# enkeejunior1/Diffusion-Pullback

Measured on AMD Instinct MI355X. Metric: pullback top-k SVD iters/sec (SD-v1.5 mid-block, 4x64x64), higher is better.
Workload: dtype bf16; 1 GPU; BASELINE configs[2]: SD-v1.5 4x64x64 latent, no edit prompt (seeded null ctx[1,77,768]), mid-block h[1280,8,8], t=696.27; pca_rank=5, ctx=null, samples_total=5, samples_this_rank=5, samples_advanced_together=1, spectrum=shaped (configs.Spectrum()), parallelism=single process, no collective, rccl_world_size=0, repeats=7

## Files before the change

### diffusion_pullback_amd/csrc/attn_fused.hip

```cpp
#include "kernels.h"

namespace dpb {

#ifndef DPB_ATT_ABL
#define DPB_ATT_ABL 0
#endif
#ifndef DPB_OUT_STORE_ATT
#define DPB_OUT_STORE_ATT 0
#endif
#define DPB_ATT_PAD 8

constexpr int att_waves(int d) { return d > 80 ? 4 : 8; }

template <int D, int W = att_waves(D)> struct FA {
  static constexpr int WAVES = W, NT = WAVES * 64;
  static constexpr int NS = (D + 15) / 16;
  static constexpr int DP = NS * 16;
  static constexpr int ND = (D + 31) / 32;
  static constexpr int DO = ND * 32;
  static constexpr int BI = D <= 80 ? 128 : 64;
  static constexpr int LDR = (DP > DO ? DP : DO) + DPB_ATT_PAD;
  static constexpr int LDT = BI + 4;
  static constexpr int ROW_ELEMS = BI * LDR;
  static constexpr int T_ELEMS = DO * LDT;
};

template <int D, int NTH = FA<D>::NT> struct RowRegs { uint4 v[(FA<D>::BI * (FA<D>::DP / 8) + NTH - 1) / NTH]; };
template <int D, int NTH = FA<D>::NT, unsigned ONE = 0>
__device__ inline void fetch_row(const bf16* __restrict__ src, long gs, RowRegs<D, NTH>& rg, int tid) {
  using F = FA<D>;
  constexpr int CPR = F::DP / 8, N = (F::BI * CPR + NTH - 1) / NTH;
#pragma unroll
  for (int i = 0; i < N; ++i) {
    const int c = tid + i * NTH;
    const int r = c / CPR, cc = (c % CPR) * 8;
    rg.v[i] = make_uint4(ONE != 0 && cc == D ? ONE : 0u, 0, 0, 0);
    if (c < F::BI * CPR && cc < D) rg.v[i] = *reinterpret_cast<const uint4*>(src + (long)r * gs + cc);
  }
}
template <int D, int NTH = FA<D>::NT>
__device__ inline void commit_row(const RowRegs<D, NTH>& rg, bf16* lds, int tid) {
  using F = FA<D>;
  constexpr int CPR = F::DP / 8, N = (F::BI * CPR + NTH - 1) / NTH;
#pragma unroll
  for (int i = 0; i < N; ++i) {
    const int c = tid + i * NTH;
    if (c < F::BI * CPR) *reinterpret_cast<uint4*>(lds + (c / CPR) * F::LDR + (c % CPR) * 8) = rg.v[i];
  }
}
template <int D, int NTH = FA<D>::NT> struct TRegs { uint4 v[(FA<D>::DO * (FA<D>::BI / 8) + NTH - 1) / NTH]; };
template <int D, int NTH = FA<D>::NT>
__device__ inline void fetch_t(const bf16* __restrict__ src, long gs, TRegs<D, NTH>& rg, int tid) {
  using F = FA<D>;
  constexpr int CPR = F::BI / 8, N = (F::DO * CPR + NTH - 1) / NTH;
#pragma unroll
  for (int i = 0; i < N; ++i) {
    const int c = tid + i * NTH;
    const int r = c / CPR, cc = (c % CPR) * 8;
    rg.v[i] = make_uint4(0, 0, 0, 0);
    if (c < F::DO * CPR && r < D) rg.v[i] = *reinterpret_cast<const uint4*>(src + (long)r * gs + cc);
  }
}
template <int D, int NTH = FA<D>::NT>
__device__ inline void commit_t(const TRegs<D, NTH>& rg, bf16* lds, int tid) {
  using F = FA<D>;
  constexpr int CPR = F::BI / 8, N = (F::DO * CPR + NTH - 1) / NTH;
#pragma unroll
  for (int i = 0; i < N; ++i) {
    const int c = tid + i * NTH;
    if (c < F::DO * CPR) {
      bf16* dst = lds + (c / CPR) * F::LDT + (c % CPR) * 8;
      *reinterpret_cast<uint2*>(dst) = make_uint2(rg.v[i].x, rg.v[i].y);
      *reinterpret_cast<uint2*>(dst + 4) = make_uint2(rg.v[i].z, rg.v[i].w);
    }
  }
}
template <int D>
__device__ inline void load_outer_frags(const bf16* __restrict__ rowptr, bf16x8* f, int lhi) {
  using F = FA<D>;
#pragma unroll
  for (int st = 0; st < F::NS; ++st) {
    const int col = st * 16 + lhi * 8;
    uint4 v = make_uint4(0, 0, 0, 0);
    if (col < D) v = *reinterpret_cast<const uint4*>(rowptr + col);
    f[st] = *reinterpret_cast<bf16x8*>(&v);
  }
}
__device__ inline bf16x8 lds_a_frag(const bf16* tile, int row, int ld, int col) {
  return *reinterpret_cast<const bf16x8*>(tile + row * ld + col);
}
__device__ inline bf16x8 lds_t_frag(const bf16* tile, int drow, int ld, int base, int lhi) {
  uint2 lo = *reinterpret_cast<const uint2*>(tile + drow * ld + base + 4 * lhi);
  uint2 hi = *reinterpret_cast<const uint2*>(tile + drow * ld + base + 8 + 4 * lhi);
  uint4 v = make_uint4(lo.x, lo.y, hi.x, hi.y);
  return *reinterpret_cast<bf16x8*>(&v);
}
typedef __attribute__((ext_vector_type(4))) short short4_;
__device__ inline bf16x8 lds_tr_frag(const bf16* tile, int ld, int base, int d0, int lane) {
  const int i16 = lane & 15, g = lane >> 4;
  const bf16* p = tile + (base + 4 * (g >> 1) + (i16 >> 2)) * ld + d0 + (g & 1) * 16 + (i16 & 3) * 4;
  short4_ lo = __builtin_amdgcn_ds_read_tr16_b64_v4i16((__attribute__((address_space(3))) short4_*)p);
  short4_ hi = __builtin_amdgcn_ds_read_tr16_b64_v4i16((__attribute__((address_space(3))) short4_*)(p + 8 * ld));
  uint2 l2 = *reinterpret_cast<uint2*>(&lo), h2 = *reinterpret_cast<uint2*>(&hi);
  uint4 v = make_uint4(l2.x, l2.y, h2.x, h2.y);
  return *reinterpret_cast<bf16x8*>(&v);
}
template <int FL>
__device__ inline void pack_b(const float* x, bf16x8* out) {
  out[0] = H16<FL>::pack8(x);
  out[1] = H16<FL>::pack8(x + 8);
}
struct BlockXY { int x, y; };
__device__ inline BlockXY xcd_group_blocks(int on) {
  const int nx = gridDim.x, ny = gridDim.y;
  if (!on || (ny & 7)) return {(int)blockIdx.x, (int)blockIdx.y};
  const int lin = blockIdx.y * nx + blockIdx.x, xcd = lin & 7, slot = lin >> 3;
  return {slot % nx, (slot / nx) * 8 + xcd};
}

static int g_attn_shared = getenv("DPB_ATTN_SHARED") ? atoi(getenv("DPB_ATTN_SHARED")) : 2;
void attn_debug_shared(int bits) { g_attn_shared = bits; }

#define MFMA(a, b, c) H16<FL>::mfma(a, b, c)

struct FusedArgs {
  const bf16 *Q, *K, *V, *O;
  const bf16 *KT, *VT, *QT;
  const float* stats;
  float* Drow;
  float* Dout;
  const bf16 *dQ, *dK, *dV, *dVT;
  bf16* dO;
  const bf16 *gO, *gOT;
  bf16 *gQ, *gK, *gV;
  int accQ, accK, accV;
  int xcd;
  int L, C, Co, H, kps;
  float scale;
};

template <int D, int FL, int W = att_waves(D)>
__global__ __launch_bounds__((FA<D, W>::NT)) void attn_fwd_kernel(FusedArgs a, bf16* O, float* stats_out) {
  using F = FA<D, W>;
  __shared__ __attribute__((aligned(16))) bf16 sm[2 * F::ROW_ELEMS];
  bf16* sK = sm; bf16* sV = sK + F::ROW_ELEMS;
  const int tid = threadIdx.x, lane = tid & 63, wave = tid >> 6, l31 = lane & 31, lhi = lane >> 5;
  const BlockXY blk = xcd_group_blocks(a.xcd);
  const int b = blk.y / a.H, h = blk.y % a.H;
  const int q_ = blk.x * (F::WAVES * 32) + wave * 32 + l31;
  const bool live = q_ < a.L;
  const int q = live ? q_ : a.L - 1;
  const long LC = (long)a.L * a.C;
  const bf16* Kp = a.K + b * LC + h * D;
  const bf16* Vp = a.V + b * LC + h * D;
  bf16x8 qf[F::NS];
  load_outer_frags<D>(a.Q + b * LC + (long)q * a.C + h * D, qf, lhi);
  const float c2 = a.scale * 1.44269504088896f;
  constexpr float FWD_THR = 4.f;
  constexpr bool LSUM = F::DP > D;
  constexpr unsigned ONE16 = FL ? 0x3C00u : 0x3F80u, VONE = LSUM ? ONE16 : 0u;
  f32x16 acc[F::ND];
#pragma unroll
  for (int d = 0; d < F::ND; ++d)
#pragma unroll
    for (int r = 0; r < 16; ++r) acc[d][r] = 0.f;
  float m = -INFINITY, l = 0.f;
  RowRegs<D, F::NT> rK, rV;
  fetch_row<D, F::NT>(Kp, a.C, rK, tid); fetch_row<D, F::NT, VONE>(Vp, a.C, rV, tid);
  for (int k0 = 0; k0 < a.L; k0 += F::BI) {
    __syncthreads();
    commit_row<D, F::NT>(rK, sK, tid); commit_row<D, F::NT>(rV, sV, tid);
    __syncthreads();
    if (k0 + F::BI < a.L) {
      const int k1 = k0 + F::BI;
      fetch_row<D, F::NT>(Kp + (long)k1 * a.C, a.C, rK, tid); fetch_row<D, F::NT, VONE>(Vp + (long)k1 * a.C, a.C, rV, tid);
    }
#pragma unroll
    for (int kb = 0; kb < F::BI / 32; ++kb) {
      f32x16 s;
#pragma unroll
      for (int r = 0; r < 16; ++r) s[r] = 0.f;
#pragma unroll
      for (int stp = 0; stp < F::NS; ++stp) s = MFMA(lds_a_frag(sK, kb * 32 + l31, F::LDR, stp * 16 + lhi * 8), qf[stp], s);
      float mx = s[0];
#pragma unroll
      for (int r = 1; r < 16; ++r) mx = fmaxf(mx, s[r]);
      mx = fmaxf(mx, __shfl_xor(mx, 32, 64)) * c2;
      if (!__all(mx - m <= FWD_THR)) {
        const float mn = fmaxf(m, mx);
        const float alpha = __builtin_amdgcn_exp2f(m - mn);
#pragma unroll
        for (int d = 0; d < F::ND; ++d)
#pragma unroll
          for (int r = 0; r < 16; ++r) acc[d][r] *= alpha;
        if (!LSUM) l *= alpha;
        m = mn;
      }
      float p[16];
#pragma unroll
      for (int r = 0; r < 16; ++r) p[r] = __builtin_amdgcn_exp2f(__builtin_fmaf(s[r], c2, -m));
      if (!LSUM) {
        float ps = 0.f;
#pragma unroll
        for (int r = 0; r < 16; ++r) ps += p[r];
        ps += __shfl_xor(ps, 32, 64);
        l += ps;
      }
      bf16x8 pb[2];
      pack_b<FL>(p, pb);
#pragma unroll
      for (int ks = 0; ks < 2; ++ks)
#pragma unroll
        for (int d = 0; d < F::ND; ++d)
          acc[d] = MFMA(lds_tr_frag(sV, F::LDR, kb * 32 + ks * 16, d * 32, lane), pb[ks], acc[d]);
    }
  }
  if (LSUM) {
    static_assert(!LSUM || (D % 8 == 0 && (D % 32) / 8 * 4 < 16), "ones column of V outside the accumulator layout");
    const float lv = acc[D / 32][(D % 32) / 8 * 4];
    const float lo = __shfl_xor(lv, 32, 64);
    l = lhi == 0 ? lv : lo;
  }
  const float il = 1.f / l;
  if (lhi == 0 && live) {
    float* st = stats_out + (((long)b * a.H + h) * a.L + q) * 2;
    st[0] = m * 0.69314718055994531f;
    st[1] = il;
  }
  bf16* Op = O + b * (long)a.L * a.Co + (long)q * a.Co + h * D;
#pragma unroll
  for (int d = 0; d < F::ND; ++d)
#pragma unroll
    for (int g = 0; g < 4; ++g) {
      const int col = d * 32 + 8 * g + 4 * lhi;
      if (col < D && live) {
        store_out8<DPB_OUT_STORE_ATT>(Op + col, H16<FL>::pack2(acc[d][g * 4] * il, acc[d][g * 4 + 1] * il),
                                                         H16<FL>::pack2(acc[d][g * 4 + 2] * il, acc[d][g * 4 + 3] * il));
      }
    }
}

template <int D, int FL, int W = att_waves(D)>
__global__ __launch_bounds__((FA<D, W>::NT), (W == 4 && D <= 40 ? 2 : 1)) void attn_jvp_kernel(FusedArgs a) {
  using F = FA<D, W>;
  __shared__ __attribute__((aligned(16))) bf16 sm[4 * F::ROW_ELEMS];
  bf16* sK = sm; bf16* sdK = sK + F::ROW_ELEMS; bf16* sV = sdK + F::ROW_ELEMS; bf16* sdV = sV + F::ROW_ELEMS;
  const int tid = threadIdx.x, lane = tid & 63, wave = tid >> 6, l31 = lane & 31, lhi = lane >> 5;
  const BlockXY blk = xcd_group_blocks(a.xcd);
  const int j = blk.y / a.H, h = blk.y % a.H, b = j / a.kps;
  const int q_ = blk.x * (F::WAVES * 32) + wave * 32 + l31;
  const bool live = q_ < a.L;
  const int q = live ? q_ : a.L - 1;
  const long LC = (long)a.L * a.C;
  const bf16* Qp = a.Q + b * LC + h * D;
  const bf16* Kp = a.K + b * LC + h * D;
  const bf16* dQp = a.dQ + j * LC + h * D;
  const bf16* dKp = a.dK + j * LC + h * D;
  const bf16* Vp = a.V + b * LC + h * D;
  const bf16* dVp = a.dV + j * LC + h * D;
  bf16x8 qf[F::NS], dqf[F::NS];
  load_outer_frags<D>(Qp + (long)q * a.C, qf, lhi);
  load_outer_frags<D>(dQp + (long)q * a.C, dqf, lhi);
  const float* st = a.stats + (((long)b * a.H + h) * a.L + q) * 2;
  const float c2 = a.scale * 1.44269504088896f;
  const float m2 = st[0] * 1.44269504088896f - __builtin_log2f(st[1]);
  constexpr bool SUMROW = F::DO > D && ((D % 32) & 4) == 0;
  constexpr unsigned ONE16 = FL ? 0x3C00u : 0x3F80u, VONE = (SUMROW && F::DP > D) ? ONE16 : 0u;
  if constexpr (SUMROW && F::DP == D) {
    for (int r = tid; r < F::BI; r += F::NT) {
      reinterpret_cast<unsigned short*>(sV)[r * F::LDR + D] = (unsigned short)ONE16;
      reinterpret_cast<unsigned short*>(sdV)[r * F::LDR + D] = 0;
    }
  }
  f32x16 acc[F::ND];
#pragma unroll
  for (int d = 0; d < F::ND; ++d)
#pragma unroll
    for (int r = 0; r < 16; ++r) acc[d][r] = 0.f;
  float delta = 0.f;
  RowRegs<D, F::NT> rK, rdK, rV, rdV;
  fetch_row<D, F::NT>(Kp, a.C, rK, tid); fetch_row<D, F::NT>(dKp, a.C, rdK, tid);
  fetch_row<D, F::NT, VONE>(Vp, a.C, rV, tid); fetch_row<D, F::NT>(dVp, a.C, rdV, tid);
  for (int k0 = 0; k0 < a.L; k0 += F::BI) {
    __syncthreads();
    commit_row<D, F::NT>(rK, sK, tid); commit_row<D, F::NT>(rdK, sdK, tid); commit_row<D, F::NT>(rV, sV, tid); commit_row<D, F::NT>(rdV, sdV, tid);
    __syncthreads();
    if (k0 + F::BI < a.L) {
      const int k1 = k0 + F::BI;
      fetch_row<D, F::NT>(Kp + (long)k1 * a.C, a.C, rK, tid); fetch_row<D, F::NT>(dKp + (long)k1 * a.C, a.C, rdK, tid);
      fetch_row<D, F::NT, VONE>(Vp + (long)k1 * a.C, a.C, rV, tid); fetch_row<D, F::NT>(dVp + (long)k1 * a.C, a.C, rdV, tid);
    }
    constexpr bool PIPE = D <= 40;
    bf16x8 kf[F::NS], dkf[F::NS];
    auto load1 = [&](int kb) {
#pragma unroll
      for (int stp = 0; stp < F::NS; ++stp) {
        kf[stp] = lds_a_frag(sK, kb * 32 + l31, F::LDR, stp * 16 + lhi * 8);
        dkf[stp] = lds_a_frag(sdK, kb * 32 + l31, F::LDR, stp * 16 + lhi * 8);
      }
    };
    if constexpr (PIPE) load1(0);
#pragma unroll
    for (int kb = 0; kb < F::BI / 32; ++kb) {
      bf16x8 vf[2][F::ND], dvf[2][F::ND];
      if constexpr (PIPE) {
#pragma unroll
        for (int ks = 0; ks < 2; ++ks)
#pragma unroll
          for (int d = 0; d < F::ND; ++d) {
            vf[ks][d] = lds_tr_frag(sV, F::LDR, kb * 32 + ks * 16, d * 32, lane);
            dvf[ks][d] = lds_tr_frag(sdV, F::LDR, kb * 32 + ks * 16, d * 32, lane);
          }
        __builtin_amdgcn_sched_barrier(0);
      } else {
        load1(kb);
      }
      f32x16 s, ds;
#pragma unroll
      for (int r = 0; r < 16; ++r) s[r] = ds[r] = 0.f;
#pragma unroll
      for (int stp = 0; stp < F::NS; ++stp) {
        s = MFMA(kf[stp], qf[stp], s);
        ds = MFMA(kf[stp], dqf[stp], ds);
        if (!((DPB_ATT_ABL & 2) && D == 40 && stp == F::NS - 1)) ds = MFMA(dkf[stp], qf[stp], ds);
      }
      if constexpr (PIPE) {
        __builtin_amdgcn_sched_barrier(0);
        if (kb + 1 < F::BI / 32) load1(kb + 1);
        __builtin_amdgcn_sched_barrier(0);
      }
      float p[16], x[16];
#pragma unroll
      for (int r = 0; r < 16; ++r) {
        p[r] = (DPB_ATT_ABL & 4) ? c2 * s[r] - m2 : __builtin_amdgcn_exp2f(c2 * s[r] - m2);
        x[r] = p[r] * (a.scale * ds[r]);
        if constexpr (!SUMROW) delta += x[r];
      }
      bf16x8 pb[2], xb[2];
      pack_b<FL>(p, pb);
      pack_b<FL>(x, xb);
#pragma unroll
      for (int ks = 0; ks < 2; ++ks)
#pragma unroll
        for (int d = 0; d < F::ND; ++d) {
          if constexpr (!PIPE) {
            vf[ks][d] = lds_tr_frag(sV, F::LDR, kb * 32 + ks * 16, d * 32, lane);
            dvf[ks][d] = lds_tr_frag(sdV, F::LDR, kb * 32 + ks * 16, d * 32, lane);
          }
          if ((DPB_ATT_ABL & 1) && D == 40 && ks == 1 && d == 1) continue;
          acc[d] = MFMA(vf[ks][d], xb[ks], acc[d]);
          acc[d] = MFMA(dvf[ks][d], pb[ks], acc[d]);
        }
    }
  }
  if constexpr (SUMROW) delta = __shfl(acc[D / 32][((D % 32) & 3) + 4 * ((D % 32) >> 3)], l31, 64);
  else delta += __shfl_xor(delta, 32, 64);
  const long LCo = (long)a.L * a.Co;
  const bf16* Op = a.O + b * LCo + (long)q * a.Co + h * D;
  bf16* dOp = a.dO + j * LCo + (long)q * a.Co + h * D;
#pragma unroll
  for (int d = 0; d < F::ND; ++d)
#pragma unroll
    for (int g = 0; g < 4; ++g) {
      const int col = d * 32 + 8 * g + 4 * lhi;
      if (col < D && live) {
        uint2 ov = *reinterpret_cast<const uint2*>(Op + col);
        unsigned ow[2] = {ov.x, ov.y};
        unsigned w[2];
#pragma unroll
        for (int i = 0; i < 2; ++i) {
          float o0 = H16<FL>::lo(ow[i]), o1 = H16<FL>::hi(ow[i]);
          float v0 = acc[d][g * 4 + 2 * i] - delta * o0, v1 = acc[d][g * 4 + 2 * i + 1] - delta * o1;
          w[i] = H16<FL>::pack2(v0, v1);
        }
        store_out8<DPB_OUT_STORE_ATT>(dOp + col, w[0], w[1]);
      }
    }
}

template <int D, int FL>
__global__ __launch_bounds__(FA<D>::NT) void attn_adj_q_kernel(FusedArgs a) {
  using F = FA<D>;
  __shared__ __attribute__((aligned(16))) bf16 sm[2 * F::ROW_ELEMS];
  bf16* sK = sm; bf16* sV = sK + F::ROW_ELEMS;
  const int tid = threadIdx.x, lane = tid & 63, wave = tid >> 6, l31 = lane & 31, lhi = lane >> 5;
  const BlockXY blk = xcd_group_blocks(a.xcd);
  const int j = blk.y / a.H, h = blk.y % a.H, b = j / a.kps;
  const int q_ = blk.x * (F::WAVES * 32) + wave * 32 + l31;
  const bool live = q_ < a.L;
  const int q = live ? q_ : a.L - 1;
  const long LC = (long)a.L * a.C;
  const bf16* Kp = a.K + b * LC + h * D;
  const bf16* Vp = a.V + b * LC + h * D;
  bf16x8 qf[F::NS], gof[F::NS], of[F::NS];
  load_outer_frags<D>(a.Q + b * LC + (long)q * a.C + h * D, qf, lhi);
  const long LCo = (long)a.L * a.Co;
  load_outer_frags<D>(a.gO + j * LCo + (long)q * a.Co + h * D, gof, lhi);
  load_outer_frags<D>(a.O + b * LCo + (long)q * a.Co + h * D, of, lhi);
  float Dq = 0.f;
#pragma unroll
  for (int stp = 0; stp < F::NS; ++stp) {
    const unsigned short* g16 = reinterpret_cast<const unsigned short*>(&gof[stp]);
    const unsigned short* o16 = reinterpret_cast<const unsigned short*>(&of[stp]);
#pragma unroll
    for (int e = 0; e < 8; ++e) Dq += H16<FL>::up(g16[e]) * H16<FL>::up(o16[e]);
  }
  Dq += __shfl_xor(Dq, 32, 64);
  const float* st = a.stats + (((long)b * a.H + h) * a.L + q) * 2;
  const float c2 = a.scale * 1.44269504088896f;
  const float m2 = st[0] * 1.44269504088896f - __builtin_log2f(st[1]);
  f32x16 acc[F::ND];
#pragma unroll
  for (int d = 0; d < F::ND; ++d)
#pragma unroll
    for (int r = 0; r < 16; ++r) acc[d][r] = 0.f;
  RowRegs<D> rK, rV;
  fetch_row<D>(Kp, a.C, rK, tid); fetch_row<D>(Vp, a.C, rV, tid);
  for (int k0 = 0; k0 < a.L; k0 += F::BI) {
    __syncthreads();
    commit_row<D>(rK, sK, tid); commit_row<D>(rV, sV, tid);
    __syncthreads();
    if (k0 + F::BI < a.L) {
      const int k1 = k0 + F::BI;
      fetch_row<D>(Kp + (long)k1 * a.C, a.C, rK, tid); fetch_row<D>(Vp + (long)k1 * a.C, a.C, rV, tid);
    }
#pragma unroll
    for (int kb = 0; kb < F::BI / 32; ++kb) {
      f32x16 s, gp;
#pragma unroll
      for (int r = 0; r < 16; ++r) s[r] = gp[r] = 0.f;
#pragma unroll
      for (int stp = 0; stp < F::NS; ++stp) {
        s = MFMA(lds_a_frag(sK, kb * 32 + l31, F::LDR, stp * 16 + lhi * 8), qf[stp], s);
        gp = MFMA(lds_a_frag(sV, kb * 32 + l31, F::LDR, stp * 16 + lhi * 8), gof[stp], gp);
      }
      float gs[16];
#pragma unroll
      for (int r = 0; r < 16; ++r) gs[r] = __builtin_amdgcn_exp2f(c2 * s[r] - m2) * (gp[r] - Dq);
      bf16x8 gsb[2];
      pack_b<FL>(gs, gsb);
#pragma unroll
      for (int ks = 0; ks < 2; ++ks)
#pragma unroll
        for (int d = 0; d < F::ND; ++d)
          acc[d] = MFMA(lds_tr_frag(sK, F::LDR, kb * 32 + ks * 16, d * 32, lane), gsb[ks], acc[d]);
    }
  }
  bf16* gQp = a.gQ + j * LC + (long)q * a.C + h * D;
#pragma unroll
  for (int d = 0; d < F::ND; ++d)
#pragma unroll
    for (int g = 0; g < 4; ++g) {
      const int col = d * 32 + 8 * g + 4 * lhi;
      if (col < D && live) {
        float v[4];
#pragma unroll
        for (int i = 0; i < 4; ++i) v[i] = a.scale * acc[d][g * 4 + i];
        if (a.accQ) {
          uint2 ov = *reinterpret_cast<const uint2*>(gQp + col);
          v[0] += H16<FL>::lo(ov.x); v[1] += H16<FL>::hi(ov.x);
          v[2] += H16<FL>::lo(ov.y); v[3] += H16<FL>::hi(ov.y);
        }
        store_out8<DPB_OUT_STORE_ATT>(gQp + col, H16<FL>::pack2(v[0], v[1]), H16<FL>::pack2(v[2], v[3]));
      }
    }
}

template <int D, int TJ, int FL>
__global__ __launch_bounds__(256) void attn_adj_q_multi_kernel(FusedArgs a) {
  using F = FA<D>;
  constexpr int NTH = 256;
  __shared__ __attribute__((aligned(16))) bf16 sm[2 * F::ROW_ELEMS];
  bf16* sK = sm; bf16* sV = sK + F::ROW_ELEMS;
  const int tid = threadIdx.x, lane = tid & 63, wave = tid >> 6, l31 = lane & 31, lhi = lane >> 5;
  const int ngrp = (a.kps + TJ - 1) / TJ;
  const int grp = blockIdx.y % ngrp, bh = blockIdx.y / ngrp, b = bh / a.H, h = bh % a.H;
  const int j0 = b * a.kps + grp * TJ, nj = min(TJ, a.kps - grp * TJ);
  const int q = blockIdx.x * 128 + wave * 32 + l31;
  const long LC = (long)a.L * a.C, LCo = (long)a.L * a.Co;
  const bf16* Kp = a.K + b * LC + h * D;
  const bf16* Vp = a.V + b * LC + h * D;
  bf16x8 qf[F::NS], gof[TJ][F::NS];
  load_outer_frags<D>(a.Q + b * LC + (long)q * a.C + h * D, qf, lhi);
  float Dq[TJ];
  {
    bf16x8 of[F::NS];
    load_outer_frags<D>(a.O + b * LCo + (long)q * a.Co + h * D, of, lhi);
#pragma unroll
    for (int t = 0; t < TJ; ++t) {
      Dq[t] = 0.f;
      if (t < nj) {
        load_outer_frags<D>(a.gO + (long)(j0 + t) * LCo + (long)q * a.Co + h * D, gof[t], lhi);
#pragma unroll
        for (int stp = 0; stp < F::NS; ++stp) {
          const unsigned short* g16 = reinterpret_cast<const unsigned short*>(&gof[t][stp]);
          const unsigned short* o16 = reinterpret_cast<const unsigned short*>(&of[stp]);
#pragma unroll
          for (int e = 0; e < 8; ++e) Dq[t] += H16<FL>::up(g16[e]) * H16<FL>::up(o16[e]);
        }
        Dq[t] += __shfl_xor(Dq[t], 32, 64);
        if (a.Dout && lhi == 0) a.Dout[((long)(j0 + t) * a.H + h) * a.L + q] = Dq[t];
      } else {
#pragma unroll
        for (int stp = 0; stp < F::NS; ++stp) gof[t][stp] = bf16x8{};
      }
    }
  }
  const float* st = a.stats + (((long)b * a.H + h) * a.L + q) * 2;
  const float c2 = a.scale * 1.44269504088896f;
  const float m2 = st[0] * 1.44269504088896f - __builtin_log2f(st[1]);
  f32x16 acc[TJ][F::ND];
#pragma unroll
  for (int t = 0; t < TJ; ++t)
#pragma unroll
    for (int d = 0; d < F::ND; ++d)
#pragma unroll
      for (int r = 0; r < 16; ++r) acc[t][d][r] = 0.f;
  RowRegs<D, NTH> rK, rV;
  fetch_row<D, NTH>(Kp, a.C, rK, tid); fetch_row<D, NTH>(Vp, a.C, rV, tid);
  for (int k0 = 0; k0 < a.L; k0 += F::BI) {
    __syncthreads();
    commit_row<D, NTH>(rK, sK, tid); commit_row<D, NTH>(rV, sV, tid);
    __syncthreads();
    if (k0 + F::BI < a.L) {
      const int k1 = k0 + F::BI;
      fetch_row<D, NTH>(Kp + (long)k1 * a.C, a.C, rK, tid); fetch_row<D, NTH>(Vp + (long)k1 * a.C, a.C, rV, tid);
    }
#pragma unroll
    for (int kb = 0; kb < F::BI / 32; ++kb) {
      bf16x8 vf[F::NS], ktf[2][F::ND];
      f32x16 s;
#pragma unroll
      for (int r = 0; r < 16; ++r) s[r] = 0.f;
#pragma unroll
      for (int stp = 0; stp < F::NS; ++stp) {
        s = MFMA(lds_a_frag(sK, kb * 32 + l31, F::LDR, stp * 16 + lhi * 8), qf[stp], s);
        vf[stp] = lds_a_frag(sV, kb * 32 + l31, F::LDR, stp * 16 + lhi * 8);
      }
#pragma unroll
      for (int ks = 0; ks < 2; ++ks)
#pragma unroll
        for (int d = 0; d < F::ND; ++d) ktf[ks][d] = lds_tr_frag(sK, F::LDR, kb * 32 + ks * 16, d * 32, lane);
      float p[16];
#pragma unroll
      for (int r = 0; r < 16; ++r) p[r] = __builtin_amdgcn_exp2f(c2 * s[r] - m2);
#pragma unroll
      for (int t = 0; t < TJ; ++t) {
        if (t < nj) {
          f32x16 gp;
#pragma unroll
          for (int r = 0; r < 16; ++r) gp[r] = 0.f;
#pragma unroll
          for (int stp = 0; stp < F::NS; ++stp) gp = MFMA(vf[stp], gof[t][stp], gp);
          float gs[16];
#pragma unroll
          for (int r = 0; r < 16; ++r) gs[r] = p[r] * (gp[r] - Dq[t]);
          bf16x8 gsb[2];
          pack_b<FL>(gs, gsb);
#pragma unroll
          for (int ks = 0; ks < 2; ++ks)
#pragma unroll
            for (int d = 0; d < F::ND; ++d) {
              if ((DPB_ATT_ABL & 1) && D == 40 && ks == 1 && d == 1) continue;
              acc[t][d] = MFMA(ktf[ks][d], gsb[ks], acc[t][d]);
            }
        }
      }
    }
  }
#pragma unroll
  for (int t = 0; t < TJ; ++t) {
    if (t >= nj) continue;
    bf16* gQp = a.gQ + (long)(j0 + t) * LC + (long)q * a.C + h * D;
#pragma unroll
    for (int d = 0; d < F::ND; ++d)
#pragma unroll
      for (int g = 0; g < 4; ++g) {
        const int col = d * 32 + 8 * g + 4 * lhi;
        if (col < D) {
          float v[4];
#pragma unroll
          for (int i = 0; i < 4; ++i) v[i] = a.scale * acc[t][d][g * 4 + i];
          if (a.accQ) {
            uint2 ov = *reinterpret_cast<const uint2*>(gQp + col);
            v[0] += H16<FL>::lo(ov.x); v[1] += H16<FL>::hi(ov.x);
            v[2] += H16<FL>::lo(ov.y); v[3] += H16<FL>::hi(ov.y);
          }
          store_out8<DPB_OUT_STORE_ATT>(gQp + col, H16<FL>::pack2(v[0], v[1]), H16<FL>::pack2(v[2], v[3]));
        }
      }
  }
}

template <int D, int FL, int W = att_waves(D)>
__global__ __launch_bounds__((FA<D, W>::NT), (D <= 40 ? 2 : 1)) void attn_adj_kv_kernel(FusedArgs a) {
  using F = FA<D, W>;
  __shared__ __attribute__((aligned(16))) bf16 sm[2 * F::ROW_ELEMS];
  __shared__ float sstat[2][F::BI];
  bf16* sQ = sm; bf16* sgO = sQ + F::ROW_ELEMS;
  const int tid = threadIdx.x, lane = tid & 63, wave = tid >> 6, l31 = lane & 31, lhi = lane >> 5;
  const BlockXY blk = xcd_group_blocks(a.xcd);
  const int j = blk.y / a.H, h = blk.y % a.H, b = j / a.kps;
  const int key_ = blk.x * (F::WAVES * 32) + wave * 32 + l31;
  const bool live = key_ < a.L;
  const int key = live ? key_ : a.L - 1;
  const long LC = (long)a.L * a.C;
  const bf16* Qp = a.Q + b * LC + h * D;
  const long LCo = (long)a.L * a.Co;
  const bf16* Op = a.O + b * LCo + h * D;
  const bf16* gOp = a.gO + j * LCo + h * D;
  const float* stp_ = a.stats + ((long)b * a.H + h) * a.L * 2;
  bf16x8 kf[F::NS], vf[F::NS];
  load_outer_frags<D>(a.K + b * LC + (long)key * a.C + h * D, kf, lhi);
  load_outer_frags<D>(a.V + b * LC + (long)key * a.C + h * D, vf, lhi);
  const float c2 = a.scale * 1.44269504088896f;
  f32x16 accK[F::ND], accV[F::ND];
#pragma unroll
  for (int d = 0; d < F::ND; ++d)
#pragma unroll
    for (int r = 0; r < 16; ++r) accK[d][r] = accV[d][r] = 0.f;
  RowRegs<D, F::NT> rQ, rgO;
  float st0 = 0.f, st2 = 0.f;
  auto fetch_stats = [&](int q0) {
    if (tid < F::BI) {
      const int qq = q0 + tid;
      st0 = stp_[2 * qq] * 1.44269504088896f - __builtin_log2f(stp_[2 * qq + 1]);
      float dq = 0.f;
      for (int c = 0; c < D; c += 8) {
        float g8[8], o8[8];
        H16<FL>::load8(gOp + (long)qq * a.Co + c, g8);
        H16<FL>::load8(Op + (long)qq * a.Co + c, o8);
#pragma unroll
        for (int e = 0; e < 8; ++e) dq += g8[e] * o8[e];
      }
      st2 = dq;
    }
  };
  fetch_row<D, F::NT>(Qp, a.C, rQ, tid); fetch_row<D, F::NT>(gOp, a.Co, rgO, tid);
  fetch_stats(0);
  for (int q0 = 0; q0 < a.L; q0 += F::BI) {
    __syncthreads();
    commit_row<D, F::NT>(rQ, sQ, tid); commit_row<D, F::NT>(rgO, sgO, tid);
    if (tid < F::BI) { sstat[0][tid] = st0; sstat[1][tid] = st2; }
    __syncthreads();
    if (q0 + F::BI < a.L) {
      const int q1 = q0 + F::BI;
      fetch_row<D, F::NT>(Qp + (long)q1 * a.C, a.C, rQ, tid); fetch_row<D, F::NT>(gOp + (long)q1 * a.Co, a.Co, rgO, tid);
      fetch_stats(q1);
    }
#pragma unroll
    for (int qb = 0; qb < F::BI / 32; ++qb) {
      f32x16 s, gp;
#pragma unroll
      for (int r = 0; r < 16; ++r) s[r] = gp[r] = 0.f;
#pragma unroll
      for (int stp = 0; stp < F::NS; ++stp) {
        s = MFMA(lds_a_frag(sQ, qb * 32 + l31, F::LDR, stp * 16 + lhi * 8), kf[stp], s);
        gp = MFMA(lds_a_frag(sgO, qb * 32 + l31, F::LDR, stp * 16 + lhi * 8), vf[stp], gp);
      }
      float p[16], gs[16];
#pragma unroll
      for (int r = 0; r < 16; ++r) {
        const int qi = qb * 32 + (r & 3) + 8 * (r >> 2) + 4 * lhi;
        p[r] = __builtin_amdgcn_exp2f(c2 * s[r] - sstat[0][qi]);
        gs[r] = p[r] * (gp[r] - sstat[1][qi]);
      }
      bf16x8 pb[2], gsb[2];
      pack_b<FL>(p, pb);
      pack_b<FL>(gs, gsb);
#pragma unroll
      for (int ks = 0; ks < 2; ++ks)
#pragma unroll
        for (int d = 0; d < F::ND; ++d) {
          accV[d] = MFMA(lds_tr_frag(sgO, F::LDR, qb * 32 + ks * 16, d * 32, lane), pb[ks], accV[d]);
          accK[d] = MFMA(lds_tr_frag(sQ, F::LDR, qb * 32 + ks * 16, d * 32, lane), gsb[ks], accK[d]);
        }
    }
  }
  bf16* gKp = a.gK + j * LC + (long)key * a.C + h * D;
  bf16* gVp = a.gV + j * LC + (long)key * a.C + h * D;
  const bool kv_same = a.gK == a.gV;
#pragma unroll
  for (int d = 0; d < F::ND; ++d)
#pragma unroll
    for (int g = 0; g < 4; ++g) {
      const int col = d * 32 + 8 * g + 4 * lhi;
      if (col < D && live) {
        float vk[4], vv[4];
#pragma unroll
        for (int i = 0; i < 4; ++i) { vk[i] = a.scale * accK[d][g * 4 + i]; vv[i] = accV[d][g * 4 + i]; }
        if (kv_same)
          for (int i = 0; i < 4; ++i) vk[i] += vv[i];
        if (a.accK) {
          uint2 ov = *reinterpret_cast<const uint2*>(gKp + col);
          vk[0] += H16<FL>::lo(ov.x); vk[1] += H16<FL>::hi(ov.x);
          vk[2] += H16<FL>::lo(ov.y); vk[3] += H16<FL>::hi(ov.y);
        }
        if (a.accV && !kv_same) {
          uint2 ov = *reinterpret_cast<const uint2*>(gVp + col);
          vv[0] += H16<FL>::lo(ov.x); vv[1] += H16<FL>::hi(ov.x);
          vv[2] += H16<FL>::lo(ov.y); vv[3] += H16<FL>::hi(ov.y);
        }
        store_out8<DPB_OUT_STORE_ATT>(gKp + col, H16<FL>::pack2(vk[0], vk[1]), H16<FL>::pack2(vk[2], vk[3]));
        if (!kv_same) store_out8<DPB_OUT_STORE_ATT>(gVp + col, H16<FL>::pack2(vv[0], vv[1]), H16<FL>::pack2(vv[2], vv[3]));
      }
    }
}

template <int D, int FL>
__global__ __launch_bounds__(256) void attn_rowdot_kernel(FusedArgs a, int nt) {
  const long idx = (long)blockIdx.x * 256 + threadIdx.x;
  if (idx >= (long)nt * a.L * a.H) return;
  const int h = (int)(idx % a.H);
  const long jq = idx / a.H;
  const int q = (int)(jq % a.L), j = (int)(jq / a.L), b = j / a.kps;
  const bf16* gp_ = a.gO + ((long)j * a.L + q) * a.Co + h * D;
  const bf16* op_ = a.O + ((long)b * a.L + q) * a.Co + h * D;
  float dq = 0.f;
#pragma unroll
  for (int c = 0; c < D; c += 8) {
    float g8[8], o8[8];
    H16<FL>::load8(gp_ + c, g8);
    H16<FL>::load8(op_ + c, o8);
#pragma unroll
    for (int e = 0; e < 8; ++e) dq += g8[e] * o8[e];
  }
  a.Drow[((long)j * a.H + h) * a.L + q] = dq;
}

template <int D, int TJ> struct SHK {
  static constexpr int QG = 2, NP = QG, NW = NP + QG * TJ, NT = NW * 64;
  static constexpr int BI = 64;
  static constexpr int NS = (D + 15) / 16, DP = NS * 16, ND = (D + 31) / 32, DO = ND * 32;
  static constexpr int LDR = (DP > DO ? DP : DO) + DPB_ATT_PAD, ROW_ELEMS = BI * LDR;
  static constexpr int NTILE = 1 + TJ, CPR = DP / 8;
  static constexpr int CPT = BI * CPR;
  static constexpr int NLD = NTILE * CPT / NT;
  static_assert(NTILE * CPT % NT == 0, "whole loads per thread");
};

template <int D, int TJ, int FL>
__global__ __launch_bounds__((SHK<D, TJ>::NT)) void attn_adj_kv_shared_kernel(FusedArgs a) {
  using S = SHK<D, TJ>;
  __shared__ __attribute__((aligned(16))) bf16 sm[2 * S::NTILE * S::ROW_ELEMS];
  __shared__ __attribute__((aligned(16))) uint4 sP[2][2][S::QG][2][64];
  __shared__ float sD[2][TJ][S::BI];
  const int tid = threadIdx.x, lane = tid & 63, wave = tid >> 6, l31 = lane & 31, lhi = lane >> 5;
  const int ngrp = (a.kps + TJ - 1) / TJ;
  const int grp = blockIdx.y % ngrp, bh = blockIdx.y / ngrp, b = bh / a.H, h = bh % a.H;
  const int j0 = b * a.kps + grp * TJ, nj = min(TJ, a.kps - grp * TJ);
  const long LC = (long)a.L * a.C, LCo = (long)a.L * a.Co;
  const bf16* Qp = a.Q + b * LC + h * D;
  const float* stp_ = a.stats + ((long)b * a.H + h) * a.L * 2;
  const bf16* lsrc[S::NLD];
  long lstr[S::NLD];
  int ldst[S::NLD];
#pragma unroll
  for (int i = 0; i < S::NLD; ++i) {
    const int c = tid + i * S::NT, tile = c / S::CPT, lrow = (c % S::CPT) / S::CPR, lcc = (c % S::CPR) * 8;
    const bf16* base = nullptr;
    lstr[i] = tile == 0 ? a.C : a.Co;
    if (tile == 0) base = Qp;
    else if (tile - 1 < nj) base = a.gO + (long)(j0 + tile - 1) * LCo + h * D;
    lsrc[i] = (base && lcc < D) ? base + (long)lrow * lstr[i] + lcc : nullptr;
    ldst[i] = tile * S::ROW_ELEMS + lrow * S::LDR + lcc;
  }
  uint4 rg[S::NLD];
  float dreg = 0.f;
  const int dt_ = tid / S::BI, dq_ = tid % S::BI;
  auto fetch = [&](int q0) {
#pragma unroll
    for (int i = 0; i < S::NLD; ++i) rg[i] = lsrc[i] ? *reinterpret_cast<const uint4*>(lsrc[i] + (long)q0 * lstr[i]) : make_uint4(0, 0, 0, 0);
    if (dt_ < nj) dreg = a.Drow[((long)(j0 + dt_) * a.H + h) * a.L + q0 + dq_];
  };
  auto commit = [&](int par) {
#pragma unroll
    for (int i = 0; i < S::NLD; ++i) *reinterpret_cast<uint4*>(sm + par * S::NTILE * S::ROW_ELEMS + ldst[i]) = rg[i];
    if (dt_ < TJ) sD[par][dt_][dq_] = dreg;
  };
  const bool producer = wave < S::NP;
  const int g = producer ? wave : (wave - S::NP) % S::QG;
  const int t = producer ? 0 : (wave - S::NP) / S::QG;
  const int key = blockIdx.x * (S::QG * 32) + g * 32 + l31;
  const float c2 = a.scale * 1.44269504088896f;
  const int nst = a.L / S::BI;
  bf16x8 of[S::NS];
  load_outer_frags<D>((producer ? a.K : a.V) + b * LC + (long)key * a.C + h * D, of, lhi);
  fetch(0);
  commit(0);
  if (nst > 1) fetch(S::BI);
  if (producer) {
    bf16x8 qfn[2][S::NS];
    float4 stn[2][8];
    auto load_q = [&](int q0) {
#pragma unroll
      for (int qb = 0; qb < 2; ++qb) {
#pragma unroll
        for (int st_ = 0; st_ < S::NS; ++st_) {
          const int col = st_ * 16 + lhi * 8;
          uint4 v = make_uint4(0, 0, 0, 0);
          if (col < D) v = *reinterpret_cast<const uint4*>(Qp + (long)(q0 + qb * 32 + l31) * a.C + col);
          qfn[qb][st_] = *reinterpret_cast<bf16x8*>(&v);
        }
#pragma unroll
        for (int gg = 0; gg < 4; ++gg) {
          const float* sp = stp_ + 2 * (long)(q0 + qb * 32 + 8 * gg + 4 * lhi);
          stn[qb][2 * gg] = *reinterpret_cast<const float4*>(sp);
          stn[qb][2 * gg + 1] = *reinterpret_cast<const float4*>(sp + 4);
        }
      }
    };
    auto produce = [&](int par) {
#pragma unroll
      for (int qb = 0; qb < 2; ++qb) {
        f32x16 sc;
#pragma unroll
        for (int r = 0; r < 16; ++r) sc[r] = 0.f;
#pragma unroll
        for (int st_ = 0; st_ < S::NS; ++st_) sc = MFMA(qfn[qb][st_], of[st_], sc);
        float p[16];
#pragma unroll
        for (int gg = 0; gg < 4; ++gg) {
          const float4 s0 = stn[qb][2 * gg], s1 = stn[qb][2 * gg + 1];
          p[4 * gg] = __builtin_amdgcn_exp2f(c2 * sc[4 * gg] - s0.x * 1.44269504088896f) * s0.y;
          p[4 * gg + 1] = __builtin_amdgcn_exp2f(c2 * sc[4 * gg + 1] - s0.z * 1.44269504088896f) * s0.w;
          p[4 * gg + 2] = __builtin_amdgcn_exp2f(c2 * sc[4 * gg + 2] - s1.x * 1.44269504088896f) * s1.y;
          p[4 * gg + 3] = __builtin_amdgcn_exp2f(c2 * sc[4 * gg + 3] - s1.z * 1.44269504088896f) * s1.w;
        }
        bf16x8 pb[2];
        pack_b<FL>(p, pb);
        sP[par][qb][g][0][lane] = *reinterpret_cast<uint4*>(&pb[0]);
        sP[par][qb][g][1][lane] = *reinterpret_cast<uint4*>(&pb[1]);
      }
    };
    load_q(0);
    produce(0);
    if (nst > 1) load_q(S::BI);
    __syncthreads();
    for (int s = 0; s < nst; ++s) {
      if (s + 1 < nst) {
        commit((s + 1) & 1);
        if (s + 2 < nst) fetch((s + 2) * S::BI);
        produce((s + 1) & 1);
        if (s + 2 < nst) load_q((s + 2) * S::BI);
      }
      __syncthreads();
    }
    return;
  }
  f32x16 accK[S::ND], accV[S::ND];
#pragma unroll
  for (int d = 0; d < S::ND; ++d)
#pragma unroll
    for (int r = 0; r < 16; ++r) accK[d][r] = accV[d][r] = 0.f;
  __syncthreads();
  for (int s = 0; s < nst; ++s) {
    if (s + 1 < nst) {
      commit((s + 1) & 1);
      if (s + 2 < nst) fetch((s + 2) * S::BI);
    }
    if (t < nj) {
      const bf16* sQ = sm + (s & 1) * S::NTILE * S::ROW_ELEMS;
      const bf16* sgO = sQ + (1 + t) * S::ROW_ELEMS;
#pragma unroll
      for (int qb = 0; qb < 2; ++qb) {
        f32x16 gp;
#pragma unroll
        for (int r = 0; r < 16; ++r) gp[r] = 0.f;
#pragma unroll
        for (int st_ = 0; st_ < S::NS; ++st_) gp = MFMA(lds_a_frag(sgO, qb * 32 + l31, S::LDR, st_ * 16 + lhi * 8), of[st_], gp);
        uint4 pw[2] = {sP[s & 1][qb][g][0][lane], sP[s & 1][qb][g][1][lane]};
        const unsigned w[8] = {pw[0].x, pw[0].y, pw[0].z, pw[0].w, pw[1].x, pw[1].y, pw[1].z, pw[1].w};
        float gs[16];
#pragma unroll
        for (int i = 0; i < 8; ++i) {
          const int r0 = 2 * i, r1 = 2 * i + 1;
          const int q0i = qb * 32 + (r0 & 3) + 8 * (r0 >> 2) + 4 * lhi;
          gs[r0] = H16<FL>::lo(w[i]) * (gp[r0] - sD[s & 1][t][q0i]);
          gs[r1] = H16<FL>::hi(w[i]) * (gp[r1] - sD[s & 1][t][q0i + 1]);
        }
        bf16x8 gsb[2];
        pack_b<FL>(gs, gsb);
#pragma unroll
        for (int ks = 0; ks < 2; ++ks)
#pragma unroll
          for (int d = 0; d < S::ND; ++d) {
            if ((DPB_ATT_ABL & 1) && D == 40 && ks == 1 && d == 1) continue;
            accV[d] = MFMA(lds_tr_frag(sgO, S::LDR, qb * 32 + ks * 16, d * 32, lane), *reinterpret_cast<bf16x8*>(&pw[ks]), accV[d]);
            accK[d] = MFMA(lds_tr_frag(sQ, S::LDR, qb * 32 + ks * 16, d * 32, lane), gsb[ks], accK[d]);
          }
      }
    }
    __syncthreads();
  }
  if (t >= nj) return;
  bf16* gKp = a.gK + (long)(j0 + t) * LC + (long)key * a.C + h * D;
  bf16* gVp = a.gV + (long)(j0 + t) * LC + (long)key * a.C + h * D;
  const bool kv_same = a.gK == a.gV;
#pragma unroll
  for (int d = 0; d < S::ND; ++d)
#pragma unroll
    for (int gg = 0; gg < 4; ++gg) {
      const int col = d * 32 + 8 * gg + 4 * lhi;
      if (col < D) {
        float vk[4], vv[4];
#pragma unroll
        for (int i = 0; i < 4; ++i) { vk[i] = a.scale * accK[d][gg * 4 + i]; vv[i] = accV[d][gg * 4 + i]; }
        if (kv_same)
          for (int i = 0; i < 4; ++i) vk[i] += vv[i];
        if (a.accK) {
          uint2 ov = *reinterpret_cast<const uint2*>(gKp + col);
          vk[0] += H16<FL>::lo(ov.x); vk[1] += H16<FL>::hi(ov.x);
          vk[2] += H16<FL>::lo(ov.y); vk[3] += H16<FL>::hi(ov.y);
        }
        if (a.accV && !kv_same) {
          uint2 ov = *reinterpret_cast<const uint2*>(gVp + col);
          vv[0] += H16<FL>::lo(ov.x); vv[1] += H16<FL>::hi(ov.x);
          vv[2] += H16<FL>::lo(ov.y); vv[3] += H16<FL>::hi(ov.y);
        }
        store_out8<DPB_OUT_STORE_ATT>(gKp + col, H16<FL>::pack2(vk[0], vk[1]), H16<FL>::pack2(vk[2], vk[3]));
        if (!kv_same) store_out8<DPB_OUT_STORE_ATT>(gVp + col, H16<FL>::pack2(vv[0], vv[1]), H16<FL>::pack2(vv[2], vv[3]));
      }
    }
}

struct CrossArgs {
  const bf16 *Q, *K, *V;
  const bf16* BT;
  const bf16* X; bf16* Y;
  int L, Lk, Lkp, C, Ck, Cx, Cy, H, kps, a_is_v, accumulate, xcd;
  int primal;
  float scale, c_in, c_out;
};
constexpr int XKEYS = 96, XLDT = XKEYS + 4;

template <int D, int FL>
__global__ __launch_bounds__(256) void attn_cross_kernel(CrossArgs a) {
  using F = FA<D>;
  __shared__ __attribute__((aligned(16))) bf16 sm[2 * XKEYS * F::LDR + F::DO * XLDT];
  bf16* sK = sm; bf16* sV = sK + XKEYS * F::LDR; bf16* sBT = sV + XKEYS * F::LDR;
  const int tid = threadIdx.x, nthr = blockDim.x, lane = tid & 63, wave = tid >> 6, l31 = lane & 31, lhi = lane >> 5;
  const BlockXY blk = xcd_group_blocks(a.xcd);
  const int j = blk.y / a.H, h = blk.y % a.H, b = j / a.kps;
  const int q = blk.x * (nthr >> 1) + wave * 32 + l31;
  {
    constexpr int CPR = F::DP / 8;
    const bf16* Kp = a.K + (long)b * a.Lk * a.Ck + h * D;
    const bf16* Vp = a.V + (long)b * a.Lk * a.Ck + h * D;
    for (int c = tid; c < XKEYS * CPR; c += nthr) {
      const int r = c / CPR, cc = (c % CPR) * 8;
      uint4 kv = make_uint4(0, 0, 0, 0), vv = kv;
      if (r < a.Lk && cc < D) {
        kv = *reinterpret_cast<const uint4*>(Kp + (long)r * a.Ck + cc);
        vv = *reinterpret_cast<const uint4*>(Vp + (long)r * a.Ck + cc);
      }
      *reinterpret_cast<uint4*>(sK + r * F::LDR + cc) = kv;
      *reinterpret_cast<uint4*>(sV + r * F::LDR + cc) = vv;
    }
    constexpr int CPT = XKEYS / 8;
    if (a.BT) {
      const bf16* Bp = a.BT + ((long)b * a.H + h) * D * a.Lkp;
      for (int c = tid; c < F::DO * CPT; c += nthr) {
        const int r = c / CPT, cc = (c % CPT) * 8;
        uint4 v = make_uint4(0, 0, 0, 0);
        if (r < D && cc < a.Lkp) v = *reinterpret_cast<const uint4*>(Bp + (long)r * a.Lkp + cc);
        bf16* dst = sBT + r * XLDT + cc;
        *reinterpret_cast<uint2*>(dst) = make_uint2(v.x, v.y);
        *reinterpret_cast<uint2*>(dst + 4) = make_uint2(v.z, v.w);
      }
    } else {
      const bf16* Bp = (a.a_is_v ? a.K : a.V) + (long)b * a.Lk * a.Ck + h * D;
      for (int c = tid; c < XKEYS * (F::DO / 8); c += nthr) {
        const int r = c % XKEYS, cc = (c / XKEYS) * 8;
        uint4 v = make_uint4(0, 0, 0, 0);
        if (r < a.Lk && cc < D) v = *reinterpret_cast<const uint4*>(Bp + (long)r * a.Ck + cc);
        const unsigned short* e = reinterpret_cast<const unsigned short*>(&v);
#pragma unroll
        for (int i = 0; i < 8; ++i) sBT[(cc + i) * XLDT + r].v = e[i];
      }
    }
  }
  bf16x8 qf[F::NS], xf[F::NS];
  load_outer_frags<D>(a.Q + (long)b * a.L * a.C + (long)q * a.C + h * D, qf, lhi);
  if (!a.primal) load_outer_frags<D>(a.X + (long)j * a.L * a.Cx + (long)q * a.Cx + h * D, xf, lhi);
  __syncthreads();
  const bf16* sA = a.a_is_v ? sV : sK;
  f32x16 s[3], t[3];
#pragma unroll
  for (int kb = 0; kb < 3; ++kb) {
#pragma unroll
    for (int r = 0; r < 16; ++r) s[kb][r] = t[kb][r] = 0.f;
#pragma unroll
    for (int stp = 0; stp < F::NS; ++stp) {
      s[kb] = MFMA(lds_a_frag(sK, kb * 32 + l31, F::LDR, stp * 16 + lhi * 8), qf[stp], s[kb]);
      if (!a.primal) t[kb] = MFMA(lds_a_frag(sA, kb * 32 + l31, F::LDR, stp * 16 + lhi * 8), xf[stp], t[kb]);
    }
  }
  const float c2 = a.scale * 1.44269504088896f;
  float mx = -INFINITY;
#pragma unroll
  for (int kb = 0; kb < 3; ++kb)
#pragma unroll
    for (int r = 0; r < 16; ++r) {
      const int key = kb * 32 + (r & 3) + 8 * (r >> 2) + 4 * lhi;
      s[kb][r] = key < a.Lk ? s[kb][r] * c2 : -INFINITY;
      mx = fmaxf(mx, s[kb][r]);
    }
  mx = fmaxf(mx, __shfl_xor(mx, 32, 64));
  float l = 0.f;
#pragma unroll
  for (int kb = 0; kb < 3; ++kb)
#pragma unroll
    for (int r = 0; r < 16; ++r) { s[kb][r] = __builtin_amdgcn_exp2f(s[kb][r] - mx); l += s[kb][r]; }
  l += __shfl_xor(l, 32, 64);
  const float il = 1.f / l;
  float delta = 0.f;
#pragma unroll
  for (int kb = 0; kb < 3; ++kb)
#pragma unroll
    for (int r = 0; r < 16; ++r) {
      s[kb][r] *= il;
      t[kb][r] *= a.c_in * s[kb][r];
      delta += t[kb][r];
    }
  delta += __shfl_xor(delta, 32, 64);
  f32x16 acc[F::ND];
#pragma unroll
  for (int d = 0; d < F::ND; ++d)
#pragma unroll
    for (int r = 0; r < 16; ++r) acc[d][r] = 0.f;
#pragma unroll
  for (int kb = 0; kb < 3; ++kb) {
    float w[16];
#pragma unroll
    for (int r = 0; r < 16; ++r) w[r] = a.primal ? s[kb][r] : t[kb][r] - delta * s[kb][r];
    bf16x8 wb[2];
    pack_b<FL>(w, wb);
#pragma unroll
    for (int ks = 0; ks < 2; ++ks)
#pragma unroll
      for (int d = 0; d < F::ND; ++d)
        acc[d] = MFMA(lds_t_frag(sBT, d * 32 + l31, XLDT, kb * 32 + ks * 16, lhi), wb[ks], acc[d]);
  }
  bf16* Yp = a.Y + (long)j * a.L * a.Cy + (long)q * a.Cy + h * D;
#pragma unroll
  for (int d = 0; d < F::ND; ++d)
#pragma unroll
    for (int g = 0; g < 4; ++g) {
      const int col = d * 32 + 8 * g + 4 * lhi;
      if (col < D) {
        float v[4];
#pragma unroll
        for (int i = 0; i < 4; ++i) v[i] = a.c_out * acc[d][g * 4 + i];
        if (a.accumulate) {
          uint2 ov = *reinterpret_cast<const uint2*>(Yp + col);
          v[0] += H16<FL>::lo(ov.x); v[1] += H16<FL>::hi(ov.x);
          v[2] += H16<FL>::lo(ov.y); v[3] += H16<FL>::hi(ov.y);
        }
        *reinterpret_cast<uint2*>(Yp + col) =
            make_uint2(H16<FL>::pack2(v[0], v[1]), H16<FL>::pack2(v[2], v[3]));
      }
    }
}

static bool head_dim_ok(int d) { return d == 40 || d == 64 || d == 80 || d == 160; }
#define DPB_ATT_DISPATCH(d, fl, ...)                                                        \
  do {                                                                                       \
    if ((fl) == 0) { constexpr int FL = 0; DPB_ATT_D(d, __VA_ARGS__) } else { constexpr int FL = 1; DPB_ATT_D(d, __VA_ARGS__) } \
  } while (0)
#define DPB_ATT_D(d, ...)                                          \
  if ((d) == 40) { constexpr int D = 40; __VA_ARGS__; }            \
  else if ((d) == 64) { constexpr int D = 64; __VA_ARGS__; }       \
  else if ((d) == 80) { constexpr int D = 80; __VA_ARGS__; }       \
  else { constexpr int D = 160; __VA_ARGS__; }

int cross_attention_supported(int dtype, int d, int Lq, int Lk, int kv_const) {
  return dtype != DT_F32 && kv_const && head_dim_ok(d) && Lk <= XKEYS && Lq % 32 == 0 && (Lq >= 128 ? Lq % 128 == 0 : true);
}

int launch_attn_cross(const CrossAttnArgs& f, int nt, hipStream_t st) {
  CrossArgs a;
  a.Q = (const bf16*)f.Q; a.K = (const bf16*)f.K; a.V = (const bf16*)f.V; a.BT = (const bf16*)f.BT;
  a.X = (const bf16*)f.X; a.Y = (bf16*)f.Y;
  a.L = f.L; a.Lk = f.Lk; a.Lkp = f.Lkp; a.C = f.C; a.Ck = f.Ck; a.Cx = f.Cx; a.Cy = f.Cy; a.H = f.H; a.kps = f.kps;
  a.a_is_v = f.adjoint; a.accumulate = f.accumulate; a.scale = f.scale; a.xcd = 0;
  a.c_in = f.adjoint ? 1.f : f.scale; a.c_out = f.adjoint ? f.scale : 1.f;
  a.primal = f.primal;
  if (f.primal) { a.a_is_v = 0; a.c_in = 1.f; a.c_out = 1.f; a.accumulate = 0; }
  const int waves = f.L >= 128 ? 4 : f.L / 32;
  dim3 grid(f.L / (waves * 32), nt * f.H);
  if (!head_dim_ok(f.d)) { set_error("cross attention: head dim %d unsupported", f.d); return -1; }
  DPB_ATT_DISPATCH(f.d, f.fl, hipLaunchKernelGGL((attn_cross_kernel<D, FL>), grid, dim3(waves * 64), 0, st, a));
  DPB_CHECK(hipGetLastError());
  return 0;
}

template <int FL>
__global__ __launch_bounds__(256) void row_stats_kernel(const bf16* S, float* stats, long nrows, int Lk, int ld) {
  const int lane = threadIdx.x & 63;
  const long row = (long)blockIdx.x * 4 + (threadIdx.x >> 6);
  if (row >= nrows) return;
  const bf16* sp = S + row * ld;
  float m = -INFINITY;
  for (int c = lane * 8; c < Lk; c += 512) {
    float v[8];
    H16<FL>::load8(sp + c, v);
#pragma unroll
    for (int e = 0; e < 8; ++e) if (c + e < Lk) m = fmaxf(m, v[e]);
  }
  m = wave_max(m);
  float s = 0.f;
  for (int c = lane * 8; c < Lk; c += 512) {
    float v[8];
    H16<FL>::load8(sp + c, v);
#pragma unroll
    for (int e = 0; e < 8; ++e) if (c + e < Lk) s += __expf(v[e] - m);
  }
  s = wave_sum(s);
  if (lane == 0) { stats[2 * row] = m; stats[2 * row + 1] = 1.f / s; }
}

int fused_attention_supported(int dtype, int d, int L, int kv_const) {
  return dtype != DT_F32 && !kv_const && head_dim_ok(d) && ((L >= 256 && L % (att_waves(d) * 32) == 0) || (d == 160 && L == 64));
}

int launch_row_stats(int fl, const void* S, float* stats, long nrows, int Lk, int ld, hipStream_t st) {
  if (fl) hipLaunchKernelGGL((row_stats_kernel<1>), dim3((unsigned)((nrows + 3) / 4)), dim3(256), 0, st, (const bf16*)S, stats, nrows, Lk, ld);
  else hipLaunchKernelGGL((row_stats_kernel<0>), dim3((unsigned)((nrows + 3) / 4)), dim3(256), 0, st, (const bf16*)S, stats, nrows, Lk, ld);
  DPB_CHECK(hipGetLastError());
  return 0;
}

static int attn_xcd_on() { static int on = getenv("DPB_ATTN_XCD") ? atoi(getenv("DPB_ATTN_XCD")) : 0; return on; }

static FusedArgs to_args(const FusedAttnArgs& f) {
  FusedArgs a;
  a.xcd = attn_xcd_on();
  a.Q = (const bf16*)f.Q; a.K = (const bf16*)f.K; a.V = (const bf16*)f.V; a.O = (const bf16*)f.O;
  a.KT = (const bf16*)f.KT; a.VT = (const bf16*)f.VT; a.QT = (const bf16*)f.QT; a.stats = f.stats; a.Drow = f.Drow; a.Dout = nullptr;
  a.dQ = (const bf16*)f.dQ; a.dK = (const bf16*)f.dK; a.dV = (const bf16*)f.dV; a.dVT = (const bf16*)f.dVT; a.dO = (bf16*)f.dO;
  a.gO = (const bf16*)f.gO; a.gOT = (const bf16*)f.gOT; a.gQ = (bf16*)f.gQ; a.gK = (bf16*)f.gK; a.gV = (bf16*)f.gV;
  a.accQ = f.accQ; a.accK = f.accK; a.accV = f.accV;
  a.L = f.L; a.C = f.C; a.Co = f.Co; a.H = f.H; a.kps = f.kps; a.scale = f.scale;
  return a;
}

int launch_attn_fwd_fused(const FusedAttnArgs& f, int batch, void* O, float* stats, hipStream_t st) {
  FusedArgs a = to_args(f);
  dim3 grid((f.L + att_waves(f.d) * 32 - 1) / (att_waves(f.d) * 32), batch * f.H);
  if (!head_dim_ok(f.d)) { set_error("fused attention: head dim %d unsupported", f.d); return -1; }
  static const int fwd4 = getenv("DPB_ATTN_FWD4") ? atoi(getenv("DPB_ATTN_FWD4")) : 1;
  if (fwd4 && att_waves(f.d) == 8 && f.L % 128 == 0 && f.L >= 256 && (long)grid.x * grid.y < 256) {
    dim3 g4(f.L / 128, batch * f.H);
    if (f.d == 40) { if (f.fl) hipLaunchKernelGGL((attn_fwd_kernel<40, 1, 4>), g4, dim3(256), 0, st, a, (bf16*)O, stats); else hipLaunchKernelGGL((attn_fwd_kernel<40, 0, 4>), g4, dim3(256), 0, st, a, (bf16*)O, stats); }
    else if (f.d == 64) { if (f.fl) hipLaunchKernelGGL((attn_fwd_kernel<64, 1, 4>), g4, dim3(256), 0, st, a, (bf16*)O, stats); else hipLaunchKernelGGL((attn_fwd_kernel<64, 0, 4>), g4, dim3(256), 0, st, a, (bf16*)O, stats); }
    else { if (f.fl) hipLaunchKernelGGL((attn_fwd_kernel<80, 1, 4>), g4, dim3(256), 0, st, a, (bf16*)O, stats); else hipLaunchKernelGGL((attn_fwd_kernel<80, 0, 4>), g4, dim3(256), 0, st, a, (bf16*)O, stats); }
    DPB_CHECK(hipGetLastError());
    return 0;
  }
  DPB_ATT_DISPATCH(f.d, f.fl, hipLaunchKernelGGL((attn_fwd_kernel<D, FL>), grid, dim3(att_waves(D) * 64), 0, st, a, (bf16*)O, stats));
  DPB_CHECK(hipGetLastError());
  return 0;
}

static int att_block_waves(int d, int L, int pairs) {
  static const int force = getenv("DPB_ATTN_WAVES") ? atoi(getenv("DPB_ATTN_WAVES")) : 0;
  if (d != 40 || L % 256) return att_waves(d);
  if (force == 4 || force == 8) return force;
  return ((long)(L / 256) * pairs) % 256 == 0 ? 8 : 4;
}

int attn_jvp_block_waves(int d, int L, int pairs) { return att_block_waves(d, L, pairs); }

int launch_attn_jvp_fused(const FusedAttnArgs& f, int nt, hipStream_t st) {
  FusedArgs a = to_args(f);
  if (!head_dim_ok(f.d)) { set_error("fused attention: head dim %d unsupported", f.d); return -1; }
  if (att_block_waves(f.d, f.L, nt * f.H) == 4 && f.d == 40) {
    dim3 g4(f.L / 128, nt * f.H);
    if (f.fl) hipLaunchKernelGGL((attn_jvp_kernel<40, 1, 4>), g4, dim3(256), 0, st, a);
    else hipLaunchKernelGGL((attn_jvp_kernel<40, 0, 4>), g4, dim3(256), 0, st, a);
    DPB_CHECK(hipGetLastError());
    return 0;
  }
  dim3 grid((f.L + att_waves(f.d) * 32 - 1) / (att_waves(f.d) * 32), nt * f.H);
  DPB_ATT_DISPATCH(f.d, f.fl, hipLaunchKernelGGL((attn_jvp_kernel<D, FL>), grid, dim3(att_waves(D) * 64), 0, st, a));
  DPB_CHECK(hipGetLastError());
  return 0;
}

static int attn_adj_route(int d, int L, int kps, int nt, bool have_drow) {
  static const int multi = getenv("DPB_ATTN_MULTI") ? atoi(getenv("DPB_ATTN_MULTI")) : 1;
  const int shared = g_attn_shared;
  const bool dsh = d == 40 || (d == 64 && (shared & 4));
  int r = 0;
  if (dsh && (multi & 1) && L % 128 == 0 && nt % kps == 0) r |= 1;
  if (dsh && (shared & 2) && L % 64 == 0 && kps >= 4 && nt % kps == 0 && have_drow) r |= 2;
  return r;
}
int attn_adj_route_bits(int d, int L, int kps, int nt) { return attn_adj_route(d, L, kps, nt, true); }
int attn_adj_launches(int d, int L, int kps, int nt) { const int r = attn_adj_route(d, L, kps, nt, true); return 2 + (r == 2); }

int launch_attn_adj_fused(const FusedAttnArgs& f, int nt, hipStream_t st) {
  FusedArgs a = to_args(f);
  dim3 grid((f.L + att_waves(f.d) * 32 - 1) / (att_waves(f.d) * 32), nt * f.H);
  if (!head_dim_ok(f.d)) { set_error("fused attention: head dim %d unsupported", f.d); return -1; }
  const int route = attn_adj_route(f.d, f.L, f.kps, nt, f.Drow != nullptr);
  if (route & 1) {
    constexpr int TJ = 5;
    const int ngrp = (f.kps + TJ - 1) / TJ;
    const dim3 gq(f.L / 128, (nt / f.kps) * f.H * ngrp);
    if (route & 2) a.Dout = a.Drow;
#define DPB_ADJQ(DV, FLV) hipLaunchKernelGGL((attn_adj_q_multi_kernel<DV, TJ, FLV>), gq, dim3(256), 0, st, a)
    if (f.d == 40) { if (f.fl) DPB_ADJQ(40, 1); else DPB_ADJQ(40, 0); }
    else { if (f.fl) DPB_ADJQ(64, 1); else DPB_ADJQ(64, 0); }
#undef DPB_ADJQ
  } else {
    DPB_ATT_DISPATCH(f.d, f.fl, hipLaunchKernelGGL((attn_adj_q_kernel<D, FL>), grid, dim3(att_waves(D) * 64), 0, st, a));
  }
  if (route & 2) {
    constexpr int TJ = 5;
    const int ngrp = (f.kps + TJ - 1) / TJ;
    const dim3 gs(f.L / 64, (nt / f.kps) * f.H * ngrp);
    const unsigned nrd = (unsigned)(((long)nt * f.L * f.H + 255) / 256);
#define DPB_ADJKV(DV, FLV)                                                                                                          \
    do {                                                                                                                              \
      if (!(route & 1)) hipLaunchKernelGGL((attn_rowdot_kernel<DV, FLV>), dim3(nrd), dim3(256), 0, st, a, nt);                       \
      hipLaunchKernelGGL((attn_adj_kv_shared_kernel<DV, TJ, FLV>), gs, dim3(SHK<DV, TJ>::NT), 0, st, a);                             \
    } while (0)
    if (f.d == 40) { if (f.fl) DPB_ADJKV(40, 1); else DPB_ADJKV(40, 0); }
    else { if (f.fl) DPB_ADJKV(64, 1); else DPB_ADJKV(64, 0); }
#undef DPB_ADJKV
  } else if (att_block_waves(f.d, f.L, nt * f.H) == 4 && f.d == 40) {
    dim3 g4(f.L / 128, nt * f.H);
    if (f.fl) hipLaunchKernelGGL((attn_adj_kv_kernel<40, 1, 4>), g4, dim3(256), 0, st, a);
    else hipLaunchKernelGGL((attn_adj_kv_kernel<40, 0, 4>), g4, dim3(256), 0, st, a);
  } else {
    DPB_ATT_DISPATCH(f.d, f.fl, hipLaunchKernelGGL((attn_adj_kv_kernel<D, FL>), grid, dim3(att_waves(D) * 64), 0, st, a));
  }
  DPB_CHECK(hipGetLastError());
  return 0;
}

}
```

### diffusion_pullback_amd/csrc/engine.cpp

```cpp
#include <math.h>
#include <stdarg.h>
#include <stdio.h>
#include <stdlib.h>
#include <string.h>

#include <string>
#include <vector>

#include "../../include/dpb.h"
#include "kernels.h"

namespace dpb {

static thread_local char g_err[1024] = "";
void set_error(const char* fmt, ...) {
  va_list ap;
  va_start(ap, fmt);
  vsnprintf(g_err, sizeof(g_err), fmt, ap);
  va_end(ap);
}
const char* last_error() { return g_err; }

static inline size_t align_up(size_t v, size_t a = 256) { return (v + a - 1) / a * a; }
static inline int round8(int v) { return (v + 7) / 8 * 8; }

struct Buf {
  int rows = 0, C = 0, kind = 0, Cv = 0;
  bool is_const = true;
  size_t p_off = 0, t_off = 0, g_off = 0, g_off0 = 0;
};

struct AttnPlan {
  int heads = 0, d = 0, Lq = 0, Lk = 0, Lqp = 0, Lkp = 0;
  bool causal = false;
  bool kv_const = false, fused = false, cross = false;
  int oq = 0, ok = 0, ov = 0;
  size_t P = 0, PT = 0, KT = 0, VT = 0, QT = 0, stats = 0;
};

struct Op {
  dpb_op_desc d;
  bool is_const = true;
  int attn = -1;
  size_t pstats = 0, tstats = 0;
  int geglu_next = -1;
  int geglu_prev = -1;
  int ln_next = -1;
  int ln_prev = -1;
};

}

using namespace dpb;

struct dpb_engine {
  int dtype = DT_F32, es = 4;
  int maxB = 1, maxT = 1;
  std::vector<Buf> bufs;
  std::vector<Op> ops;
  std::vector<AttnPlan> plans;
  std::vector<int> producer;
  int x_buf = -1, x_channels = 0, temb_buf = -1, temb_dim = 0, temb_flip = 0, temb_hm1 = 0, ctx_buf = -1;
  hipStream_t stream = 0;
  char* ws = nullptr;
  size_t ws_bytes = 0;
  size_t pstats_off = 0, pstats_bytes = 0, tstats_off = 0, tstats_bytes = 0, gnpart = 0, gnpart_bytes = 0, gnticket = 0;
  size_t S1 = 0, S2 = 0, T1 = 0, Dv = 0, convtmp = 0, io_in = 0, io_out = 0, orth = 0, slab = 0, slab_bytes = 64u << 20, zeros = 0;
  size_t orth_stride = 0;
  size_t pbW = 0;
  size_t temb_host_stage = 0;
  int cur_batch = 0;
  std::vector<int> uses;
  int cur_tap = -1;
  int src = -1;
  const char* bact = nullptr;
  const char* oact = nullptr;
  std::vector<std::vector<char>> act_cache;
  int primal_last = -1;
  int fwd_seed = -1;
  const float* fwd_h = nullptr;
  struct { bool on = false; GemmArgs a; } pend;
  bool fwd_only = false;
  std::vector<char> ginit;
  std::vector<char> skip;
  long n_launch = 0;
  double flops = 0, gbytes = 0;
  struct GraphKey {
    int tap, k, B; const void *V, *U, *s, *conv;
    bool operator==(const GraphKey& o) const { return tap == o.tap && k == o.k && B == o.B && V == o.V && U == o.U && s == o.s && conv == o.conv; }
  };
  hipGraphExec_t gexec = nullptr;
  GraphKey gkey{};
  long g_launches = 0; double g_flops = 0, g_bytes = 0;
  bool profiling = false;
  struct Prof { hipEvent_t a, b; double flops; int big; int M, N, K, Z, gather; };
  std::vector<Prof> prof;
  float prof_overhead_ms = 0.f;

  char* P(int b) const { return ws + bufs[b].p_off; }
  char* T(int b) const { return ws + bufs[b].t_off; }
  char* G(int b) const { return ws + bufs[b].g_off; }
};

namespace {

int fail(const char* fmt, ...) {
  va_list ap;
  va_start(ap, fmt);
  vsnprintf(g_err, sizeof(g_err), fmt, ap);
  va_end(ap);
  return -1;
}

void gemm_prep(dpb_engine* e, GemmArgs& a) {
  a.slab = (float*)(e->ws + e->slab);
  a.zeros = e->ws + e->zeros;
  a.slab_bytes = e->slab_bytes;
}

int g_lazy_reduce = getenv("DPB_LAZY_REDUCE") ? atoi(getenv("DPB_LAZY_REDUCE")) : 1;
int g_ln_fuse = getenv("DPB_LN_FUSE") ? atoi(getenv("DPB_LN_FUSE")) : 0;
int g_ln_kmax = getenv("DPB_LN_FUSE_KMAX") ? atoi(getenv("DPB_LN_FUSE_KMAX")) : 1024;

int flush_pending(dpb_engine* e) {
  if (!e->pend.on) return 0;
  e->pend.on = false;
  e->n_launch++;
  return launch_gemm_reduce(e->dtype, e->pend.a, e->stream);
}

int prof_open(dpb_engine* e, double flops, int kind, int M, int N, int K, int Z, int gather) {
  if (!e->profiling) return -1;
  dpb_engine::Prof p;
  p.flops = flops; p.big = kind; p.M = M; p.N = N; p.K = K; p.Z = Z; p.gather = gather;
  if (hipEventCreate(&p.a) != hipSuccess) return -1;
  if (hipEventCreate(&p.b) != hipSuccess) { (void)hipEventDestroy(p.a); return -1; }
  (void)hipEventRecord(p.a, e->stream);
  e->prof.push_back(p);
  return (int)e->prof.size() - 1;
}
void prof_close(dpb_engine* e, int idx) {
  if (idx >= 0) (void)hipEventRecord(e->prof[idx].b, e->stream);
}

int g_geglu_fwd = getenv("DPB_GEGLU_FWD") ? atoi(getenv("DPB_GEGLU_FWD")) : 1;
int g_cross_primal = getenv("DPB_CROSS_PRIMAL") ? atoi(getenv("DPB_CROSS_PRIMAL")) : 1;
int gemm(dpb_engine* e, GemmArgs a, bool can_defer = false) {
  if (e->pend.on)
    if (int r = flush_pending(e)) return r;
  gemm_prep(e, a);
  GemmArgs* pend = (can_defer && g_lazy_reduce) ? &e->pend.a : nullptr;
  const double kk = (double)a.K + (a.A2 ? a.K2 : 0);
  e->flops += 2.0 * a.M * (double)a.N * kk * a.Z1 * a.Z2;
  e->gbytes += ((double)a.M * a.K + (double)a.N * a.K + (double)a.M * a.N) * a.Z1 * a.Z2 * e->es;
  int nl = 1;
  if (!e->profiling) { const int r = launch_gemm(e->dtype, a, e->stream, &nl, pend); e->n_launch += nl; e->pend.on = pend && pend->splitk > 1; return r; }
  int kind;
  { GemmArgs az = a; az.zeros = e->ws + e->zeros; const int dm = gemm_uses_dma(e->dtype, a); kind = gemm_uses_halo(e->dtype, az) ? 5 : dm == 540 ? 12 : dm == 530 ? 11 : dm == 518 ? 6 : dm >= 512 ? 4 : (dm == 128 || dm == 130 || dm == 132 || dm == 256) ? 2 : dm ? 3 : gemm_uses_big_tile(e->dtype, a); }
  const int pi = prof_open(e, 2.0 * a.M * (double)a.N * kk * a.Z1 * a.Z2, kind, a.M, a.N, a.K, a.Z1 * a.Z2, a.gather);
  int r = launch_gemm(e->dtype, a, e->stream, &nl, pend);
  e->n_launch += nl;
  e->pend.on = pend && pend->splitk > 1;
  prof_close(e, pi);
  return r;
}

int conv_fwd(dpb_engine* e, const Op& op, int mode, int n) {
  const dpb_op_desc& d = op.d;
  const int H = d.ip[0], W = d.ip[1], Cin = d.ip[2], Ho = d.ip[3], Wo = d.ip[4], Cout = d.ip[5], KS = d.ip[6];
  const Buf& bi = e->bufs[d.in0];
  const Buf& bo = e->bufs[d.out];
  if (mode == 1 && !e->bact[d.in0]) {
    e->n_launch++;
    return launch_axpy(e->dtype, e->T(d.res), e->T(d.out), (long)n * bo.rows * bo.C, 0, e->stream);
  }
  GemmArgs g;
  const bool shared_out = bo.kind == DPB_BUF_SHARED;
  const int ns = shared_out ? 1 : n;
  g.A = mode == 0 ? e->P(d.in0) : e->T(d.in0);
  g.B = d.w[0];
  g.C = mode == 0 ? e->P(d.out) : e->T(d.out);
  g.N = Cout;
  g.K = KS * KS * Cin;
  g.ldb = g.K;
  g.ldc = bo.C;
  g.lda = bi.C;
  g.gather = d.ip[9];
  if (g.gather == GATHER_NONE) {
    g.M = ns * bi.rows;
  } else {
    g.M = ns * Ho * Wo;
    g.H = H; g.W = W; g.Cin = Cin; g.Ho = Ho; g.Wo = Wo; g.KS = KS; g.stride = d.ip[7]; g.pad = d.ip[8];
  }
  if (mode == 0) {
    g.bias = (const float*)d.w[2];
    if (d.rowbias >= 0) {
      g.rowbias = e->P(d.rowbias) + (size_t)d.ip[10] * e->es;
      g.rows_per_sample = bo.rows;
      g.rowbias_div = 1 << 30;
    }
  }
  if (d.res >= 0 && (mode == 0 || e->bact[d.res])) {
    g.R = mode == 0 ? e->P(d.res) : e->T(d.res);
    g.ldr = e->bufs[d.res].C;
  }
  if (mode == 1 && op.ln_next >= 0 && g_ln_fuse) {
    const dpb_op_desc& ld = e->ops[op.ln_next].d;
    GemmArgs f = g;
    f.epi = EPI_LN_TAN; f.C2 = e->T(ld.out); f.ln_x = e->P(ld.in0); f.ln_gamma = (const float*)ld.w[0]; f.ln_eps = ld.fp[0];
    f.rows_per_sample = bo.rows; f.epi_kps = n / e->cur_batch;
    gemm_prep(e, f);
    if (gemm_epi_supported(e->dtype, f)) {
      e->skip[op.ln_next] = 1;
      return gemm(e, f);
    }
  }
  if (mode == 1 && op.geglu_next >= 0) {
    const dpb_op_desc& gd = e->ops[op.geglu_next].d;
    GemmArgs f = g;
    f.epi = EPI_GEGLU_TAN; f.hprim = e->P(d.out); f.epi_kps = n / e->cur_batch; f.rows_per_sample = bo.rows;
    f.C = e->T(gd.out); f.ldc = e->bufs[gd.out].C;
    gemm_prep(e, f);
    if (gemm_epi_supported(e->dtype, f)) {
      e->skip[op.geglu_next] = 1;
      return gemm(e, f);
    }
  }
  if (mode == 0 && e->fwd_only && op.geglu_next >= 0 && g_geglu_fwd && !shared_out && d.out != e->cur_tap && d.out != e->fwd_seed) {
    const dpb_op_desc& gd = e->ops[op.geglu_next].d;
    GemmArgs f = g;
    f.epi = EPI_GEGLU_FWD; f.C = e->P(gd.out); f.ldc = e->bufs[gd.out].C; f.rowbias = nullptr; f.R = nullptr;
    gemm_prep(e, f);
    GemmArgs probe = g; gemm_prep(e, probe);
    if (!g.rowbias && !g.R && gemm_epi_supported(e->dtype, f) && gemm_plan(e->dtype, probe).splitk == 1) {
      e->skip[op.geglu_next] = 1;
      return gemm(e, f);
    }
  }
  return gemm(e, g, mode == 1 && !shared_out);
}

int conv_adj(dpb_engine* e, const Op& op, int n) {
  const dpb_op_desc& d = op.d;
  const int H = d.ip[0], W = d.ip[1], Cin = d.ip[2], Ho = d.ip[3], Wo = d.ip[4], KS = d.ip[6];
  const Buf& bi = e->bufs[d.in0];
  const Buf& bo = e->bufs[d.out];
  const int Cout = bo.C;
  if (e->bact[d.in0]) {
    if (!d.w[1]) return fail("conv op has no transposed weight (w[1]) but its adjoint is needed");
    GemmArgs g;
    g.A = e->G(d.out);
    g.lda = bo.C;
    g.B = d.w[1];
    g.N = Cin;
    g.K = KS * KS * Cout;
    g.ldb = g.K;
    g.ldc = bi.C;
    const int gather = d.ip[9];
    if (gather == GATHER_NONE && op.ln_prev >= 0 && g_ln_fuse && e->uses[d.in0] == 1 && d.in0 != e->src && (g.K <= g_ln_kmax || (g_ln_fuse & 2))) {
      const dpb_op_desc& ld = e->ops[op.ln_prev].d;
      GemmArgs f = g;
      f.M = n * bi.rows;
      f.epi = EPI_LN_ADJ; f.C = e->G(ld.in0); f.ldc = e->bufs[ld.in0].C; f.accumulate = e->ginit[ld.in0];
      f.ln_x = e->P(ld.in0); f.ln_gamma = (const float*)ld.w[0]; f.ln_eps = ld.fp[0];
      f.rows_per_sample = bi.rows; f.epi_kps = n / e->cur_batch;
      gemm_prep(e, f);
      if (gemm_epi_supported(e->dtype, f)) {
        if (int r = gemm(e, f)) return r;
        e->ginit[ld.in0] = 1;
        goto residual;
      }
    }
    if (gather == GATHER_NONE && op.geglu_prev >= 0 && d.in0 != e->src) {
      const dpb_op_desc& gd = e->ops[op.geglu_prev].d;
      GemmArgs f = g;
      f.M = n * bi.rows;
      f.epi = EPI_GEGLU_ADJ; f.hprim = e->P(gd.in0); f.epi_kps = n / e->cur_batch; f.rows_per_sample = bi.rows;
      f.C = e->G(gd.in0); f.ldc = e->bufs[gd.in0].C; f.accumulate = e->ginit[gd.in0];
      gemm_prep(e, f);
      if (gemm_epi_supported(e->dtype, f)) {
        if (int r = gemm(e, f)) return r;
        e->ginit[gd.in0] = 1;
        goto residual;
      }
    }
    const bool lone = e->uses[d.in0] == 1 && d.in0 != e->src;
    if (gather == GATHER_NONE) {
      g.M = n * bi.rows;
      g.C = e->G(d.in0);
      g.accumulate = e->ginit[d.in0];
      if (int r = gemm(e, g, lone)) return r;
    } else if (gather == GATHER_CONV) {
      g.gather = GATHER_CONVT;
      g.M = n * H * W;
      g.H = Ho; g.W = Wo; g.Cin = Cout; g.Ho = H; g.Wo = W; g.KS = KS; g.stride = d.ip[7]; g.pad = d.ip[8];
      g.C = e->G(d.in0);
      g.accumulate = e->ginit[d.in0];
      if (int r = gemm(e, g, lone)) return r;
    } else {
      g.gather = GATHER_CONVT;
      g.M = n * Ho * Wo;
      g.H = Ho; g.W = Wo; g.Cin = Cout; g.Ho = Ho; g.Wo = Wo; g.KS = KS; g.stride = 1; g.pad = 1;
      g.C = e->ws + e->convtmp;
      if (int r = gemm(e, g)) return r;
      e->n_launch++;
      if (int r = launch_pool2x2_sum(e->dtype, e->ws + e->convtmp, e->G(d.in0), n, H, W, bi.C, e->ginit[d.in0], e->stream)) return r;
    }
    e->ginit[d.in0] = 1;
  }
residual:
  if (d.res >= 0 && e->bact[d.res]) {
    Buf& br = e->bufs[d.res];
    if (!e->ginit[d.res] && br.rows == bo.rows && br.C == bo.C && br.kind == bo.kind) {
      std::swap(br.g_off, e->bufs[d.out].g_off);
    } else {
      e->n_launch++;
      if (int r = launch_axpy(e->dtype, e->G(d.out), e->G(d.res), (long)n * bo.rows * bo.C, e->ginit[d.res], e->stream)) return r;
    }
    e->ginit[d.res] = 1;
  }
  return 0;
}

void take_pending(dpb_engine* e, SlabSrc& src, const void* d, bool store) {
  if (!e->pend.on || e->pend.a.C != d) return;
  const GemmArgs& g = e->pend.a;
  src.slab = g.slab; src.splitk = g.splitk; src.MN = (long)g.M * g.N; src.N = g.N;
  src.R = g.R; src.ldr = g.ldr;
  src.store = store ? g.C : nullptr;
  e->pend.on = false;
}

bool consumes_pending(dpb_engine* e, const Op& op, int mode) {
  if (mode == MODE_PRIMAL || (op.d.kind != DPB_OP_GROUPNORM && op.d.kind != DPB_OP_LAYERNORM)) return false;
  const void* d = mode == MODE_TANGENT ? (const void*)e->T(op.d.in0) : (const void*)e->G(op.d.out);
  if (d != e->pend.a.C) return false;
  const Buf& bi = e->bufs[op.d.in0];
  if (e->pend.a.N != bi.C) return false;
  if (op.d.kind == DPB_OP_GROUPNORM) {
    GNArgs a; a.HW = bi.rows; a.C = bi.C; a.G = op.d.ip[0]; a.NT = 1;
    return groupnorm_launches(e->dtype, mode, a) == 1;
  }
  return true;
}

int gn_run(dpb_engine* e, const Op& op, int mode, int n) {
  const dpb_op_desc& d = op.d;
  const Buf& bi = e->bufs[d.in0];
  GNArgs a;
  a.x = e->P(d.in0);
  a.gamma = (const float*)d.w[0];
  a.beta = (const float*)d.w[1];
  a.pstats = (double*)(e->ws + op.pstats);
  a.tstats = (double*)(e->ws + op.tstats);
  a.part = (float*)(e->ws + e->gnpart); a.part_bytes = e->gnpart_bytes; a.ticket = (int*)(e->ws + e->gnticket);
  a.det = gn_deterministic();
  a.HW = bi.rows; a.C = bi.C; a.G = d.ip[0]; a.silu = d.ip[1]; a.eps = d.fp[0];
  a.Bp = e->cur_batch;
  if (mode == MODE_PRIMAL) {
    a.Bp = n;
    a.y = e->P(d.out);
  } else {
    a.NT = n;
    a.kps = n / e->cur_batch;
    if (mode == MODE_TANGENT) {
      a.d = e->T(d.in0);
      a.y = e->T(d.out);
    } else {
      a.d = e->G(d.out);
      a.y = e->G(d.in0);
      a.accumulate = e->ginit[d.in0];
      e->ginit[d.in0] = 1;
    }
    take_pending(e, a.src, a.d, mode == MODE_TANGENT && (e->uses[d.in0] > 1 || d.in0 == e->cur_tap));
  }
  e->n_launch += groupnorm_launches(e->dtype, mode, a);
  return launch_groupnorm(e->dtype, mode, a, e->stream);
}

int ln_run(dpb_engine* e, const Op& op, int mode, int n) {
  const dpb_op_desc& d = op.d;
  const Buf& bi = e->bufs[d.in0];
  LNArgs a;
  a.x = e->P(d.in0);
  a.gamma = (const float*)d.w[0];
  a.beta = (const float*)d.w[1];
  a.rows_per_sample = bi.rows; a.C = bi.C; a.eps = d.fp[0];
  a.Bp = e->cur_batch;
  if (mode == MODE_PRIMAL) {
    a.Bp = n;
    a.y = e->P(d.out);
  } else {
    a.NT = n;
    a.kps = n / e->cur_batch;
    if (mode == MODE_TANGENT) {
      a.d = e->T(d.in0);
      a.y = e->T(d.out);
    } else {
      a.d = e->G(d.out);
      a.y = e->G(d.in0);
      a.accumulate = e->ginit[d.in0];
      e->ginit[d.in0] = 1;
    }
    take_pending(e, a.src, a.d, mode == MODE_TANGENT && (e->uses[d.in0] > 1 || d.in0 == e->cur_tap));
  }
  e->n_launch++;
  return launch_layernorm(e->dtype, mode, a, e->stream);
}

int geglu_run(dpb_engine* e, const Op& op, int mode, int n) {
  const dpb_op_desc& d = op.d;
  const Buf& bi = e->bufs[d.in0];
  GegluArgs a;
  a.h = e->P(d.in0);
  a.rows_per_sample = bi.rows; a.F = bi.C / 2; a.il = d.ip[1];
  a.Bp = e->cur_batch;
  if (mode == MODE_PRIMAL) {
    a.Bp = n;
    a.y = e->P(d.out);
    a.stash = !e->fwd_only;
  } else {
    a.NT = n;
    a.kps = n / e->cur_batch;
    if (mode == MODE_TANGENT) {
      a.d = e->T(d.in0);
      a.y = e->T(d.out);
    } else {
      a.d = e->G(d.out);
      a.y = e->G(d.in0);
      a.accumulate = e->ginit[d.in0];
      e->ginit[d.in0] = 1;
    }
  }
  e->n_launch++;
  return launch_geglu(e->dtype, mode, a, e->stream);
}

int concat_run(dpb_engine* e, const Op& op, int mode, int n) {
  const dpb_op_desc& d = op.d;
  const Buf& b0 = e->bufs[d.in0];
  const Buf& b1 = e->bufs[d.in1];
  const Buf& bo = e->bufs[d.out];
  const long rows = (long)n * bo.rows;
  e->n_launch += 2;
  if (mode == MODE_ADJOINT) {
    if (e->bact[d.in0]) {
      if (int r = launch_copy_cols(e->dtype, e->G(d.out), bo.C, 0, e->G(d.in0), b0.C, 0, rows, b0.C, e->ginit[d.in0], e->stream)) return r;
      e->ginit[d.in0] = 1;
    }
    if (e->bact[d.in1]) {
      if (int r = launch_copy_cols(e->dtype, e->G(d.out), bo.C, b0.C, e->G(d.in1), b1.C, 0, rows, b1.C, e->ginit[d.in1], e->stream)) return r;
      e->ginit[d.in1] = 1;
    }
    return 0;
  }
  if (mode == MODE_TANGENT && (!e->bact[d.in0] || !e->bact[d.in1])) {
    char* o = e->T(d.out);
    if (int r = e->bact[d.in0] ? launch_copy_cols(e->dtype, e->T(d.in0), b0.C, 0, o, bo.C, 0, rows, b0.C, 0, e->stream)
                               : launch_zero_cols(e->dtype, o, bo.C, 0, rows, b0.C, e->stream)) return r;
    return e->bact[d.in1] ? launch_copy_cols(e->dtype, e->T(d.in1), b1.C, 0, o, bo.C, b0.C, rows, b1.C, 0, e->stream)
                          : launch_zero_cols(e->dtype, o, bo.C, b0.C, rows, b1.C, e->stream);
  }
  char* o = mode == MODE_PRIMAL ? e->P(d.out) : e->T(d.out);
  const char* i0 = mode == MODE_PRIMAL ? e->P(d.in0) : e->T(d.in0);
  const char* i1 = mode == MODE_PRIMAL ? e->P(d.in1) : e->T(d.in1);
  if (int r = launch_copy_cols(e->dtype, i0, b0.C, 0, o, bo.C, 0, rows, b0.C, 0, e->stream)) return r;
  return launch_copy_cols(e->dtype, i1, b1.C, 0, o, bo.C, b0.C, rows, b1.C, 0, e->stream);
}

struct AttnPtrs {
  const char *Q, *K, *V; char* O;
  int ldq, ldk, ldv, ldo;
};
static AttnPtrs attn_ptrs(dpb_engine* e, const dpb_op_desc& d, const AttnPlan& p, int which ) {
  AttnPtrs a;
  auto base = [&](int b) { return which == 0 ? e->P(b) : which == 1 ? e->T(b) : e->G(b); };
  a.ldq = e->bufs[d.in0].C; a.ldk = e->bufs[d.in1].C; a.ldv = e->bufs[d.in2].C; a.ldo = e->bufs[d.out].C;
  a.Q = base(d.in0) + (size_t)p.oq * e->es;
  a.K = (which == 0 || !p.kv_const) ? base(d.in1) + (size_t)p.ok * e->es : nullptr;
  a.V = (which == 0 || !p.kv_const) ? base(d.in2) + (size_t)p.ov * e->es : nullptr;
  a.O = base(d.out);
  return a;
}

static void fill_fused(dpb_engine* e, const AttnPlan& p, const AttnPtrs& x, FusedAttnArgs& f, int kps, float scale);

int attn_primal(dpb_engine* e, const Op& op, int B) {
  const dpb_op_desc& d = op.d;
  const AttnPlan& p = e->plans[op.attn];
  const int H = p.heads;
  const float scale = 1.f / sqrtf((float)p.d);
  char* ws = e->ws;
  const AttnPtrs x = attn_ptrs(e, d, p, 0);
  if (p.fused) {
    e->n_launch += 1;
    FusedAttnArgs f;
    fill_fused(e, p, x, f, 1, scale);
    const double fl = 2.0 * p.Lq * (double)p.Lk * p.d * 2 * B * H;
    e->flops += fl;
    const int pi = prof_open(e, fl, 7, p.Lq, p.Lk, p.d, B * H, 0);
    const int r = launch_attn_fwd_fused(f, B, x.O, (float*)(ws + p.stats), e->stream);
    prof_close(e, pi);
    return r;
  }
  if (p.cross && g_cross_primal) {
    CrossAttnArgs f;
    f.Q = x.Q; f.K = x.K; f.V = x.V; f.BT = nullptr; f.X = nullptr; f.Y = x.O;
    f.L = p.Lq; f.Lk = p.Lk; f.Lkp = p.Lkp; f.C = x.ldq; f.Ck = x.ldk; f.Cx = x.ldq; f.Cy = x.ldo;
    f.H = H; f.d = p.d; f.kps = 1; f.primal = 1; f.scale = scale; f.fl = e->dtype == DT_F16;
    e->n_launch++;
    const double fl = 2.0 * p.Lq * (double)p.Lk * p.d * 2 * B * H;
    e->flops += fl;
    const int pi = prof_open(e, fl, 10, p.Lq, p.Lk, p.d, B * H, 2);
    const int r = launch_attn_cross(f, B, e->stream);
    prof_close(e, pi);
    if (r || e->fwd_only) return r;
    e->n_launch += 2;
    if (int r2 = launch_transpose(e->dtype, x.V, ws + p.VT, B, H, (long)p.Lk * x.ldv, p.d, p.Lk, p.d, x.ldv, p.Lkp, (long)p.d * p.Lkp, e->stream)) return r2;
    return launch_transpose(e->dtype, x.K, ws + p.KT, B, H, (long)p.Lk * x.ldk, p.d, p.Lk, p.d, x.ldk, p.Lkp, (long)p.d * p.Lkp, e->stream);
  }
  GemmArgs g;
  g.A = x.Q; g.lda = x.ldq; g.sA1 = (long)p.Lq * x.ldq; g.sA2 = p.d;
  g.B = x.K; g.ldb = x.ldk; g.sB1 = (long)p.Lk * x.ldk; g.sB2 = p.d;
  g.C = ws + p.P; g.ldc = p.Lkp; g.sC1 = (long)H * p.Lq * p.Lkp; g.sC2 = (long)p.Lq * p.Lkp;
  g.M = p.Lq; g.N = p.Lk; g.K = p.d; g.Z1 = B; g.Z2 = H; g.alpha = scale;
  if (int r = gemm(e, g)) return r;
  e->n_launch += 3;
  if (p.fused) {
    e->n_launch++;
    if (int r = launch_row_stats(e->dtype == DT_F16, ws + p.P, (float*)(ws + p.stats), (long)B * H * p.Lq, p.Lk, p.Lkp, e->stream)) return r;
  }
  if (int r = launch_softmax_fwd(e->dtype, ws + p.P, (long)B * H, p.Lq, p.Lk, p.Lkp, p.causal, e->stream)) return r;
  if (int r = launch_transpose(e->dtype, x.V, ws + p.VT, B, H, (long)p.Lk * x.ldv, p.d, p.Lk, p.d, x.ldv, p.Lkp, (long)p.d * p.Lkp, e->stream)) return r;
  if (e->fwd_only) e->n_launch--;
  else if (int r = launch_transpose(e->dtype, x.K, ws + p.KT, B, H, (long)p.Lk * x.ldk, p.d, p.Lk, p.d, x.ldk, p.Lkp, (long)p.d * p.Lkp, e->stream)) return r;
  GemmArgs o;
  o.A = ws + p.P; o.lda = p.Lkp; o.sA1 = (long)H * p.Lq * p.Lkp; o.sA2 = (long)p.Lq * p.Lkp;
  o.B = ws + p.VT; o.ldb = p.Lkp; o.sB1 = (long)H * p.d * p.Lkp; o.sB2 = (long)p.d * p.Lkp;
  o.C = x.O; o.ldc = x.ldo; o.sC1 = (long)p.Lq * x.ldo; o.sC2 = p.d;
  o.M = p.Lq; o.N = p.d; o.K = p.Lkp; o.Z1 = B; o.Z2 = H;
  if (int r = gemm(e, o)) return r;
  if (!p.kv_const && !e->fwd_only) {
    e->n_launch += 2;
    if (!p.fused)
      if (int r = launch_transpose(e->dtype, ws + p.P, ws + p.PT, B * H, 1, (long)p.Lq * p.Lkp, 0, p.Lq, p.Lk, p.Lkp, p.Lqp, (long)p.Lk * p.Lqp, e->stream)) return r;
    if (int r = launch_transpose(e->dtype, x.Q, ws + p.QT, B, H, (long)p.Lq * x.ldq, p.d, p.Lq, p.d, x.ldq, p.Lqp, (long)p.d * p.Lqp, e->stream)) return r;
  }
  return 0;
}

static void fill_fused(dpb_engine* e, const AttnPlan& p, const AttnPtrs& x, FusedAttnArgs& f, int kps, float scale) {
  char* ws = e->ws;
  f.Q = x.Q; f.K = x.K; f.V = x.V; f.O = x.O; f.VT = ws + p.VT; f.KT = ws + p.KT; f.QT = ws + p.QT;
  f.stats = (const float*)(ws + p.stats);
  f.L = p.Lq; f.C = x.ldq; f.Co = x.ldo; f.H = p.heads; f.d = p.d; f.kps = kps; f.scale = scale; f.fl = e->dtype == DT_F16;
}

int attn_tangent(dpb_engine* e, const Op& op, int nt) {
  const dpb_op_desc& d = op.d;
  const AttnPlan& p = e->plans[op.attn];
  const int H = p.heads, kps = nt / e->cur_batch;
  const float scale = 1.f / sqrtf((float)p.d);
  char* ws = e->ws;
  char* S1 = ws + e->S1;
  const AttnPtrs x = attn_ptrs(e, d, p, 0), t = attn_ptrs(e, d, p, 1);
  if (p.fused) {
    e->n_launch += 1;
    FusedAttnArgs f;
    fill_fused(e, p, x, f, kps, scale);
    f.dQ = t.Q; f.dK = t.K; f.dV = t.V; f.dO = t.O;
    const double fl = 2.0 * p.Lq * (double)p.Lk * p.d * 5 * nt * H;
    e->flops += fl;
    const int pi = prof_open(e, fl, 8, p.Lq, p.Lk, p.d, nt * H, attn_jvp_block_waves(p.d, p.Lq, nt * H));
    const int r = launch_attn_jvp_fused(f, nt, e->stream);
    prof_close(e, pi);
    return r;
  }
  if (p.cross) {
    CrossAttnArgs f;
    f.Q = x.Q; f.K = x.K; f.V = x.V; f.BT = ws + p.VT; f.X = t.Q; f.Y = t.O;
    f.L = p.Lq; f.Lk = p.Lk; f.Lkp = p.Lkp; f.C = x.ldq; f.Ck = x.ldk; f.Cx = t.ldq; f.Cy = t.ldo;
    f.H = H; f.d = p.d; f.kps = kps; f.adjoint = 0; f.scale = scale; f.fl = e->dtype == DT_F16;
    e->n_launch++;
    const double fl = 2.0 * p.Lq * (double)p.Lk * p.d * 2 * nt * H;
    e->flops += fl;
    const int pi = prof_open(e, fl, 10, p.Lq, p.Lk, p.d, nt * H, 0);
    const int r = launch_attn_cross(f, nt, e->stream);
    prof_close(e, pi);
    return r;
  }
  GemmArgs g;
  g.A = t.Q; g.lda = t.ldq; g.sA1 = (long)p.Lq * t.ldq; g.sA2 = p.d;
  g.B = x.K; g.ldb = x.ldk; g.sB1 = (long)p.Lk * x.ldk; g.sB2 = p.d; g.divB = kps;
  g.C = S1; g.ldc = p.Lkp; g.sC1 = (long)H * p.Lq * p.Lkp; g.sC2 = (long)p.Lq * p.Lkp;
  g.M = p.Lq; g.N = p.Lk; g.K = p.d; g.Z1 = nt; g.Z2 = H; g.alpha = scale;
  if (!p.kv_const) {
    g.A2 = x.Q; g.lda2 = x.ldq; g.sA21 = (long)p.Lq * x.ldq; g.sA22 = p.d; g.divA2 = kps;
    g.B2 = t.K; g.ldb2 = t.ldk; g.sB21 = (long)p.Lk * t.ldk; g.sB22 = p.d; g.divB2 = 1;
    g.K2 = p.d;
  }
  if (int r = gemm(e, g)) return r;
  e->n_launch++;
  if (int r = launch_softmax_jvp(e->dtype, ws + p.P, S1, nullptr, (long)nt * H, H, kps, p.Lq, p.Lk, p.Lkp, e->stream)) return r;
  GemmArgs o;
  o.A = S1; o.lda = p.Lkp; o.sA1 = (long)H * p.Lq * p.Lkp; o.sA2 = (long)p.Lq * p.Lkp;
  o.B = ws + p.VT; o.ldb = p.Lkp; o.sB1 = (long)H * p.d * p.Lkp; o.sB2 = (long)p.d * p.Lkp; o.divB = kps;
  o.C = t.O; o.ldc = t.ldo; o.sC1 = (long)p.Lq * t.ldo; o.sC2 = p.d;
  o.M = p.Lq; o.N = p.d; o.K = p.Lkp; o.Z1 = nt; o.Z2 = H;
  if (!p.kv_const) {
    char* T1 = ws + e->T1;
    e->n_launch++;
    if (int r = launch_transpose(e->dtype, t.V, T1, nt, H, (long)p.Lk * t.ldv, p.d, p.Lk, p.d, t.ldv, p.Lkp, (long)p.d * p.Lkp, e->stream)) return r;
    o.A2 = ws + p.P; o.lda2 = p.Lkp; o.sA21 = (long)H * p.Lq * p.Lkp; o.sA22 = (long)p.Lq * p.Lkp; o.divA2 = kps;
    o.B2 = T1; o.ldb2 = p.Lkp; o.sB21 = (long)H * p.d * p.Lkp; o.sB22 = (long)p.d * p.Lkp; o.divB2 = 1;
    o.K2 = p.Lkp;
  }
  return gemm(e, o);
}

int attn_adjoint(dpb_engine* e, const Op& op, int nt) {
  const dpb_op_desc& d = op.d;
  const AttnPlan& p = e->plans[op.attn];
  const int H = p.heads, kps = nt / e->cur_batch;
  const float scale = 1.f / sqrtf((float)p.d);
  char* ws = e->ws;
  char* S1 = ws + e->S1;
  float* Dv = (float*)(ws + e->Dv);
  const AttnPtrs x = attn_ptrs(e, d, p, 0), c = attn_ptrs(e, d, p, 2);
  const char* gO = c.O;
  const bool kq = d.in1 == d.in0 && p.ok == p.oq, vq = d.in2 == d.in0 && p.ov == p.oq, vk = d.in2 == d.in1 && p.ov == p.ok;
  const int accQ = e->ginit[d.in0], accK = p.kv_const ? 0 : e->ginit[d.in1] || kq || (!p.fused && vk),
            accV = p.kv_const ? 0 : e->ginit[d.in2] || vq;
  if (p.fused) {
    e->n_launch += attn_adj_launches(p.d, p.Lq, kps, nt);
    FusedAttnArgs f;
    fill_fused(e, p, x, f, kps, scale);
    f.gO = gO; f.gQ = (void*)c.Q; f.gK = (void*)c.K; f.gV = (void*)c.V; f.Drow = Dv;
    f.accQ = accQ; f.accK = accK; f.accV = accV;
    const double fl = 2.0 * p.Lq * (double)p.Lk * p.d * 7 * nt * H;
    e->flops += fl;
    const int pi = prof_open(e, fl, 9, p.Lq, p.Lk, p.d, nt * H, attn_adj_route_bits(p.d, p.Lq, kps, nt));
    const int r = launch_attn_adj_fused(f, nt, e->stream);
    prof_close(e, pi);
    if (r) return r;
    e->ginit[d.in0] = e->ginit[d.in1] = e->ginit[d.in2] = 1;
    return 0;
  }
  if (p.cross) {
    CrossAttnArgs f;
    f.Q = x.Q; f.K = x.K; f.V = x.V; f.BT = ws + p.KT; f.X = gO; f.Y = (void*)c.Q;
    f.L = p.Lq; f.Lk = p.Lk; f.Lkp = p.Lkp; f.C = x.ldq; f.Ck = x.ldk; f.Cx = c.ldo; f.Cy = c.ldq;
    f.H = H; f.d = p.d; f.kps = kps; f.adjoint = 1; f.accumulate = accQ; f.scale = scale; f.fl = e->dtype == DT_F16;
    e->n_launch++;
    const double fl = 2.0 * p.Lq * (double)p.Lk * p.d * 2 * nt * H;
    e->flops += fl;
    const int pi = prof_open(e, fl, 10, p.Lq, p.Lk, p.d, nt * H, 1);
    const int r = launch_attn_cross(f, nt, e->stream);
    prof_close(e, pi);
    if (r) return r;
    e->ginit[d.in0] = 1;
    return 0;
  }
  GemmArgs g;
  g.A = gO; g.lda = c.ldo; g.sA1 = (long)p.Lq * c.ldo; g.sA2 = p.d;
  g.B = x.V; g.ldb = x.ldv; g.sB1 = (long)p.Lk * x.ldv; g.sB2 = p.d; g.divB = kps;
  g.C = S1; g.ldc = p.Lkp; g.sC1 = (long)H * p.Lq * p.Lkp; g.sC2 = (long)p.Lq * p.Lkp;
  g.M = p.Lq; g.N = p.Lk; g.K = p.d; g.Z1 = nt; g.Z2 = H;
  if (int r = gemm(e, g)) return r;
  e->n_launch++;
  if (int r = launch_softmax_jvp(e->dtype, ws + p.P, S1, p.kv_const ? nullptr : Dv, (long)nt * H, H, kps, p.Lq, p.Lk, p.Lkp, e->stream)) return r;
  GemmArgs q;
  q.A = S1; q.lda = p.Lkp; q.sA1 = (long)H * p.Lq * p.Lkp; q.sA2 = (long)p.Lq * p.Lkp;
  q.B = ws + p.KT; q.ldb = p.Lkp; q.sB1 = (long)H * p.d * p.Lkp; q.sB2 = (long)p.d * p.Lkp; q.divB = kps;
  q.C = (void*)c.Q; q.ldc = c.ldq; q.sC1 = (long)p.Lq * c.ldq; q.sC2 = p.d;
  q.M = p.Lq; q.N = p.d; q.K = p.Lkp; q.Z1 = nt; q.Z2 = H; q.alpha = scale;
  q.accumulate = accQ;
  if (int r = gemm(e, q)) return r;
  e->ginit[d.in0] = 1;
  if (p.kv_const) return 0;
  char* T1 = ws + e->T1;
  char* S2 = ws + e->S2;
  e->n_launch += 2;
  if (int r = launch_transpose(e->dtype, gO, T1, nt, H, (long)p.Lq * c.ldo, p.d, p.Lq, p.d, c.ldo, p.Lqp, (long)p.d * p.Lqp, e->stream)) return r;
  GemmArgs v;
  v.A = ws + p.PT; v.lda = p.Lqp; v.sA1 = (long)H * p.Lk * p.Lqp; v.sA2 = (long)p.Lk * p.Lqp; v.divA = kps;
  v.B = T1; v.ldb = p.Lqp; v.sB1 = (long)H * p.d * p.Lqp; v.sB2 = (long)p.d * p.Lqp;
  v.C = (void*)c.V; v.ldc = c.ldv; v.sC1 = (long)p.Lk * c.ldv; v.sC2 = p.d;
  v.M = p.Lk; v.N = p.d; v.K = p.Lqp; v.Z1 = nt; v.Z2 = H;
  v.accumulate = accV;
  if (int r = gemm(e, v)) return r;
  GemmArgs t;
  t.A = x.V; t.lda = x.ldv; t.sA1 = (long)p.Lk * x.ldv; t.sA2 = p.d; t.divA = kps;
  t.B = gO; t.ldb = c.ldo; t.sB1 = (long)p.Lq * c.ldo; t.sB2 = p.d;
  t.C = S2; t.ldc = p.Lqp; t.sC1 = (long)H * p.Lk * p.Lqp; t.sC2 = (long)p.Lk * p.Lqp;
  t.M = p.Lk; t.N = p.Lq; t.K = p.d; t.Z1 = nt; t.Z2 = H;
  if (int r = gemm(e, t)) return r;
  if (int r = launch_softmax_adjT(e->dtype, ws + p.PT, S2, Dv, (long)nt * H, H, kps, p.Lk, p.Lq, p.Lqp, e->stream)) return r;
  GemmArgs k;
  k.A = S2; k.lda = p.Lqp; k.sA1 = (long)H * p.Lk * p.Lqp; k.sA2 = (long)p.Lk * p.Lqp;
  k.B = ws + p.QT; k.ldb = p.Lqp; k.sB1 = (long)H * p.d * p.Lqp; k.sB2 = (long)p.d * p.Lqp; k.divB = kps;
  k.C = (void*)c.K; k.ldc = c.ldk; k.sC1 = (long)p.Lk * c.ldk; k.sC2 = p.d;
  k.M = p.Lk; k.N = p.d; k.K = p.Lqp; k.Z1 = nt; k.Z2 = H; k.alpha = scale;
  k.accumulate = accK;
  if (int r = gemm(e, k)) return r;
  e->ginit[d.in1] = e->ginit[d.in2] = 1;
  return 0;
}

int run_op(dpb_engine* e, const Op& op, int mode, int n) {
  if (e->pend.on && !consumes_pending(e, op, mode))
    if (int r = flush_pending(e)) return r;
  switch (op.d.kind) {
    case DPB_OP_CONV: return mode == MODE_ADJOINT ? conv_adj(e, op, n) : conv_fwd(e, op, mode, n);
    case DPB_OP_GROUPNORM: return gn_run(e, op, mode, n);
    case DPB_OP_LAYERNORM: return ln_run(e, op, mode, n);
    case DPB_OP_GEGLU: return geglu_run(e, op, mode, n);
    case DPB_OP_CONCAT: return concat_run(e, op, mode, n);
    case DPB_OP_ATTENTION:
      return mode == MODE_PRIMAL ? attn_primal(e, op, n) : mode == MODE_TANGENT ? attn_tangent(e, op, n) : attn_adjoint(e, op, n);
    case DPB_OP_SILU: {
      if (mode != MODE_PRIMAL) return fail("SILU / quick-GELU ops are primal only (time-embedding path, text encoder)");
      const Buf& b = e->bufs[op.d.in0];
      e->n_launch++;
      if (op.d.ip[0] == 2)
        return launch_gelu(e->dtype, e->P(op.d.in0), e->P(op.d.out), (long)(b.kind == DPB_BUF_SHARED ? 1 : n) * b.rows * b.C, e->stream);
      if (op.d.ip[0] == 1)
        return launch_quick_gelu(e->dtype, e->P(op.d.in0), e->P(op.d.out), (long)(b.kind == DPB_BUF_SHARED ? 1 : n) * b.rows * b.C, e->stream);
      return launch_silu(e->dtype, e->P(op.d.in0), e->P(op.d.out), (long)(b.kind == DPB_BUF_SHARED ? 1 : n) * b.rows * b.C, e->stream);
    }
  }
  return fail("unknown op kind %d", op.d.kind);
}

int check_tap(dpb_engine* e, int tap, int nt) {
  if (!e->ws) return fail("workspace not set (dpb_engine_set_workspace)");
  if (tap < 0 || tap >= (int)e->bufs.size() || e->producer[tap] < 0) return fail("invalid tap buffer %d", tap);
  if (e->bufs[tap].is_const) return fail("tap buffer %d does not depend on x", tap);
  if (e->cur_batch <= 0) return fail("dpb_primal must run before jvp/vjp");
  if (nt <= 0 || nt > e->maxT || nt % e->cur_batch) return fail("nt=%d must be a positive multiple of batch=%d and <= max_tangents=%d", nt, e->cur_batch, e->maxT);
  return 0;
}

int set_seed(dpb_engine* e, int src) {
  const int nb = (int)e->bufs.size(), no = (int)e->ops.size();
  std::vector<char>& a = e->act_cache[src];
  if (a.empty()) {
    std::vector<char> f(nb + no, 0);
    if (src == e->x_buf) {
      for (int b = 0; b < nb; ++b) f[b] = !e->bufs[b].is_const;
      for (int i = 0; i < no; ++i) f[nb + i] = !e->ops[i].is_const;
    } else {
      f[src] = 1;
      for (int i = e->producer[src] + 1; i < no; ++i) {
        const Op& op = e->ops[i];
        const dpb_op_desc& d = op.d;
        bool on = f[d.in0];
        if (d.kind == DPB_OP_ATTENTION || d.kind == DPB_OP_CONCAT) on = on || f[d.in1];
        if (d.kind == DPB_OP_ATTENTION) on = on || f[d.in2];
        if (d.kind == DPB_OP_CONV && d.res >= 0) on = on || f[d.res];
        if (d.kind == DPB_OP_SILU && on) return fail("op %d (SILU / GELU, primal only) depends on source buffer %d", i, src);
        if (on && d.kind == DPB_OP_ATTENTION) {
          const AttnPlan& p = e->plans[op.attn];
          if (!f[d.in0] || f[d.in1] != f[d.in2] || (bool)f[d.in1] == p.kv_const)
            return fail("attention op %d: q, k, v depend on source buffer %d differently than on x (unsupported)", i, src);
        }
        f[nb + i] = on;
        if (on) f[d.out] = 1;
      }
    }
    a.swap(f);
  }
  e->src = src;
  e->bact = a.data();
  e->oact = a.data() + nb;
  return 0;
}

int seed_channels(const dpb_engine* e, int src) { return src == e->x_buf ? e->x_channels : e->bufs[src].Cv; }

int check_pair(dpb_engine* e, int src, int dst, int nt) {
  if (int r = check_tap(e, dst, nt)) return r;
  if (src != e->x_buf) {
    if (src < 0 || src >= (int)e->bufs.size() || e->producer[src] < 0 || e->bufs[src].kind != DPB_BUF_ACT) return fail("invalid source buffer %d", src);
    if (e->bufs[src].is_const) return fail("source buffer %d does not depend on x", src);
    if (e->producer[dst] > e->primal_last)
      return fail("no primal state up to dst buffer %d (produced by op %d, the primal pass covers ops 0..%d): run dpb_primal with upto_buf = dst or later",
                  dst, e->producer[dst], e->primal_last);
  }
  if (int r = set_seed(e, src)) return r;
  if (dst == src || !e->bact[dst]) return fail("dst buffer %d is not downstream of source buffer %d", dst, src);
  return 0;
}

}

extern "C" {

const char* dpb_last_error(void) { return g_err; }
int dpb_abi_version(void) { return DPB_ABI_VERSION; }

int dpb_engine_create(const dpb_net_desc* net, dpb_engine** out) {
  if (!net || !out) return fail("null argument");
  if (net->dtype != DPB_F32 && net->dtype != DPB_BF16 && net->dtype != DPB_F16) return fail("bad dtype %d", net->dtype);
  if (net->max_batch < 1 || net->max_tangents < 1) return fail("max_batch/max_tangents must be >= 1");
  dpb_engine* e = new dpb_engine();
  e->dtype = net->dtype;
  e->es = net->dtype == DPB_F32 ? 4 : 2;
  e->maxB = net->max_batch;
  e->maxT = net->max_tangents;
  e->x_buf = net->x_buf; e->x_channels = net->x_channels; e->temb_buf = net->temb_buf; e->temb_dim = net->temb_dim;
  e->temb_flip = net->temb_flip_sin_to_cos; e->temb_hm1 = net->temb_half_minus_one; e->ctx_buf = net->ctx_buf;
  const int nb = net->n_buffers;
  e->bufs.resize(nb);
  e->producer.assign(nb, -1);
  auto bad = [&](const char* m, int i) { fail("op %d: %s", i, m); delete e; return -1; };
  for (int i = 0; i < nb; ++i) {
    e->bufs[i].rows = net->buffers[i].rows;
    e->bufs[i].C = net->buffers[i].channels;
    e->bufs[i].kind = net->buffers[i].kind;
    e->bufs[i].Cv = net->buffers[i].valid_channels > 0 ? net->buffers[i].valid_channels : net->buffers[i].channels;
    if (e->bufs[i].rows < 1 || e->bufs[i].C < 8 || e->bufs[i].C % 8) { fail("buffer %d: rows=%d channels=%d (channels must be a multiple of 8)", i, e->bufs[i].rows, e->bufs[i].C); delete e; return -1; }
  }
  if (net->x_buf < 0 || net->x_buf >= nb) { fail("bad x_buf"); delete e; return -1; }
  e->bufs[net->x_buf].is_const = false;
  auto okb = [&](int b) { return b >= 0 && b < nb; };
  for (int i = 0; i < net->n_ops; ++i) {
    Op op;
    op.d = net->ops[i];
    const dpb_op_desc& d = op.d;
    if (!okb(d.in0) || !okb(d.out)) return bad("bad buffer id", i);
    bool c = e->bufs[d.in0].is_const;
    if (d.kind == DPB_OP_ATTENTION || d.kind == DPB_OP_CONCAT) {
      if (!okb(d.in1)) return bad("bad in1", i);
      c = c && e->bufs[d.in1].is_const;
    }
    if (d.kind == DPB_OP_ATTENTION) {
      if (!okb(d.in2)) return bad("bad in2", i);
      c = c && e->bufs[d.in2].is_const;
      AttnPlan p;
      p.heads = d.ip[0];
      p.oq = d.ip[1]; p.ok = d.ip[2]; p.ov = d.ip[3];
      p.causal = d.ip[4] != 0;
      const int Cattn = e->bufs[d.out].C;
      if (p.heads < 1 || Cattn % p.heads) return bad("channels not divisible by heads", i);
      p.d = Cattn / p.heads;
      if (p.oq % 8 || p.ok % 8 || p.ov % 8 || p.oq + Cattn > e->bufs[d.in0].C || p.ok + Cattn > e->bufs[d.in1].C || p.ov + Cattn > e->bufs[d.in2].C)
        return bad("bad q/k/v column window", i);
      auto part = [&](int b0, int o0, int b1, int o1) { return b0 == b1 && o0 != o1 && o0 < o1 + Cattn && o1 < o0 + Cattn; };
      if (part(d.in0, p.oq, d.in1, p.ok) || part(d.in0, p.oq, d.in2, p.ov) || part(d.in1, p.ok, d.in2, p.ov))
        return bad("q/k/v windows of one buffer must coincide or be disjoint", i);
      if (p.d % 8) return bad("head dim must be a multiple of 8", i);
      p.Lq = e->bufs[d.in0].rows; p.Lk = e->bufs[d.in1].rows;
      p.Lqp = round8(p.Lq); p.Lkp = round8(p.Lk);
      if (e->bufs[d.in1].is_const != e->bufs[d.in2].is_const) return bad("k and v must both depend on x or both not", i);
      if (e->bufs[d.in0].is_const) return bad("attention query independent of x is unsupported", i);
      p.kv_const = e->bufs[d.in1].is_const;
      op.attn = (int)e->plans.size();
      e->plans.push_back(p);
    }
    if (d.kind == DPB_OP_CONV) {
      if (d.res >= 0) { if (!okb(d.res)) return bad("bad res", i); c = c && e->bufs[d.res].is_const; }
      if (d.rowbias >= 0 && (!okb(d.rowbias) || e->bufs[d.rowbias].kind != DPB_BUF_SHARED)) return bad("rowbias must be a SHARED buffer", i);
      if (d.rowbias >= 0 && (d.ip[10] < 0 || d.ip[10] % 8 || d.ip[10] + round8(d.ip[5]) > e->bufs[d.rowbias].C)) return bad("bad rowbias column window", i);
      if (!d.w[0]) return bad("missing weight", i);
      if (d.ip[2] != e->bufs[d.in0].C || e->bufs[d.out].C != round8(d.ip[5])) return bad("conv channel mismatch", i);
    }
    op.is_const = c;
    e->bufs[d.out].is_const = c;
    if (e->producer[d.out] >= 0) return bad("buffer written twice (tape must be SSA)", i);
    e->producer[d.out] = i;
    e->ops.push_back(op);
  }
  {
    std::vector<int> uses(nb, 0), user(nb, -1);
    for (size_t i = 0; i < e->ops.size(); ++i) {
      const dpb_op_desc& d = e->ops[i].d;
      for (int b : {d.in0, d.in1, d.in2, d.res}) if (b >= 0 && b < nb) { uses[b]++; user[b] = (int)i; }
    }
    e->uses = uses;
    for (size_t j = 0; j < e->ops.size(); ++j) {
      const dpb_op_desc& d = e->ops[j].d;
      if (d.kind != DPB_OP_LAYERNORM || e->ops[j].is_const || e->dtype == DT_F32 || e->bufs[d.in0].C != 320 || e->bufs[d.in0].kind != DPB_BUF_ACT) continue;
      const int pi = e->producer[d.in0];
      if (pi >= 0 && e->ops[pi].d.kind == DPB_OP_CONV && e->ops[pi].d.ip[9] == DPB_GATHER_NONE && !e->ops[pi].is_const) e->ops[pi].ln_next = (int)j;
      if (uses[d.out] == 1) {
        const int ci = user[d.out];
        const dpb_op_desc& cd = e->ops[ci].d;
        if (cd.kind == DPB_OP_CONV && cd.ip[9] == DPB_GATHER_NONE && cd.in0 == d.out && cd.w[1]) e->ops[ci].ln_prev = (int)j;
      }
    }
    for (size_t j = 0; j < e->ops.size(); ++j) {
      const dpb_op_desc& d = e->ops[j].d;
      if (d.kind == DPB_OP_GEGLU && uses[d.in0] != 1) return bad("the input buffer of a GEGLU op must have no other consumer (the primal pass overwrites it in place)", (int)j);
      if (d.kind != DPB_OP_GEGLU || d.ip[1] != 64 || e->ops[j].is_const || getenv("DPB_NO_GEGLU_FUSE")) continue;
      const int pi = e->producer[d.in0];
      if (pi >= 0 && uses[d.in0] == 1) {
        const dpb_op_desc& pd = e->ops[pi].d;
        if (pd.kind == DPB_OP_CONV && pd.ip[9] == DPB_GATHER_NONE && pd.res < 0 && e->bufs[d.in0].kind == DPB_BUF_ACT) e->ops[pi].geglu_next = (int)j;
      }
      if (uses[d.out] == 1) {
        const int ci = user[d.out];
        const dpb_op_desc& cd = e->ops[ci].d;
        if (cd.kind == DPB_OP_CONV && cd.ip[9] == DPB_GATHER_NONE && cd.in0 == d.out) e->ops[ci].geglu_prev = (int)j;
      }
    }
    e->skip.assign(e->ops.size(), 0);
  }
  size_t off = 0;
  auto take = [&](size_t bytes) { size_t o = off; off = align_up(off + bytes); return o; };
  const size_t es = e->es;
  for (auto& b : e->bufs) {
    size_t n = b.kind == DPB_BUF_SHARED ? 1 : e->maxB;
    b.p_off = take(n * b.rows * (size_t)b.C * es);
  }
  for (auto& b : e->bufs)
    if (!b.is_const) b.t_off = take((size_t)e->maxT * b.rows * b.C * es);
  for (auto& b : e->bufs)
    if (!b.is_const) b.g_off = b.g_off0 = take((size_t)e->maxT * b.rows * b.C * es);
  size_t s1 = 0, s2 = 0, t1 = 0, dv = 0, ctmp = 0, maxrc = 0;
  for (auto& op : e->ops) {
    const dpb_op_desc& d = op.d;
    if (d.kind == DPB_OP_ATTENTION) {
      AttnPlan& p = e->plans[op.attn];
      const size_t H = p.heads;
      p.fused = !p.causal && fused_attention_supported(e->dtype, p.d, p.Lq, p.kv_const) && !getenv("DPB_NO_FUSED_ATTN") &&
                p.Lq >= (getenv("DPB_FUSED_ATTN_MIN_L") ? atoi(getenv("DPB_FUSED_ATTN_MIN_L")) : 64) &&
                e->bufs[d.in0].C == e->bufs[d.in1].C && e->bufs[d.in0].C == e->bufs[d.in2].C;
      p.cross = !p.causal && cross_attention_supported(e->dtype, p.d, p.Lq, p.Lk, p.kv_const) && !getenv("DPB_NO_CROSS_ATTN") &&
                e->bufs[d.in1].C == e->bufs[d.in2].C;
      if (!p.fused) p.P = take((size_t)e->maxB * H * p.Lq * p.Lkp * es);
      p.VT = take((size_t)e->maxB * H * p.d * p.Lkp * es);
      p.KT = take((size_t)e->maxB * H * p.d * p.Lkp * es);
      if (!p.fused) s1 = std::max(s1, (size_t)e->maxT * H * p.Lq * p.Lkp * es);
      size_t lmax = std::max(p.Lqp, p.Lkp);
      t1 = std::max(t1, (size_t)e->maxT * H * p.d * lmax * es);
      if (p.fused) p.stats = take((size_t)e->maxB * H * p.Lq * 2 * sizeof(float));
      if (!p.kv_const) {
        if (!p.fused) p.PT = take((size_t)e->maxB * H * p.Lk * p.Lqp * es);
        p.QT = take((size_t)e->maxB * H * p.d * p.Lqp * es);
        if (!p.fused) s2 = std::max(s2, (size_t)e->maxT * H * p.Lk * p.Lqp * es);
        dv = std::max(dv, (size_t)e->maxT * H * p.Lq * sizeof(float));
      }
    } else if (d.kind == DPB_OP_GROUPNORM) {
      op.pstats = e->pstats_bytes;
      e->pstats_bytes += (size_t)e->maxB * d.ip[0] * 2 * sizeof(double);
      if (!op.is_const) {
        op.tstats = e->tstats_bytes;
        e->tstats_bytes += (size_t)e->maxT * d.ip[0] * 2 * sizeof(double);
      }
    } else if (d.kind == DPB_OP_CONV && d.ip[9] == DPB_GATHER_UPCONV && !op.is_const) {
      ctmp = std::max(ctmp, (size_t)e->maxT * d.ip[3] * d.ip[4] * e->bufs[d.in0].C * es);
    }
  }
  for (auto& b : e->bufs) maxrc = std::max(maxrc, (size_t)b.rows * b.C);
  e->pstats_off = take(e->pstats_bytes);
  e->tstats_off = take(e->tstats_bytes);
  {
    size_t need = 0;
    for (auto& op : e->ops)
      if (op.d.kind == DPB_OP_GROUPNORM) {
        const size_t hw = e->bufs[op.d.in0].rows, nmax = (size_t)std::max(e->maxB, e->maxT);
        const size_t blocks = std::max<size_t>(nmax * ((hw + 7) / 8), 1);
        need = std::max(need, std::min<size_t>(blocks, std::max<size_t>(1024, nmax * ((hw + 63) / 64))) * 2 * op.d.ip[0] * sizeof(float));
      }
    e->gnpart_bytes = need;
    e->gnpart = take(need);
    e->gnticket = take(sizeof(int) * (size_t)std::max(e->maxB, e->maxT));
  }
  for (auto& op : e->ops)
    if (op.d.kind == DPB_OP_GROUPNORM) { op.pstats += e->pstats_off; op.tstats += e->tstats_off; }
  e->S1 = take(s1); e->S2 = take(s2); e->T1 = take(t1); e->Dv = take(dv); e->convtmp = take(ctmp);
  const size_t nio = (size_t)std::max(e->maxB, e->maxT) * maxrc * sizeof(float);
  e->io_in = take(nio);
  e->io_out = take(nio);
  e->orth_stride = align_up(orth_scratch_bytes(std::min(ORTH_MAX_RANK, std::max(56, e->maxT)), (long)e->bufs[e->x_buf].rows * e->x_channels));
  e->orth = take(e->orth_stride * (size_t)e->maxB);
  e->slab = take(e->slab_bytes);
  e->zeros = take(256);
  const size_t nx = (size_t)e->bufs[e->x_buf].rows * e->x_channels;
  e->pbW = take((size_t)e->maxT * nx * sizeof(float));
  e->ws_bytes = off;
  e->ginit.assign(nb, 0);
  e->act_cache.assign(nb, std::vector<char>());
  if (set_seed(e, e->x_buf)) { delete e; return -1; }
  *out = e;
  return 0;
}

void dpb_engine_destroy(dpb_engine* e) {
  if (e && e->gexec) (void)hipGraphExecDestroy(e->gexec);
  delete e;
}

int dpb_engine_set_stream(dpb_engine* e, void* s) {
  if (!e) return fail("null engine");
  e->stream = (hipStream_t)s;
  return 0;
}

size_t dpb_engine_workspace_bytes(const dpb_engine* e) { return e ? e->ws_bytes : 0; }

int dpb_engine_set_workspace(dpb_engine* e, void* ws, size_t bytes) {
  if (!e || !ws) return fail("null argument");
  if (bytes < e->ws_bytes) return fail("workspace too small: %zu < %zu", bytes, e->ws_bytes);
  if ((uintptr_t)ws % 256) return fail("workspace must be 256-byte aligned");
  e->ws = (char*)ws;
  e->cur_batch = 0;
  DPB_CHECK(hipMemsetAsync(ws, 0, e->ws_bytes, e->stream));
  return 0;
}

static int primal_pass(dpb_engine* e, const float* x, int batch, float t, const float* ctx, int upto_buf) {
  if (!e || !x) return fail("null argument");
  if (!e->ws) return fail("workspace not set (dpb_engine_set_workspace)");
  if (batch < 1 || batch > e->maxB) return fail("batch=%d outside [1,%d]", batch, e->maxB);
  if (upto_buf < 0 || upto_buf >= (int)e->bufs.size() || e->producer[upto_buf] < 0) return fail("invalid upto buffer %d", upto_buf);
  e->n_launch = 0; e->flops = 0; e->gbytes = 0;
  const Buf& bx = e->bufs[e->x_buf];
  e->n_launch++;
  if (int r = launch_nchw_to_nhwc(e->dtype, x, e->P(e->x_buf), batch, e->x_channels, bx.rows, bx.C, e->stream)) return r;
  if (e->ctx_buf >= 0) {
    if (!ctx) return fail("this network needs ctx (encoder_hidden_states)");
    const Buf& bc = e->bufs[e->ctx_buf];
    e->n_launch++;
    if (int r = launch_nchw_to_nhwc(e->dtype, ctx, e->P(e->ctx_buf), batch * bc.rows, bc.Cv, 1, bc.C, e->stream)) return r;
  }
  if (e->temb_buf >= 0) {
    const int dim = e->temb_dim, half = dim / 2;
    std::vector<float> emb(e->bufs[e->temb_buf].C, 0.f);
    for (int i = 0; i < half; ++i) {
      float f;
      if (e->temb_hm1) f = expf((float)i * (float)(-(log(10000.0) / (double)(half - 1))));
      else f = expf(((float)(-log(10000.0)) * (float)i) / (float)half);
      float ang = t * f;
      float s = sinf(ang), c = cosf(ang);
      if (e->temb_flip) { emb[i] = c; emb[half + i] = s; } else { emb[i] = s; emb[half + i] = c; }
    }
    float* stage = (float*)(e->ws + e->io_in);
    DPB_CHECK(hipMemcpyAsync(stage, emb.data(), emb.size() * sizeof(float), hipMemcpyHostToDevice, e->stream));
    DPB_CHECK(hipStreamSynchronize(e->stream));
    e->n_launch++;
    if (int r = launch_nchw_to_nhwc(e->dtype, stage, e->P(e->temb_buf), 1, (int)emb.size(), 1, (int)emb.size(), e->stream)) return r;
  }
  if (e->pstats_bytes && !gn_deterministic()) DPB_CHECK(hipMemsetAsync(e->ws + e->pstats_off, 0, e->pstats_bytes, e->stream));
  e->cur_batch = batch;
  e->cur_tap = upto_buf; e->pend.on = false;
  const int last = e->producer[upto_buf];
  const int seed_op = e->fwd_seed >= 0 ? e->producer[e->fwd_seed] : -1;
  e->primal_last = -1;
  std::fill(e->skip.begin(), e->skip.end(), 0);
  for (int i = 0; i <= last; ++i) {
    if (!e->skip[i])
      if (int r = run_op(e, e->ops[i], MODE_PRIMAL, batch)) return r;
    if (i == seed_op) {
      const Buf& bs = e->bufs[e->fwd_seed];
      e->n_launch++;
      if (int r = launch_nchw_to_nhwc(e->dtype, e->fwd_h, e->P(e->fwd_seed), batch, bs.Cv, bs.rows, bs.C, e->stream)) return r;
    }
  }
  if (!e->fwd_only) e->primal_last = last;
  return 0;
}

int dpb_primal(dpb_engine* e, const float* x, int batch, float t, const float* ctx, int upto_buf) {
  if (e) e->fwd_only = false;
  return primal_pass(e, x, batch, t, ctx, upto_buf);
}

int dpb_forward(dpb_engine* e, const float* x, int batch, float t, const float* ctx, int upto_buf, int channels, float* out) {
  if (!e || !out) return fail("null argument");
  e->fwd_only = true;
  int r = primal_pass(e, x, batch, t, ctx, upto_buf);
  e->fwd_only = false;
  if (!r) r = dpb_read_buffer(e, upto_buf, channels, out);
  e->cur_batch = 0;
  return r;
}

int dpb_forward_from(dpb_engine* e, const float* x, int batch, float t, const float* ctx, int src_buf, const float* h, int dst_buf, int channels,
                     float* out) {
  if (!e || !out || !h) return fail("null argument");
  const int nb = (int)e->bufs.size();
  if (src_buf < 0 || src_buf >= nb || e->producer[src_buf] < 0 || e->bufs[src_buf].kind != DPB_BUF_ACT || e->bufs[src_buf].is_const)
    return fail("invalid source buffer %d (an x-dependent activation produced by an op)", src_buf);
  if (dst_buf < 0 || dst_buf >= nb || e->producer[dst_buf] < 0) return fail("invalid dst buffer %d", dst_buf);
  const int prev = e->src;
  if (int r = set_seed(e, src_buf)) return r;
  const bool down = dst_buf != src_buf && e->bact[dst_buf];
  set_seed(e, prev);
  if (!down) return fail("dst buffer %d is not downstream of source buffer %d", dst_buf, src_buf);
  e->fwd_seed = src_buf; e->fwd_h = h;
  const int r = dpb_forward(e, x, batch, t, ctx, dst_buf, channels, out);
  e->fwd_seed = -1; e->fwd_h = nullptr;
  return r;
}

int dpb_read_buffer(dpb_engine* e, int buf, int channels, float* out) {
  if (!e || !out) return fail("null argument");
  if (buf < 0 || buf >= (int)e->bufs.size()) return fail("bad buffer %d", buf);
  const Buf& b = e->bufs[buf];
  if (channels < 1 || channels > b.C) return fail("bad channel count");
  int n = b.kind == DPB_BUF_SHARED ? 1 : e->cur_batch;
  if (n < 1) return fail("no primal state to read (dpb_forward invalidates it; run dpb_primal first)");
  return launch_nhwc_to_nchw(e->dtype, e->P(buf), out, n, channels, b.rows, b.C, e->stream);
}

static int jvp_pass(dpb_engine* e, int src, int tap, const float* V, int nt, float* U) {
  if (!e || !V) return fail("null argument");
  if (int r = check_pair(e, src, tap, nt)) return r;
  e->n_launch = 0; e->flops = 0; e->gbytes = 0;
  const Buf& bx = e->bufs[src];
  e->n_launch++;
  if (int r = launch_nchw_to_nhwc(e->dtype, V, e->T(src), nt, seed_channels(e, src), bx.rows, bx.C, e->stream)) return r;
  if (e->tstats_bytes && !gn_deterministic()) DPB_CHECK(hipMemsetAsync(e->ws + e->tstats_off, 0, e->tstats_bytes, e->stream));
  const int last = e->producer[tap];
  std::fill(e->skip.begin(), e->skip.end(), 0);
  e->cur_tap = tap; e->pend.on = false;
  for (int i = e->producer[src] + 1; i <= last; ++i) {
    if (!e->oact[i] || e->skip[i]) continue;
    if (int r = run_op(e, e->ops[i], MODE_TANGENT, nt)) return r;
  }
  if (int r = flush_pending(e)) return r;
  if (!U) return 0;
  const Buf& bt = e->bufs[tap];
  e->n_launch++;
  return launch_nhwc_to_nchw(e->dtype, e->T(tap), U, nt, bt.Cv, bt.rows, bt.C, e->stream);
}

int dpb_jvp(dpb_engine* e, int tap, const float* V, int nt, float* U) {
  if (!U) return fail("null argument");
  return jvp_pass(e, e ? e->x_buf : -1, tap, V, nt, U);
}

int dpb_jvp_between(dpb_engine* e, int src_buf, int dst_buf, const float* V, int nt, float* U) {
  if (!e || !U) return fail("null argument");
  return jvp_pass(e, src_buf, dst_buf, V, nt, U);
}

static int vjp_pass(dpb_engine* e, int src, int tap, const float* U, int nt, float* W) {
  if (!e || !W) return fail("null argument");
  if (int r = check_pair(e, src, tap, nt)) return r;
  e->n_launch = 0; e->flops = 0; e->gbytes = 0;
  const Buf& bt = e->bufs[tap];
  std::fill(e->ginit.begin(), e->ginit.end(), 0);
  for (auto& b : e->bufs) b.g_off = b.g_off0;
  if (U) {
    e->n_launch++;
    if (int r = launch_nchw_to_nhwc(e->dtype, U, e->G(tap), nt, bt.Cv, bt.rows, bt.C, e->stream)) return r;
  } else {
    e->bufs[tap].g_off = e->bufs[tap].t_off;
  }
  e->ginit[tap] = 1;
  if (e->tstats_bytes && !gn_deterministic()) DPB_CHECK(hipMemsetAsync(e->ws + e->tstats_off, 0, e->tstats_bytes, e->stream));
  e->cur_tap = tap; e->pend.on = false;
  for (int i = e->producer[tap]; i > e->producer[src]; --i) {
    const Op& op = e->ops[i];
    if (!e->oact[i] || !e->ginit[op.d.out]) continue;
    if (int r = run_op(e, op, MODE_ADJOINT, nt)) return r;
  }
  if (int r = flush_pending(e)) return r;
  if (!e->ginit[src]) {
    for (auto& b : e->bufs) b.g_off = b.g_off0;
    return src == e->x_buf ? fail("tap buffer %d is not connected to x", tap) : fail("dst buffer %d is not connected to source buffer %d", tap, src);
  }
  const Buf& bx = e->bufs[src];
  e->n_launch++;
  const int r = launch_nhwc_to_nchw(e->dtype, e->G(src), W, nt, seed_channels(e, src), bx.rows, bx.C, e->stream);
  for (auto& b : e->bufs) b.g_off = b.g_off0;
  return r;
}

int dpb_vjp(dpb_engine* e, int tap, const float* U, int nt, float* W) {
  if (!U) return fail("null argument");
  return vjp_pass(e, e ? e->x_buf : -1, tap, U, nt, W);
}

int dpb_vjp_between(dpb_engine* e, int src_buf, int dst_buf, const float* U, int nt, float* W) {
  if (!e || !U) return fail("null argument");
  return vjp_pass(e, src_buf, dst_buf, U, nt, W);
}

int dpb_orth(const float* W, const float* Vprev, float* V, float* s, float* conv, void* scratch, int k, int64_t N, void* stream) {
  if (!W || !Vprev || !V || !s || !conv || !scratch) return fail("null argument");
  OrthArgs a;
  a.W = W; a.Vprev = Vprev; a.V = V; a.s = s; a.conv = conv; a.scratch = (double*)scratch; a.k = k; a.N = N;
  a.scratch_bytes = orth_scratch_bytes(k, N);
  return launch_orth(a, (hipStream_t)stream);
}

int dpb_orth_checked(const float* W, const float* Vprev, float* V, float* s, float* conv, void* scratch, size_t scratch_bytes, int k, int64_t N,
                     void* stream) {
  if (!W || !Vprev || !V || !s || !conv || !scratch) return fail("null argument");
  if (k < 1 || k > ORTH_MAX_RANK || N < 1) return fail("dpb_orth: k=%d outside [1,%d] or N=%lld < 1", k, ORTH_MAX_RANK, (long long)N);
  const size_t need = orth_scratch_bytes(k, N);
  if (scratch_bytes < need) return fail("dpb_orth: scratch of %zu bytes, dpb_orth_scratch_bytes(%d, %lld) = %zu", scratch_bytes, k, (long long)N, need);
  OrthArgs a;
  a.W = W; a.Vprev = Vprev; a.V = V; a.s = s; a.conv = conv; a.scratch = (double*)scratch; a.k = k; a.N = N;
  a.scratch_bytes = scratch_bytes;
  return launch_orth(a, (hipStream_t)stream);
}

size_t dpb_orth_scratch_bytes(int k, int64_t N) { return (k < 1 || k > ORTH_MAX_RANK || N < 1) ? 0 : orth_scratch_bytes(k, N); }

size_t dpb_pca_scratch_bytes(int q, int64_t N, int64_t D) { return pca_scratch_bytes(q, N, D); }

int dpb_pca_lowrank(const float* H, int64_t N, int64_t D, const float* R, int q, int niter, float* u, float* s, void* scratch,
                    size_t scratch_bytes, void* stream) {
  if (!H || !R || !u || !s || (!scratch && scratch_bytes)) return fail("dpb_pca_lowrank: null argument");
  return launch_pca_lowrank(H, N, D, R, q, niter, u, s, scratch, scratch_bytes, (hipStream_t)stream);
}

static int g_iter_alias = getenv("DPB_ITER_ALIAS") ? atoi(getenv("DPB_ITER_ALIAS")) : 1;
static int g_orth_batch = getenv("DPB_ORTH_BATCH") ? atoi(getenv("DPB_ORTH_BATCH")) : 1;
static int g_graph_iterate = 0;

static int iterate_pass(dpb_engine* e, int src, int tap, float* V, float* U, float* s, float* conv, int k, int n_iters, float* Wm, char* orth_scratch,
                        size_t orth_stride) {
  const int B = e->cur_batch;
  const int nt = k * B;
  const long N = (long)e->bufs[src].rows * seed_channels(e, src);
  long launches = 0; double fl = 0, gb = 0;
  const bool alias_ok = e->bufs[tap].Cv == e->bufs[tap].C && g_iter_alias;
  auto body = [&](bool want_u) -> int {
    const bool keep = alias_ok && !want_u;
    if (int r = jvp_pass(e, src, tap, V, nt, keep ? nullptr : U)) return r;
    launches += e->n_launch; fl += e->flops; gb += e->gbytes;
    if (int r = vjp_pass(e, src, tap, keep ? nullptr : U, nt, Wm)) return r;
    launches += e->n_launch; fl += e->flops; gb += e->gbytes;
    {
      OrthArgs a;
      a.W = Wm; a.Vprev = V; a.V = V; a.s = s; a.conv = conv; a.scratch = (double*)orth_scratch; a.k = k; a.N = N;
      a.scratch_bytes = orth_scratch_bytes(k, N);
      a.batch = B; a.stride_w = (long)k * N; a.stride_v = (long)k * N; a.stride_s = k; a.stride_conv = 2; a.scratch_stride = orth_stride;
      if (g_orth_batch) {
        if (int r = launch_orth(a, e->stream)) return r;
      } else {
        a.batch = 1;
        for (int b = 0; b < B; ++b) {
          if (int r = launch_orth(a, e->stream)) return r;
          a.W += a.stride_w; a.Vprev += a.stride_v; a.V += a.stride_v; a.s += k; a.conv += 2; a.scratch += orth_stride / sizeof(double);
        }
      }
    }
    launches += g_orth_batch ? 4 : 4 * B;
    return 0;
  };
  int it = 0;
  if (g_graph_iterate && !e->profiling && e->stream != 0 && src == e->x_buf) {
    const dpb_engine::GraphKey key{tap, k, B, V, U, s, conv};
    if (!e->gexec || !(key == e->gkey)) {
      if (int r = body(true)) return r;
      ++it;
      if (e->gexec) { (void)hipGraphExecDestroy(e->gexec); e->gexec = nullptr; }
      hipGraph_t g = nullptr;
      const long l0 = launches; const double f0 = fl, b0 = gb;
      DPB_CHECK(hipStreamBeginCapture(e->stream, hipStreamCaptureModeThreadLocal));
      const int r = body(true);
      const hipError_t ce = hipStreamEndCapture(e->stream, &g);
      e->g_launches = launches - l0; e->g_flops = fl - f0; e->g_bytes = gb - b0;
      launches = l0; fl = f0; gb = b0;
      if (r) { if (g) (void)hipGraphDestroy(g); return r; }
      DPB_CHECK(ce);
      DPB_CHECK(hipGraphInstantiate(&e->gexec, g, nullptr, nullptr, 0));
      (void)hipGraphDestroy(g);
      e->gkey = key;
    }
    for (; it < n_iters; ++it) {
      DPB_CHECK(hipGraphLaunch(e->gexec, e->stream));
      launches += e->g_launches; fl += e->g_flops; gb += e->g_bytes;
    }
  }
  for (; it < n_iters; ++it)
    if (int r = body(it == n_iters - 1)) return r;
  e->n_launch = launches; e->flops = fl; e->gbytes = gb;
  return 0;
}

int dpb_pullback_iterate(dpb_engine* e, int tap, float* V, float* U, float* s, float* conv, int k, int n_iters) {
  if (!e || !V || !U || !s || !conv) return fail("null argument");
  if (k < 1 || k > ORTH_MAX_RANK) return fail("pca_rank k=%d outside [1,%d]", k, ORTH_MAX_RANK);
  const int B = e->cur_batch;
  if (int r = check_tap(e, tap, k * (B > 0 ? B : 1))) return r;
  return iterate_pass(e, e->x_buf, tap, V, U, s, conv, k, n_iters, (float*)(e->ws + e->pbW), e->ws + e->orth, e->orth_stride);
}

static size_t between_scratch_bytes(const dpb_engine* e, int src, int k, int batch) {
  const long N = (long)e->bufs[src].rows * seed_channels(e, src);
  return align_up((size_t)batch * k * N * sizeof(float)) + (size_t)batch * align_up(orth_scratch_bytes(k, N));
}

size_t dpb_pullback_scratch_bytes(const dpb_engine* e, int src_buf, int k) {
  if (!e || k < 1 || k > ORTH_MAX_RANK || src_buf < 0 || src_buf >= (int)e->bufs.size() || e->bufs[src_buf].kind != DPB_BUF_ACT) return 0;
  return between_scratch_bytes(e, src_buf, k, e->maxB);
}

int dpb_pullback_iterate_between(dpb_engine* e, int src_buf, int dst_buf, float* V, float* U, float* s, float* conv, int k, int n_iters, void* scratch,
                                 size_t scratch_bytes) {
  if (!e || !V || !U || !s || !conv || !scratch) return fail("null argument");
  if (k < 1 || k > ORTH_MAX_RANK) return fail("pca_rank k=%d outside [1,%d]", k, ORTH_MAX_RANK);
  const int B = e->cur_batch;
  if (int r = check_pair(e, src_buf, dst_buf, k * (B > 0 ? B : 1))) return r;
  if ((uintptr_t)scratch % 256) return fail("scratch must be 256-byte aligned");
  const size_t need = between_scratch_bytes(e, src_buf, k, B);
  if (scratch_bytes < need) return fail("scratch of %zu bytes, the iteration needs %zu (dpb_pullback_scratch_bytes)", scratch_bytes, need);
  const long N = (long)e->bufs[src_buf].rows * seed_channels(e, src_buf);
  const size_t wbytes = align_up((size_t)B * k * N * sizeof(float));
  return iterate_pass(e, src_buf, dst_buf, V, U, s, conv, k, n_iters, (float*)scratch, (char*)scratch + wbytes, align_up(orth_scratch_bytes(k, N)));
}

int dpb_ddim_step(const float* x, const float* eps, float* out, float* x0, int64_t n, float a_t, float a_next, void* stream) {
  if (!x || !eps || !out) return fail("null argument");
  return launch_ddim_step(x, eps, out, x0, n, a_t, a_next, (hipStream_t)stream);
}

int dpb_embed_tokens(const int32_t* ids, const void* tok_table, const void* pos_table, int dtype, float* out, int batch, int tokens,
                     int channels, int vocab, void* stream) {
  if (!ids || !tok_table || !pos_table || !out) return fail("null argument");
  if (dtype != DPB_F32 && dtype != DPB_BF16 && dtype != DPB_F16) return fail("bad dtype %d", dtype);
  return launch_embed_tokens(dtype, ids, tok_table, pos_table, out, batch, tokens, channels, vocab, (hipStream_t)stream);
}

int dpb_lincomb(const float* x, const float* y, const float* z, float* out, int64_t n, float a, float b, float c, void* stream) {
  if (!x || !y || !out) return fail("null argument");
  return launch_lincomb(x, y, z, out, n, a, b, c, (hipStream_t)stream);
}

int dpb_engine_profile(dpb_engine* e, int enable) {
  if (!e) return fail("null engine");
  for (auto& p : e->prof) { (void)hipEventDestroy(p.a); (void)hipEventDestroy(p.b); }
  e->prof.clear();
  e->profiling = enable != 0;
  if (e->profiling) {
    hipEvent_t a, b;
    DPB_CHECK(hipEventCreate(&a));
    DPB_CHECK(hipEventCreate(&b));
    float best = 1e9f;
    for (int i = 0; i < 24; ++i) {
      DPB_CHECK(hipEventRecord(a, e->stream));
      if (int r = launch_axpy(e->dtype, e->ws + e->zeros, e->ws + e->zeros, 64, 0, e->stream)) return r;
      DPB_CHECK(hipEventRecord(b, e->stream));
      DPB_CHECK(hipEventSynchronize(b));
      float ms = 0;
      DPB_CHECK(hipEventElapsedTime(&ms, a, b));
      if (i >= 4) best = ms < best ? ms : best;
    }
    (void)hipEventDestroy(a);
    (void)hipEventDestroy(b);
    best -= 1.5e-3f;
    if (best < 0.f) best = 0.f;
    e->prof_overhead_ms = best < 1e8f ? best : 0.f;
  }
  return 0;
}

int dpb_engine_profile_dump(dpb_engine* e, const char* path) {
  if (!e || !path) return fail("null argument");
  DPB_CHECK(hipStreamSynchronize(e->stream));
  FILE* f = fopen(path, "w");
  if (!f) return fail("cannot open %s", path);
  fprintf(f, "idx,big,gather,M,N,K,Z,us,tflops,raw_us,bracket_overhead_us\n");
  int i = 0;
  for (auto& p : e->prof) {
    float raw = 0;
    (void)hipEventElapsedTime(&raw, p.a, p.b);
    const float ms = raw > e->prof_overhead_ms ? raw - e->prof_overhead_ms : 0.f;
    fprintf(f, "%d,%d,%d,%d,%d,%d,%d,%.2f,%.2f,%.2f,%.2f\n", i++, p.big, p.gather, p.M, p.N, p.K, p.Z, ms * 1e3, ms > 0 ? p.flops / (ms * 1e-3) / 1e12 : 0.0,
            raw * 1e3, e->prof_overhead_ms * 1e3);
  }
  fclose(f);
  return 0;
}

int dpb_engine_profile_read(dpb_engine* e, int big_tile, int64_t* count, double* total_ms, double* flops) {
  if (!e || !count || !total_ms || !flops) return fail("null argument");
  DPB_CHECK(hipStreamSynchronize(e->stream));
  *count = 0; *total_ms = 0; *flops = 0;
  const bool raw = big_tile >= 1000;
  if (raw) big_tile -= 1000;
  if (big_tile < 0 || big_tile > 12) return fail("dpb_engine_profile_read: kind must be 0..12 or 1000..1012");
  for (auto& p : e->prof) {
    if (p.big != big_tile) continue;
    float ms = 0;
    DPB_CHECK(hipEventElapsedTime(&ms, p.a, p.b));
    if (!raw) ms = ms > e->prof_overhead_ms ? ms - e->prof_overhead_ms : 0.f;
    *count += 1; *total_ms += ms; *flops += p.flops;
  }
  return 0;
}

int dpb_engine_profile_overhead(const dpb_engine* e, double* bracket_overhead_ms) {
  if (!e || !bracket_overhead_ms) return fail("null argument");
  *bracket_overhead_ms = e->prof_overhead_ms;
  return 0;
}

int dpb_debug_set(const char* key, int value) {
  static int tile = 0, splitk = 0, kch = 0;
  if (!key) return fail("null key");
  if (!strcmp(key, "gemm_tile")) tile = value;
  else if (!strcmp(key, "gemm_splitk")) splitk = value;
  else if (!strcmp(key, "gemm_kch")) kch = value;
  else if (!strcmp(key, "gemm_dma_auto")) { gemm_debug_dma_auto(value); return 0; }
  else if (!strcmp(key, "gemm_order")) { gemm_debug_order(value); return 0; }
  else if (!strcmp(key, "p8")) { gemm_debug_p8(value); return 0; }
  else if (!strcmp(key, "halo_loop")) { conv_halo_debug_loop(value); return 0; }
  else if (!strcmp(key, "wres")) { gemm_debug_wres(value); return 0; }
  else if (!strcmp(key, "gn_deterministic")) { gn_debug_deterministic(value); return 0; }
  else if (!strcmp(key, "graph_iterate")) { g_graph_iterate = value; return 0; }
  else if (!strcmp(key, "attn_shared")) { attn_debug_shared(value); return 0; }
  else if (!strcmp(key, "lazy_reduce")) { g_lazy_reduce = value; return 0; }
  else if (!strcmp(key, "ln_fuse")) { g_ln_fuse = value; return 0; }
  else if (!strcmp(key, "cross_primal")) { g_cross_primal = value; return 0; }
  else if (!strcmp(key, "geglu_fwd")) { g_geglu_fwd = value; return 0; }
  else if (!strcmp(key, "iter_alias")) { g_iter_alias = value; return 0; }
  else return fail("unknown debug key %s", key);
  gemm_debug_set(tile, splitk, kch);
  return 0;
}

int dpb_debug_gemm_plan(int dtype, int M, int N, int K, int conv_hw, int conv_cin, int epilogue, int64_t slab_bytes, int* kind, int* tile,
                        int* splitk) {
  if (!kind || !tile || !splitk) return fail("null argument");
  if (dtype != DPB_F32 && dtype != DPB_BF16 && dtype != DPB_F16) return fail("bad dtype %d", dtype);
  static char dummy[16];
  GemmArgs a;
  a.M = M; a.N = N; a.K = K; a.lda = K; a.ldb = K; a.ldc = N;
  a.zeros = dummy;
  if (slab_bytes > 0) { a.slab = (float*)dummy; a.slab_bytes = (size_t)slab_bytes; }
  a.epi = epilogue;
  if (conv_hw > 0) {
    if (conv_cin <= 0 || K != 9 * conv_cin || M % (conv_hw * conv_hw)) return fail("conv plan: K must be 9*cin and M whole images");
    a.gather = GATHER_CONV; a.H = a.W = a.Ho = a.Wo = conv_hw; a.Cin = conv_cin; a.KS = 3; a.stride = 1; a.pad = 1; a.lda = conv_cin;
  }
  const GemmPlan pl = gemm_plan(dtype, a);
  if (pl.kind < 0) return -1;
  *kind = pl.kind; *tile = pl.tile; *splitk = pl.splitk;
  return 0;
}

int dpb_engine_stats(const dpb_engine* e, int64_t* launches, double* gemm_flops, double* gemm_bytes) {
  if (!e) return fail("null engine");
  if (launches) *launches = e->n_launch;
  if (gemm_flops) *gemm_flops = e->flops;
  if (gemm_bytes) *gemm_bytes = e->gbytes;
  return 0;
}

}
```

### diffusion_pullback_amd/csrc/kernels.h

```cpp
#pragma once
#include <algorithm>

#include "common.h"

namespace dpb {

enum { GATHER_NONE = 0, GATHER_CONV = 1, GATHER_CONVT = 2, GATHER_UPCONV = 3 };
enum { EPI_PLAIN = 0, EPI_GEGLU_TAN = 1, EPI_GEGLU_ADJ = 2, EPI_LN_TAN = 3, EPI_LN_ADJ = 4, EPI_GEGLU_FWD = 5 };
struct GemmArgs {
  const void* A = nullptr; const void* B = nullptr; void* C = nullptr; const void* R = nullptr;
  const float* bias = nullptr;
  const void* rowbias = nullptr;
  int rows_per_sample = 1, rowbias_div = 1;
  int M = 0, N = 0, K = 0;
  int lda = 0, ldb = 0, ldc = 0, ldr = 0;
  int Z1 = 1, Z2 = 1;
  long sA1 = 0, sA2 = 0, sB1 = 0, sB2 = 0, sC1 = 0, sC2 = 0, sR1 = 0, sR2 = 0;
  int divA = 1, divB = 1;
  float alpha = 1.f;
  int accumulate = 0;
  int gather = GATHER_NONE;
  int H = 0, W = 0, Cin = 0, Ho = 0, Wo = 0, KS = 1, stride = 1, pad = 0;
  const void* A2 = nullptr; const void* B2 = nullptr;
  int K2 = 0, lda2 = 0, ldb2 = 0, divA2 = 1, divB2 = 1;
  long sA21 = 0, sA22 = 0, sB21 = 0, sB22 = 0;
  float* slab = nullptr; size_t slab_bytes = 0;
  const void* zeros = nullptr;
  int splitk = 1, vec_ok = 0;
  int epi = EPI_PLAIN, epi_kps = 1;
  const void* hprim = nullptr;
  const void* ln_x = nullptr; const float* ln_gamma = nullptr; float ln_eps = 1e-5f; void* C2 = nullptr;
  int fl = 0;
  int order = 0;
};
struct GemmPlan { int kind, tile, splitk; };
int launch_gemm(int dtype, const GemmArgs& a, hipStream_t st, int* launches = nullptr, GemmArgs* pending = nullptr);
int launch_gemm_reduce(int dtype, const GemmArgs& pending, hipStream_t st);
GemmPlan gemm_plan(int dtype, const GemmArgs& a);
int gemm_uses_big_tile(int dtype, const GemmArgs& a);
void gemm_debug_set(int tile, int splitk, int kch);
int gemm_kch(const GemmArgs& a);
int launch_gemm_dma(const GemmArgs& a, int tile, hipStream_t st);
int launch_gemm_ring64(const GemmArgs& a, int tile, hipStream_t st);
bool gemm_p8_fits32(const GemmArgs& a);
int launch_gemm_p8(const GemmArgs& a, int tile, hipStream_t st);
int conv_halo_supported(const GemmArgs& a);
int launch_conv_halo(const GemmArgs& a, hipStream_t st);
void conv_halo_debug_loop(int on);
int gemm_uses_halo(int dtype, const GemmArgs& a);
int gemm_epi_supported(int dtype, const GemmArgs& a);
int gemm_uses_dma(int dtype, const GemmArgs& a);
void gemm_debug_dma_auto(int on);
void gn_debug_deterministic(int on);
int gn_deterministic();
bool gemm_wres_supported(int dtype, const GemmArgs& a);
int launch_gemm_wres(const GemmArgs& a, hipStream_t st);
void gemm_debug_wres(int on);
void gemm_debug_p8(int on);
void gemm_debug_order(int o);
int gemm_pick_splitk_dma(const GemmArgs& a, int tile);

enum { MODE_PRIMAL = 0, MODE_TANGENT = 1, MODE_ADJOINT = 2 };
struct SlabSrc {
  const float* slab = nullptr; int splitk = 0; long MN = 0; int N = 0;
  const void* R = nullptr; int ldr = 0;
  void* store = nullptr;
};
struct GNArgs {
  const void* x = nullptr;
  const void* d = nullptr;
  void* y = nullptr;
  const float* gamma = nullptr; const float* beta = nullptr;
  double* pstats = nullptr;
  double* tstats = nullptr;
  float* part = nullptr;
  size_t part_bytes = 0;
  int* ticket = nullptr;
  int det = 1;
  int red = 0;
  int Bp = 1, NT = 0, kps = 1;
  int HW = 0, C = 0, G = 32;
  float eps = 1e-5f;
  int silu = 0, accumulate = 0;
  SlabSrc src;
};
int launch_groupnorm(int dtype, int mode, const GNArgs& a, hipStream_t st);
int groupnorm_launches(int dtype, int mode, const GNArgs& a);

struct LNArgs {
  const void* x = nullptr; const void* d = nullptr; void* y = nullptr;
  const float* gamma = nullptr; const float* beta = nullptr;
  int rows_per_sample = 0, Bp = 1, NT = 0, kps = 1, C = 0;
  float eps = 1e-5f;
  int accumulate = 0;
  SlabSrc src;
};
int launch_layernorm(int dtype, int mode, const LNArgs& a, hipStream_t st);

int launch_softmax_fwd(int dtype, void* S, long Z, int Lq, int Lk, int ld, int causal, hipStream_t st);
int launch_softmax_jvp(int dtype, const void* P, void* dS, float* D, long Z, int Z2, int kps, int Lq, int Lk, int ld,
                       hipStream_t st);
int launch_softmax_adjT(int dtype, const void* PT, void* gPT, const float* D, long Z, int Z2, int kps, int Lk, int Lq,
                        int ld, hipStream_t st);
int launch_transpose(int dtype, const void* in, void* out, int Z1, int Z2, long s1, long s2, int R, int Ccols, int ldin,
                     int ldout, long outZstride, hipStream_t st);

struct FusedAttnArgs {
  const void *Q = nullptr, *K = nullptr, *V = nullptr, *O = nullptr, *KT = nullptr, *VT = nullptr, *QT = nullptr;
  const float* stats = nullptr;
  float* Drow = nullptr;
  const void *dQ = nullptr, *dK = nullptr, *dV = nullptr, *dVT = nullptr; void* dO = nullptr;
  const void *gO = nullptr, *gOT = nullptr; void *gQ = nullptr, *gK = nullptr, *gV = nullptr;
  int accQ = 0, accK = 0, accV = 0;
  int fl = 0;
  int L = 0, C = 0, Co = 0, H = 0, d = 0, kps = 1;
  float scale = 1.f;
};
int fused_attention_supported(int dtype, int d, int L, int kv_const);
void attn_debug_shared(int bits);
struct CrossAttnArgs {
  const void *Q = nullptr, *K = nullptr, *V = nullptr;
  const void* BT = nullptr;
  const void* X = nullptr; void* Y = nullptr;
  int L = 0, Lk = 0, Lkp = 0, C = 0, Ck = 0, Cx = 0, Cy = 0, H = 0, d = 0, kps = 1, adjoint = 0, accumulate = 0, fl = 0;
  int primal = 0;
  float scale = 1.f;
};
int cross_attention_supported(int dtype, int d, int Lq, int Lk, int kv_const);
int launch_attn_cross(const CrossAttnArgs& f, int nt, hipStream_t st);
int launch_row_stats(int fl, const void* S, float* stats, long nrows, int Lk, int ld, hipStream_t st);
int attn_adj_route_bits(int d, int L, int kps, int nt);
int attn_adj_launches(int d, int L, int kps, int nt);
int attn_jvp_block_waves(int d, int L, int pairs);
int launch_attn_fwd_fused(const FusedAttnArgs& f, int batch, void* O, float* stats, hipStream_t st);
int launch_attn_jvp_fused(const FusedAttnArgs& f, int nt, hipStream_t st);
int launch_attn_adj_fused(const FusedAttnArgs& f, int nt, hipStream_t st);

struct GegluArgs {
  const void* h = nullptr;
  const void* d = nullptr;
  void* y = nullptr;
  int rows_per_sample = 0, Bp = 1, NT = 0, kps = 1, F = 0;
  int accumulate = 0;
  int stash = 1;
  int il = 0;
};
int launch_geglu(int dtype, int mode, const GegluArgs& a, hipStream_t st);
int launch_silu(int dtype, const void* x, void* y, long n, hipStream_t st);
int launch_quick_gelu(int dtype, const void* x, void* y, long n, hipStream_t st);
int launch_gelu(int dtype, const void* x, void* y, long n, hipStream_t st);
int launch_embed_tokens(int dtype, const int* ids, const void* tok, const void* pos, float* out, int batch, int L, int C, int vocab, hipStream_t st);
int launch_axpy(int dtype, const void* x, void* y, long n, int accumulate, hipStream_t st);
int launch_copy_cols(int dtype, const void* src, int lds, int cs0, void* dst, int ldd, int cd0, long rows, int ncols,
                     int accumulate, hipStream_t st);
int launch_zero_cols(int dtype, void* dst, int ldd, int cd0, long rows, int ncols, hipStream_t st);
int launch_nchw_to_nhwc(int dtype, const float* src, void* dst, int n, int C, int HW, int Cpad, hipStream_t st);
int launch_nhwc_to_nchw(int dtype, const void* src, float* dst, int n, int C, int HW, int Cpad, hipStream_t st);
int launch_pool2x2_sum(int dtype, const void* in, void* out, int n, int H, int W, int C, int accumulate, hipStream_t st);

struct OrthArgs {
  const float* W = nullptr;
  const float* Vprev = nullptr;
  float* V = nullptr;
  float* s = nullptr;
  float* conv = nullptr;
  double* scratch = nullptr;
  size_t scratch_bytes = 0;
  int k = 0; long N = 0;
  int batch = 1; long stride_w = 0, stride_v = 0, stride_s = 0, stride_conv = 0; size_t scratch_stride = 0;
};
constexpr int ORTH_MAX_RANK = 128;
int launch_orth(const OrthArgs& a, hipStream_t st);
size_t orth_scratch_bytes(int k, long N);

const char* pca_invalid(int q, long N, long D);
size_t pca_scratch_bytes(int q, long N, long D);
int launch_pca_lowrank(const float* H, long N, long D, const float* R, int q, int niter, float* u, float* s, void* scratch, size_t scratch_bytes,
                       hipStream_t st);

int launch_ddim_step(const float* x, const float* e, float* out, float* x0, long n, float a_t, float a_next, hipStream_t st);
int launch_lincomb(const float* x, const float* y, const float* z, float* out, long n, float a, float b, float c, hipStream_t st);

}
```

### diffusion_pullback_amd/lib.py

```python
from __future__ import annotations

import ctypes as C
import glob
import hashlib
import os
import subprocess

_HERE = os.path.dirname(os.path.abspath(__file__))
LIB_PATH = os.environ.get("DPB_LIB") or os.path.join(_HERE, "libdpb.so")
CSRC = os.path.join(_HERE, "csrc")
HIPCC = "/opt/rocm/bin/hipcc"
STAMP_PATH = LIB_PATH + ".srchash"

DPB_F32, DPB_BF16, DPB_F16 = 0, 1, 2


def dtype_code(dtype) -> int:
    import torch
    try:
        return {torch.float32: DPB_F32, torch.bfloat16: DPB_BF16, torch.float16: DPB_F16}[dtype]
    except KeyError:
        raise DpbError(f"engine dtype must be float32, bfloat16 or float16, got {dtype}") from None
OP_CONV, OP_GROUPNORM, OP_LAYERNORM, OP_ATTENTION, OP_GEGLU, OP_SILU, OP_CONCAT = 1, 2, 3, 4, 5, 6, 7
GATHER_NONE, GATHER_CONV, GATHER_UPCONV = 0, 1, 3
BUF_ACT, BUF_SHARED = 0, 1


class BufferDesc(C.Structure):
    _fields_ = [("rows", C.c_int32), ("channels", C.c_int32), ("kind", C.c_int32), ("valid_channels", C.c_int32)]


class OpDesc(C.Structure):
    _fields_ = [("kind", C.c_int32), ("in0", C.c_int32), ("in1", C.c_int32), ("in2", C.c_int32), ("out", C.c_int32),
                ("res", C.c_int32), ("rowbias", C.c_int32), ("ip", C.c_int32 * 12), ("fp", C.c_float * 4),
                ("w", C.c_void_p * 4)]


class NetDesc(C.Structure):
    _fields_ = [("dtype", C.c_int32), ("max_batch", C.c_int32), ("max_tangents", C.c_int32), ("n_buffers", C.c_int32),
                ("n_ops", C.c_int32), ("buffers", C.POINTER(BufferDesc)), ("ops", C.POINTER(OpDesc)),
                ("x_buf", C.c_int32), ("x_channels", C.c_int32), ("temb_buf", C.c_int32), ("temb_dim", C.c_int32),
                ("temb_flip_sin_to_cos", C.c_int32), ("temb_half_minus_one", C.c_int32), ("ctx_buf", C.c_int32)]


_P, _I, _F, _L = C.c_void_p, C.c_int, C.c_float, C.c_int64
SYMBOLS = {
    "dpb_last_error": (C.c_char_p, []),
    "dpb_abi_version": (_I, []),
    "dpb_engine_create": (_I, [C.POINTER(NetDesc), C.POINTER(_P)]),
    "dpb_engine_destroy": (None, [_P]),
    "dpb_engine_set_stream": (_I, [_P, _P]),
    "dpb_engine_workspace_bytes": (C.c_size_t, [_P]),
    "dpb_engine_set_workspace": (_I, [_P, _P, C.c_size_t]),
    "dpb_primal": (_I, [_P, _P, _I, _F, _P, _I]),
    "dpb_forward": (_I, [_P, _P, _I, _F, _P, _I, _I, _P]),
    "dpb_read_buffer": (_I, [_P, _I, _I, _P]),
    "dpb_jvp": (_I, [_P, _I, _P, _I, _P]),
    "dpb_vjp": (_I, [_P, _I, _P, _I, _P]),
    "dpb_orth": (_I, [_P, _P, _P, _P, _P, _P, _I, _L, _P]),
    "dpb_orth_scratch_bytes": (C.c_size_t, [_I, _L]),
    "dpb_orth_checked": (_I, [_P, _P, _P, _P, _P, _P, C.c_size_t, _I, _L, _P]),
    "dpb_pullback_iterate": (_I, [_P, _I, _P, _P, _P, _P, _I, _I]),
    "dpb_ddim_step": (_I, [_P, _P, _P, _P, _L, _F, _F, _P]),
    "dpb_lincomb": (_I, [_P, _P, _P, _P, _L, _F, _F, _F, _P]),
    "dpb_embed_tokens": (_I, [_P, _P, _P, _I, _P, _I, _I, _I, _I, _P]),
    "dpb_engine_stats": (_I, [_P, C.POINTER(_L), C.POINTER(C.c_double), C.POINTER(C.c_double)]),
    "dpb_engine_profile": (_I, [_P, _I]),
    "dpb_debug_set": (_I, [C.c_char_p, _I]),
    "dpb_debug_gemm_plan": (_I, [_I, _I, _I, _I, _I, _I, _I, _L, C.POINTER(_I), C.POINTER(_I), C.POINTER(_I)]),
    "dpb_engine_profile_dump": (_I, [_P, C.c_char_p]),
    "dpb_engine_profile_read": (_I, [_P, _I, C.POINTER(_L), C.POINTER(C.c_double), C.POINTER(C.c_double)]),
    "dpb_engine_profile_overhead": (_I, [_P, C.POINTER(C.c_double)]),
    "dpb_jvp_between": (_I, [_P, _I, _I, _P, _I, _P]),
    "dpb_vjp_between": (_I, [_P, _I, _I, _P, _I, _P]),
    "dpb_pullback_scratch_bytes": (C.c_size_t, [_P, _I, _I]),
    "dpb_pullback_iterate_between": (_I, [_P, _I, _I, _P, _P, _P, _P, _I, _I, _P, C.c_size_t]),
    "dpb_forward_from": (_I, [_P, _P, _I, _F, _P, _I, _P, _I, _I, _P]),
    "dpb_pca_scratch_bytes": (C.c_size_t, [_I, _L, _L]),
    "dpb_pca_lowrank": (_I, [_P, _L, _L, _P, _I, _I, _P, _P, _P, C.c_size_t, _P]),
}

_lib = None


class DpbError(RuntimeError):
    pass


def _source_hash() -> str:
    h = hashlib.sha1()
    files = sorted(glob.glob(os.path.join(CSRC, "*.hip")) + glob.glob(os.path.join(CSRC, "*.h")) + glob.glob(os.path.join(CSRC, "*.cpp"))
                   + [os.path.join(CSRC, "Makefile"), os.path.join(os.path.dirname(_HERE), "include", "dpb.h")])
    for f in files:
        if os.path.exists(f):
            h.update(os.path.basename(f).encode())
            with open(f, "rb") as fh:
                h.update(fh.read())
    return h.hexdigest()


def _built_hash() -> str:
    try:
        with open(STAMP_PATH) as fh:
            return fh.read().strip() if os.path.exists(LIB_PATH) else ""
    except OSError:
        return ""


def _needs_build() -> bool:
    return _source_hash() != _built_hash()


def build(force: bool = False) -> str:
    if force or (os.path.exists(LIB_PATH) and not os.path.exists(STAMP_PATH)):
        subprocess.run(["make", "-C", CSRC, "clean"], check=True, capture_output=True)
    r = subprocess.run(["make", "-C", CSRC, "-j8"], capture_output=True, text=True)
    if r.returncode != 0:
        raise DpbError("hipcc build of libdpb.so failed:\n" + r.stdout[-4000:] + r.stderr[-4000:])
    with open(os.path.join(_HERE, "libdpb.so.srchash"), "w") as fh:
        fh.write(_source_hash())
    return os.path.join(_HERE, "libdpb.so")


def load():
    global _lib
    if _lib is not None:
        return _lib
    if not os.environ.get("DPB_LIB") and os.path.exists(HIPCC) and os.path.isdir(CSRC) and os.access(_HERE, os.W_OK) and _needs_build():
        import fcntl
        import tempfile
        lock = os.path.join(_HERE, ".build.lock")
        try:
            lk = open(lock, "w")
        except OSError:
            lk = open(os.path.join(tempfile.gettempdir(), "dpb-build-%s.lock" % hashlib.sha1(_HERE.encode()).hexdigest()[:12]), "w")
        with lk:
            fcntl.flock(lk, fcntl.LOCK_EX)
            try:
                if _needs_build():
                    build()
            finally:
                fcntl.flock(lk, fcntl.LOCK_UN)
    if not os.path.exists(LIB_PATH):
        raise DpbError(f"{LIB_PATH} not found: build it with `python -c 'import __graft_entry__ as g; g.build()'` "
                       "(there is no CPU fallback for the product path)")
    lib = C.CDLL(LIB_PATH)
    for name, (res, args) in SYMBOLS.items():
        fn = getattr(lib, name)
        fn.restype = res
        fn.argtypes = args
    if lib.dpb_abi_version() != 1:
        raise DpbError("libdpb.so ABI version mismatch")
    _lib = lib
    return lib


def check(rc: int):
    if rc != 0:
        raise DpbError(load().dpb_last_error().decode())
```

### include/dpb.h

```cpp
#ifndef DPB_H
#define DPB_H
#include <stddef.h>
#include <stdint.h>

#ifdef __cplusplus
extern "C" {
#endif

#define DPB_ABI_VERSION 1

enum { DPB_F32 = 0, DPB_BF16 = 1, DPB_F16 = 2 };

enum {
  DPB_OP_CONV = 1,
  DPB_OP_GROUPNORM = 2,
  DPB_OP_LAYERNORM = 3,
  DPB_OP_ATTENTION = 4,
  DPB_OP_GEGLU = 5,
  DPB_OP_SILU = 6,
  DPB_OP_CONCAT = 7
};
enum { DPB_GATHER_NONE = 0, DPB_GATHER_CONV = 1, DPB_GATHER_UPCONV = 3 };
enum { DPB_BUF_ACT = 0,
       DPB_BUF_SHARED = 1    };

typedef struct dpb_buffer_desc {
  int32_t rows;
  int32_t channels;
  int32_t kind;
  int32_t valid_channels;
} dpb_buffer_desc;

typedef struct dpb_op_desc {
  int32_t kind;
  int32_t in0, in1, in2;
  int32_t out;
  int32_t res;
  int32_t rowbias;
  int32_t ip[12];
  float fp[4];
  const void* w[4];
} dpb_op_desc;

typedef struct dpb_net_desc {
  int32_t dtype;
  int32_t max_batch;
  int32_t max_tangents;
  int32_t n_buffers, n_ops;
  const dpb_buffer_desc* buffers;
  const dpb_op_desc* ops;
  int32_t x_buf;
  int32_t x_channels;
  int32_t temb_buf;
  int32_t temb_dim;
  int32_t temb_flip_sin_to_cos;
  int32_t temb_half_minus_one;
  int32_t ctx_buf;
} dpb_net_desc;

typedef struct dpb_engine dpb_engine;

const char* dpb_last_error(void);
int dpb_abi_version(void);

int dpb_engine_create(const dpb_net_desc* net, dpb_engine** out);
void dpb_engine_destroy(dpb_engine* e);
int dpb_engine_set_stream(dpb_engine* e, void* hip_stream);
size_t dpb_engine_workspace_bytes(const dpb_engine* e);
int dpb_engine_set_workspace(dpb_engine* e, void* ws, size_t bytes);

int dpb_primal(dpb_engine* e, const float* x, int batch, float t, const float* ctx, int upto_buf);
int dpb_forward(dpb_engine* e, const float* x, int batch, float t, const float* ctx, int upto_buf, int channels, float* out);
int dpb_read_buffer(dpb_engine* e, int buf, int channels, float* out);

int dpb_jvp(dpb_engine* e, int tap_buf, const float* V, int nt, float* U);
int dpb_vjp(dpb_engine* e, int tap_buf, const float* U, int nt, float* W);

int dpb_orth(const float* W, const float* Vprev, float* V, float* s, float* conv, void* scratch, int k, int64_t N,
             void* hip_stream);
size_t dpb_orth_scratch_bytes(int k, int64_t N);
int dpb_orth_checked(const float* W, const float* Vprev, float* V, float* s, float* conv, void* scratch, size_t scratch_bytes, int k, int64_t N,
                     void* hip_stream);

size_t dpb_pca_scratch_bytes(int q, int64_t N, int64_t D);
int dpb_pca_lowrank(const float* H, int64_t N, int64_t D, const float* R, int q, int niter, float* u, float* s, void* scratch,
                    size_t scratch_bytes, void* hip_stream);

int dpb_pullback_iterate(dpb_engine* e, int tap_buf, float* V, float* U, float* s, float* conv, int k, int n_iters);

int dpb_jvp_between(dpb_engine* e, int src_buf, int dst_buf, const float* V, int nt, float* U);
int dpb_vjp_between(dpb_engine* e, int src_buf, int dst_buf, const float* U, int nt, float* W);
size_t dpb_pullback_scratch_bytes(const dpb_engine* e, int src_buf, int k);
int dpb_pullback_iterate_between(dpb_engine* e, int src_buf, int dst_buf, float* V, float* U, float* s, float* conv, int k, int n_iters,
                                 void* scratch, size_t scratch_bytes);
int dpb_forward_from(dpb_engine* e, const float* x, int batch, float t, const float* ctx, int src_buf, const float* h, int dst_buf, int channels,
                     float* out);

int dpb_ddim_step(const float* x, const float* eps, float* out, float* x0, int64_t n, float alpha_t, float alpha_next,
                  void* hip_stream);
int dpb_lincomb(const float* x, const float* y, const float* z, float* out, int64_t n, float a, float b, float c,
                void* hip_stream);

int dpb_embed_tokens(const int32_t* ids, const void* tok_table, const void* pos_table, int dtype, float* out, int batch,
                     int tokens, int channels, int vocab, void* hip_stream);

int dpb_engine_stats(const dpb_engine* e, int64_t* launches, double* gemm_flops, double* gemm_bytes);
int dpb_engine_profile(dpb_engine* e, int enable);
int dpb_engine_profile_read(dpb_engine* e, int kind, int64_t* count, double* total_ms, double* flops);
int dpb_engine_profile_dump(dpb_engine* e, const char* csv_path);
int dpb_engine_profile_overhead(const dpb_engine* e, double* bracket_overhead_ms);
int dpb_debug_set(const char* key, int value);

int dpb_debug_gemm_plan(int dtype, int M, int N, int K, int conv_hw, int conv_cin, int epilogue, int64_t slab_bytes, int* kind, int* tile,
                        int* splitk);

#ifdef __cplusplus
}
#endif
#endif
```

Measured before the change: 119.5 iters/s.

## Split attention key loop across waves for small-grid attention JVP/adjoint launches

```diff
diff --git a/diffusion_pullback_amd/csrc/attn_fused.hip b/diffusion_pullback_amd/csrc/attn_fused.hip
--- a/diffusion_pullback_amd/csrc/attn_fused.hip
+++ b/diffusion_pullback_amd/csrc/attn_fused.hip
@@ -116,6 +116,34 @@
   if (!on || (ny & 7)) return {(int)blockIdx.x, (int)blockIdx.y};
   const int lin = blockIdx.y * nx + blockIdx.x, xcd = lin & 7, slot = lin >> 3;
   return {slot % nx, (slot / nx) * 8 + xcd};
+}
+
+template <int KS, int NG, int NACC, int LDS_BYTES>
+__device__ inline void ks_combine(f32x16* acc, float* extra, bf16* stage_lds, int rg, int kg, int lane) {
+  if constexpr (KS > 1) {
+    constexpr int NV = NACC * 16 + 1;
+    static_assert(NG * NV * 64 * 4 <= LDS_BYTES, "key-split partials exceed the stage LDS");
+    float* red = reinterpret_cast<float*>(stage_lds) + rg * NV * 64 + lane;
+#pragma unroll
+    for (int r = 1; r < KS; ++r) {
+      __syncthreads();
+      if (kg == r) {
+#pragma unroll
+        for (int i = 0; i < NACC; ++i)
+#pragma unroll
+          for (int e = 0; e < 16; ++e) red[(i * 16 + e) * 64] = acc[i][e];
+        if (extra) red[NACC * 16 * 64] = *extra;
+      }
+      __syncthreads();
+      if (kg == 0) {
+#pragma unroll
+        for (int i = 0; i < NACC; ++i)
+#pragma unroll
+          for (int e = 0; e < 16; ++e) acc[i][e] += red[(i * 16 + e) * 64];
+        if (extra) *extra += red[NACC * 16 * 64];
+      }
+    }
+  }
 }
 
 static int g_attn_shared = getenv("DPB_ATTN_SHARED") ? atoi(getenv("DPB_ATTN_SHARED")) : 2;
@@ -240,15 +268,20 @@
     }
 }
 
-template <int D, int FL, int W = att_waves(D)>
+template <int D, int FL, int W = att_waves(D), int KS = 1>
 __global__ __launch_bounds__((FA<D, W>::NT), (W == 4 && D <= 40 ? 2 : 1)) void attn_jvp_kernel(FusedArgs a) {
   using F = FA<D, W>;
+  constexpr int NG = W / KS, NKB = F::BI / 32 / KS;
+  static_assert(W % KS == 0 && (F::BI / 32) % KS == 0, "key split must divide the waves and the 32-key blocks of a stage");
   __shared__ __attribute__((aligned(16))) bf16 sm[4 * F::ROW_ELEMS];
+  const int tid = threadIdx.x, lane = tid & 63, wave = tid >> 6, l31 = lane & 31, lhi = lane >> 5;
+  const int rg = wave / KS, kg = KS > 1 ? __builtin_amdgcn_readfirstlane(wave) % KS : 0;
   bf16* sK = sm; bf16* sdK = sK + F::ROW_ELEMS; bf16* sV = sdK + F::ROW_ELEMS; bf16* sdV = sV + F::ROW_ELEMS;
-  const int tid = threadIdx.x, lane = tid & 63, wave = tid >> 6, l31 = lane & 31, lhi = lane >> 5;
+  const int koff = kg * 32 * F::LDR;
+  const bf16 *wK = sK + koff, *wdK = sdK + koff, *wV = sV + koff, *wdV = sdV + koff;
   const BlockXY blk = xcd_group_blocks(a.xcd);
   const int j = blk.y / a.H, h = blk.y % a.H, b = j / a.kps;
-  const int q_ = blk.x * (F::WAVES * 32) + wave * 32 + l31;
+  const int q_ = blk.x * (NG * 32) + rg * 32 + l31;
   const bool live = q_ < a.L;
   const int q = live ? q_ : a.L - 1;
   const long LC = (long)a.L * a.C;
@@ -295,21 +328,22 @@
     auto load1 = [&](int kb) {
 #pragma unroll
       for (int stp = 0; stp < F::NS; ++stp) {
-        kf[stp] = lds_a_frag(sK, kb * 32 + l31, F::LDR, stp * 16 + lhi * 8);
-        dkf[stp] = lds_a_frag(sdK, kb * 32 + l31, F::LDR, stp * 16 + lhi * 8);
+        kf[stp] = lds_a_frag(wK, kb * 32 + l31, F::LDR, stp * 16 + lhi * 8);
+        dkf[stp] = lds_a_frag(wdK, kb * 32 + l31, F::LDR, stp * 16 + lhi * 8);
       }
     };
     if constexpr (PIPE) load1(0);
 #pragma unroll
-    for (int kb = 0; kb < F::BI / 32; ++kb) {
+    for (int ib = 0; ib < NKB; ++ib) {
+      const int kb = ib * KS;
       bf16x8 vf[2][F::ND], dvf[2][F::ND];
       if constexpr (PIPE) {
 #pragma unroll
         for (int ks = 0; ks < 2; ++ks)
 #pragma unroll
           for (int d = 0; d < F::ND; ++d) {
-            vf[ks][d] = lds_tr_frag(sV, F::LDR, kb * 32 + ks * 16, d * 32, lane);
-            dvf[ks][d] = lds_tr_frag(sdV, F::LDR, kb * 32 + ks * 16, d * 32, lane);
+            vf[ks][d] = lds_tr_frag(wV, F::LDR, kb * 32 + ks * 16, d * 32, lane);
+            dvf[ks][d] = lds_tr_frag(wdV, F::LDR, kb * 32 + ks * 16, d * 32, lane);
           }
         __builtin_amdgcn_sched_barrier(0);
       } else {
@@ -326,7 +360,7 @@
       }
       if constexpr (PIPE) {
         __builtin_amdgcn_sched_barrier(0);
-        if (kb + 1 < F::BI / 32) load1(kb + 1);
+        if (ib + 1 < NKB) load1(kb + KS);
         __builtin_amdgcn_sched_barrier(0);
       }
       float p[16], x[16];
@@ -344,8 +378,8 @@
 #pragma unroll
         for (int d = 0; d < F::ND; ++d) {
           if constexpr (!PIPE) {
-            vf[ks][d] = lds_tr_frag(sV, F::LDR, kb * 32 + ks * 16, d * 32, lane);
-            dvf[ks][d] = lds_tr_frag(sdV, F::LDR, kb * 32 + ks * 16, d * 32, lane);
+            vf[ks][d] = lds_tr_frag(wV, F::LDR, kb * 32 + ks * 16, d * 32, lane);
+            dvf[ks][d] = lds_tr_frag(wdV, F::LDR, kb * 32 + ks * 16, d * 32, lane);
           }
           if ((DPB_ATT_ABL & 1) && D == 40 && ks == 1 && d == 1) continue;
           acc[d] = MFMA(vf[ks][d], xb[ks], acc[d]);
@@ -353,6 +387,8 @@
         }
     }
   }
+  ks_combine<KS, NG, F::ND, (int)sizeof(sm)>(acc, SUMROW ? nullptr : &delta, sm, rg, kg, lane);
+  const bool owner = kg == 0;
   if constexpr (SUMROW) delta = __shfl(acc[D / 32][((D % 32) & 3) + 4 * ((D % 32) >> 3)], l31, 64);
   else delta += __shfl_xor(delta, 32, 64);
   const long LCo = (long)a.L * a.Co;
@@ -363,7 +399,7 @@
 #pragma unroll
     for (int g = 0; g < 4; ++g) {
       const int col = d * 32 + 8 * g + 4 * lhi;
-      if (col < D && live) {
+      if (col < D && live && owner) {
         uint2 ov = *reinterpret_cast<const uint2*>(Op + col);
         unsigned ow[2] = {ov.x, ov.y};
         unsigned w[2];
@@ -378,20 +414,24 @@
     }
 }
 
-template <int D, int FL>
+template <int D, int FL, int KS = 1>
 __global__ __launch_bounds__(FA<D>::NT) void attn_adj_q_kernel(FusedArgs a) {
   using F = FA<D>;
+  constexpr int NG = F::WAVES / KS, NKB = F::BI / 32 / KS;
+  static_assert(F::WAVES % KS == 0 && (F::BI / 32) % KS == 0, "key split must divide the waves and the 32-key blocks of a stage");
   __shared__ __attribute__((aligned(16))) bf16 sm[2 * F::ROW_ELEMS];
   bf16* sK = sm; bf16* sV = sK + F::ROW_ELEMS;
   const int tid = threadIdx.x, lane = tid & 63, wave = tid >> 6, l31 = lane & 31, lhi = lane >> 5;
   const BlockXY blk = xcd_group_blocks(a.xcd);
   const int j = blk.y / a.H, h = blk.y % a.H, b = j / a.kps;
-  const int q_ = blk.x * (F::WAVES * 32) + wave * 32 + l31;
+  const int rg = wave / KS, kg = KS > 1 ? __builtin_amdgcn_readfirstlane(wave) % KS : 0;
+  const int q_ = blk.x * (NG * 32) + rg * 32 + l31;
   const bool live = q_ < a.L;
   const int q = live ? q_ : a.L - 1;
   const long LC = (long)a.L * a.C;
   const bf16* Kp = a.K + b * LC + h * D;
   const bf16* Vp = a.V + b * LC + h * D;
+  const bf16 *wK = sK + kg * 32 * F::LDR, *wV = sV + kg * 32 * F::LDR;
   bf16x8 qf[F::NS], gof[F::NS], of[F::NS];
   load_outer_frags<D>(a.Q + b * LC + (long)q * a.C + h * D, qf, lhi);
   const long LCo = (long)a.L * a.Co;
@@ -425,14 +465,15 @@
       fetch_row<D>(Kp + (long)k1 * a.C, a.C, rK, tid); fetch_row<D>(Vp + (long)k1 * a.C, a.C, rV, tid);
     }
 #pragma unroll
-    for (int kb = 0; kb < F::BI / 32; ++kb) {
+    for (int ib = 0; ib < NKB; ++ib) {
+      const int kb = ib * KS;
       f32x16 s, gp;
 #pragma unroll
       for (int r = 0; r < 16; ++r) s[r] = gp[r] = 0.f;
 #pragma unroll
       for (int stp = 0; stp < F::NS; ++stp) {
-        s = MFMA(lds_a_frag(sK, kb * 32 + l31, F::LDR, stp * 16 + lhi * 8), qf[stp], s);
-        gp = MFMA(lds_a_frag(sV, kb * 32 + l31, F::LDR, stp * 16 + lhi * 8), gof[stp], gp);
+        s = MFMA(lds_a_frag(wK, kb * 32 + l31, F::LDR, stp * 16 + lhi * 8), qf[stp], s);
+        gp = MFMA(lds_a_frag(wV, kb * 32 + l31, F::LDR, stp * 16 + lhi * 8), gof[stp], gp);
       }
       float gs[16];
 #pragma unroll
@@ -443,16 +484,18 @@
       for (int ks = 0; ks < 2; ++ks)
 #pragma unroll
         for (int d = 0; d < F::ND; ++d)
-          acc[d] = MFMA(lds_tr_frag(sK, F::LDR, kb * 32 + ks * 16, d * 32, lane), gsb[ks], acc[d]);
-    }
-  }
+          acc[d] = MFMA(lds_tr_frag(wK, F::LDR, kb * 32 + ks * 16, d * 32, lane), gsb[ks], acc[d]);
+    }
+  }
+  ks_combine<KS, NG, F::ND, (int)sizeof(sm)>(acc, nullptr, sm, rg, kg, lane);
+  const bool owner = kg == 0;
   bf16* gQp = a.gQ + j * LC + (long)q * a.C + h * D;
 #pragma unroll
   for (int d = 0; d < F::ND; ++d)
 #pragma unroll
     for (int g = 0; g < 4; ++g) {
       const int col = d * 32 + 8 * g + 4 * lhi;
-      if (col < D && live) {
+      if (col < D && live && owner) {
         float v[4];
 #pragma unroll
         for (int i = 0; i < 4; ++i) v[i] = a.scale * acc[d][g * 4 + i];
@@ -592,16 +635,19 @@
   }
 }
 
-template <int D, int FL, int W = att_waves(D)>
+template <int D, int FL, int W = att_waves(D), int KS = 1>
 __global__ __launch_bounds__((FA<D, W>::NT), (D <= 40 ? 2 : 1)) void attn_adj_kv_kernel(FusedArgs a) {
   using F = FA<D, W>;
+  constexpr int NG = W / KS, NKB = F::BI / 32 / KS;
+  static_assert(W % KS == 0 && (F::BI / 32) % KS == 0, "query split must divide the waves and the 32-query blocks of a stage");
   __shared__ __attribute__((aligned(16))) bf16 sm[2 * F::ROW_ELEMS];
   __shared__ float sstat[2][F::BI];
   bf16* sQ = sm; bf16* sgO = sQ + F::ROW_ELEMS;
   const int tid = threadIdx.x, lane = tid & 63, wave = tid >> 6, l31 = lane & 31, lhi = lane >> 5;
   const BlockXY blk = xcd_group_blocks(a.xcd);
   const int j = blk.y / a.H, h = blk.y % a.H, b = j / a.kps;
-  const int key_ = blk.x * (F::WAVES * 32) + wave * 32 + l31;
+  const int rg = wave / KS, kg = KS > 1 ? __builtin_amdgcn_readfirstlane(wave) % KS : 0;
+  const int key_ = blk.x * (NG * 32) + rg * 32 + l31;
   const bool live = key_ < a.L;
   const int key = live ? key_ : a.L - 1;
   const long LC = (long)a.L * a.C;
@@ -610,6 +656,8 @@
   const bf16* Op = a.O + b * LCo + h * D;
   const bf16* gOp = a.gO + j * LCo + h * D;
   const float* stp_ = a.stats + ((long)b * a.H + h) * a.L * 2;
+  const bf16 *wQ = sQ + kg * 32 * F::LDR, *wgO = sgO + kg * 32 * F::LDR;
+  const float *wst0 = sstat[0] + kg * 32, *wst1 = sstat[1] + kg * 32;
   bf16x8 kf[F::NS], vf[F::NS];
   load_outer_frags<D>(a.K + b * LC + (long)key * a.C + h * D, kf, lhi);
   load_outer_frags<D>(a.V + b * LC + (long)key * a.C + h * D, vf, lhi);
@@ -649,21 +697,22 @@
       fetch_stats(q1);
     }
 #pragma unroll
-    for (int qb = 0; qb < F::BI / 32; ++qb) {
+    for (int ib = 0; ib < NKB; ++ib) {
+      const int qb = ib * KS;
       f32x16 s, gp;
 #pragma unroll
       for (int r = 0; r < 16; ++r) s[r] = gp[r] = 0.f;
 #pragma unroll
       for (int stp = 0; stp < F::NS; ++stp) {
-        s = MFMA(lds_a_frag(sQ, qb * 32 + l31, F::LDR, stp * 16 + lhi * 8), kf[stp], s);
-        gp = MFMA(lds_a_frag(sgO, qb * 32 + l31, F::LDR, stp * 16 + lhi * 8), vf[stp], gp);
+        s = MFMA(lds_a_frag(wQ, qb * 32 + l31, F::LDR, stp * 16 + lhi * 8), kf[stp], s);
+        gp = MFMA(lds_a_frag(wgO, qb * 32 + l31, F::LDR, stp * 16 + lhi * 8), vf[stp], gp);
       }
       float p[16], gs[16];
 #pragma unroll
       for (int r = 0; r < 16; ++r) {
         const int qi = qb * 32 + (r & 3) + 8 * (r >> 2) + 4 * lhi;
-        p[r] = __builtin_amdgcn_exp2f(c2 * s[r] - sstat[0][qi]);
-        gs[r] = p[r] * (gp[r] - sstat[1][qi]);
+        p[r] = __builtin_amdgcn_exp2f(c2 * s[r] - wst0[qi]);
+        gs[r] = p[r] * (gp[r] - wst1[qi]);
       }
       bf16x8 pb[2], gsb[2];
       pack_b<FL>(p, pb);
@@ -672,11 +721,15 @@
       for (int ks = 0; ks < 2; ++ks)
 #pragma unroll
         for (int d = 0; d < F::ND; ++d) {
-          accV[d] = MFMA(lds_tr_frag(sgO, F::LDR, qb * 32 + ks * 16, d * 32, lane), pb[ks], accV[d]);
-          accK[d] = MFMA(lds_tr_frag(sQ, F::LDR, qb * 32 + ks * 16, d * 32, lane), gsb[ks], accK[d]);
-        }
-    }
-  }
+          accV[d] = MFMA(lds_tr_frag(wgO, F::LDR, qb * 32 + ks * 16, d * 32, lane), pb[ks], accV[d]);
+          accK[d] = MFMA(lds_tr_frag(wQ, F::LDR, qb * 32 + ks * 16, d * 32, lane), gsb[ks], accK[d]);
+        }
+      if constexpr (KS > 1) __builtin_amdgcn_sched_barrier(0);
+    }
+  }
+  ks_combine<KS, NG, F::ND, (int)sizeof(sm)>(accK, nullptr, sm, rg, kg, lane);
+  ks_combine<KS, NG, F::ND, (int)sizeof(sm)>(accV, nullptr, sm, rg, kg, lane);
+  const bool owner = kg == 0;
   bf16* gKp = a.gK + j * LC + (long)key * a.C + h * D;
   bf16* gVp = a.gV + j * LC + (long)key * a.C + h * D;
   const bool kv_same = a.gK == a.gV;
@@ -685,7 +738,7 @@
 #pragma unroll
     for (int g = 0; g < 4; ++g) {
       const int col = d * 32 + 8 * g + 4 * lhi;
-      if (col < D && live) {
+      if (col < D && live && owner) {
         float vk[4], vv[4];
 #pragma unroll
         for (int i = 0; i < 4; ++i) { vk[i] = a.scale * accK[d][g * 4 + i]; vv[i] = accV[d][g * 4 + i]; }
@@ -942,11 +995,51 @@
   const int tid = threadIdx.x, nthr = blockDim.x, lane = tid & 63, wave = tid >> 6, l31 = lane & 31, lhi = lane >> 5;
   const BlockXY blk = xcd_group_blocks(a.xcd);
   const int j = blk.y / a.H, h = blk.y % a.H, b = j / a.kps;
-  const int q = blk.x * (nthr >> 1) + wave * 32 + l31;
-  {
-    constexpr int CPR = F::DP / 8;
-    const bf16* Kp = a.K + (long)b * a.Lk * a.Ck + h * D;
-    const bf16* Vp = a.V + (long)b * a.Lk * a.Ck + h * D;
+  const int q_ = blk.x * (nthr >> 1) + wave * 32 + l31;
+  const bool live = q_ < a.L;
+  const int q = live ? q_ : a.L - 1;
+  bf16x8 qf[F::NS], xf[F::NS];
+  load_outer_frags<D>(a.Q + (long)b * a.L * a.C + (long)q * a.C + h * D, qf, lhi);
+  if (!a.primal) load_outer_frags<D>(a.X + (long)j * a.L * a.Cx + (long)q * a.Cx + h * D, xf, lhi);
+  constexpr int CPR = F::DP / 8, CPT = XKEYS / 8;
+  const bf16* Kp = a.K + (long)b * a.Lk * a.Ck + h * D;
+  const bf16* Vp = a.V + (long)b * a.Lk * a.Ck + h * D;
+  if (nthr == 256 && a.BT) {
+    constexpr int NKV = (XKEYS * CPR + 255) / 256, NBT = (F::DO * CPT + 255) / 256;
+    const bf16* Bp = a.BT + ((long)b * a.H + h) * D * a.Lkp;
+    uint4 kq[NKV], vq[NKV], bq[NBT];
+#pragma unroll
+    for (int i = 0; i < NKV; ++i) {
+      const int c = min(tid + i * 256, XKEYS * CPR - 1), r = c / CPR, cc = (c % CPR) * 8;
+      const long off = (long)min(r, a.Lk - 1) * a.Ck + min(cc, D - 8);
+      kq[i] = *reinterpret_cast<const uint4*>(Kp + off);
+      vq[i] = *reinterpret_cast<const uint4*>(Vp + off);
+    }
+#pragma unroll
+    for (int i = 0; i < NBT; ++i) {
+      const int c = min(tid + i * 256, F::DO * CPT - 1), r = c / CPT, cc = (c % CPT) * 8;
+      bq[i] = *reinterpret_cast<const uint4*>(Bp + (long)min(r, D - 1) * a.Lkp + min(cc, a.Lkp - 8));
+    }
+#pragma unroll
+    for (int i = 0; i < NKV; ++i) {
+      const int c = tid + i * 256, r = c / CPR, cc = (c % CPR) * 8;
+      const bool in = r < a.Lk && cc < D;
+      if (c < XKEYS * CPR) {
+        *reinterpret_cast<uint4*>(sK + r * F::LDR + cc) = in ? kq[i] : make_uint4(0, 0, 0, 0);
+        *reinterpret_cast<uint4*>(sV + r * F::LDR + cc) = in ? vq[i] : make_uint4(0, 0, 0, 0);
+      }
+    }
+#pragma unroll
+    for (int i = 0; i < NBT; ++i) {
+      const int c = tid + i * 256, r = c / CPT, cc = (c % CPT) * 8;
+      if (c < F::DO * CPT) {
+        const uint4 v = (r < D && cc < a.Lkp) ? bq[i] : make_uint4(0, 0, 0, 0);
+        bf16* dst = sBT + r * XLDT + cc;
+        *reinterpret_cast<uint2*>(dst) = make_uint2(v.x, v.y);
+        *reinterpret_cast<uint2*>(dst + 4) = make_uint2(v.z, v.w);
+      }
+    }
+  } else {
     for (int c = tid; c < XKEYS * CPR; c += nthr) {
       const int r = c / CPR, cc = (c % CPR) * 8;
       uint4 kv = make_uint4(0, 0, 0, 0), vv = kv;
@@ -957,7 +1050,6 @@
       *reinterpret_cast<uint4*>(sK + r * F::LDR + cc) = kv;
       *reinterpret_cast<uint4*>(sV + r * F::LDR + cc) = vv;
     }
-    constexpr int CPT = XKEYS / 8;
     if (a.BT) {
       const bf16* Bp = a.BT + ((long)b * a.H + h) * D * a.Lkp;
       for (int c = tid; c < F::DO * CPT; c += nthr) {
@@ -980,9 +1072,6 @@
       }
     }
   }
-  bf16x8 qf[F::NS], xf[F::NS];
-  load_outer_frags<D>(a.Q + (long)b * a.L * a.C + (long)q * a.C + h * D, qf, lhi);
-  if (!a.primal) load_outer_frags<D>(a.X + (long)j * a.L * a.Cx + (long)q * a.Cx + h * D, xf, lhi);
   __syncthreads();
   const bf16* sA = a.a_is_v ? sV : sK;
   f32x16 s[3], t[3];
@@ -1048,7 +1137,7 @@
 #pragma unroll
     for (int g = 0; g < 4; ++g) {
       const int col = d * 32 + 8 * g + 4 * lhi;
-      if (col < D) {
+      if (col < D && live) {
         float v[4];
 #pragma unroll
         for (int i = 0; i < 4; ++i) v[i] = a.c_out * acc[d][g * 4 + i];
@@ -1087,8 +1176,8 @@
   a.c_in = f.adjoint ? 1.f : f.scale; a.c_out = f.adjoint ? f.scale : 1.f;
   a.primal = f.primal;
   if (f.primal) { a.a_is_v = 0; a.c_in = 1.f; a.c_out = 1.f; a.accumulate = 0; }
-  const int waves = f.L >= 128 ? 4 : f.L / 32;
-  dim3 grid(f.L / (waves * 32), nt * f.H);
+  const int waves = 4;
+  dim3 grid((f.L + waves * 32 - 1) / (waves * 32), nt * f.H);
   if (!head_dim_ok(f.d)) { set_error("cross attention: head dim %d unsupported", f.d); return -1; }
   DPB_ATT_DISPATCH(f.d, f.fl, hipLaunchKernelGGL((attn_cross_kernel<D, FL>), grid, dim3(waves * 64), 0, st, a));
   DPB_CHECK(hipGetLastError());
@@ -1172,6 +1261,31 @@
 
 int attn_jvp_block_waves(int d, int L, int pairs) { return att_block_waves(d, L, pairs); }
 
+constexpr int ATT_CUS = 256;
+static int g_attn_keysplit = getenv("DPB_ATTN_KEYSPLIT") ? atoi(getenv("DPB_ATTN_KEYSPLIT")) : 1;
+void attn_debug_keysplit(int v) { g_attn_keysplit = v; }
+int attn_small_plan(int d, int L, int pairs) {
+  if (g_attn_keysplit <= 0 || (d != 80 && d != 160) || L <= 0 || pairs <= 0) return 1;
+  const int rows = att_waves(d) * 32;
+  if ((long)((L + rows - 1) / rows) * pairs >= ATT_CUS) return 1;
+  if (d == 160) return 2;
+  return g_attn_keysplit == 2 || g_attn_keysplit == 4 ? g_attn_keysplit : 1;
+}
+#define DPB_ATT_KS_LAUNCH(KERNEL80, KERNEL160, ks)                                                                               \
+  do {                                                                                                                            \
+    const int rows_ = att_waves(f.d) * 32 / (ks);                                                                                 \
+    const dim3 gk_((f.L + rows_ - 1) / rows_, nt * f.H), bk_(att_waves(f.d) * 64);                                                \
+    if (f.d == 160) { if (f.fl) hipLaunchKernelGGL((KERNEL160(1, 2)), gk_, bk_, 0, st, a); else hipLaunchKernelGGL((KERNEL160(0, 2)), gk_, bk_, 0, st, a); } \
+    else if ((ks) == 2) { if (f.fl) hipLaunchKernelGGL((KERNEL80(1, 2)), gk_, bk_, 0, st, a); else hipLaunchKernelGGL((KERNEL80(0, 2)), gk_, bk_, 0, st, a); } \
+    else { if (f.fl) hipLaunchKernelGGL((KERNEL80(1, 4)), gk_, bk_, 0, st, a); else hipLaunchKernelGGL((KERNEL80(0, 4)), gk_, bk_, 0, st, a); } \
+  } while (0)
+#define DPB_JVP80(FLV, KSV) attn_jvp_kernel<80, FLV, 8, KSV>
+#define DPB_JVP160(FLV, KSV) attn_jvp_kernel<160, FLV, 4, KSV>
+#define DPB_ADJQ80(FLV, KSV) attn_adj_q_kernel<80, FLV, KSV>
+#define DPB_ADJQ160(FLV, KSV) attn_adj_q_kernel<160, FLV, KSV>
+#define DPB_ADJKV80(FLV, KSV) attn_adj_kv_kernel<80, FLV, 8, KSV>
+#define DPB_ADJKV160(FLV, KSV) attn_adj_kv_kernel<160, FLV, 4, KSV>
+
 int launch_attn_jvp_fused(const FusedAttnArgs& f, int nt, hipStream_t st) {
   FusedArgs a = to_args(f);
   if (!head_dim_ok(f.d)) { set_error("fused attention: head dim %d unsupported", f.d); return -1; }
@@ -1182,6 +1296,11 @@
     DPB_CHECK(hipGetLastError());
     return 0;
   }
+  if (const int ks = attn_small_plan(f.d, f.L, nt * f.H); ks > 1) {
+    DPB_ATT_KS_LAUNCH(DPB_JVP80, DPB_JVP160, ks);
+    DPB_CHECK(hipGetLastError());
+    return 0;
+  }
   dim3 grid((f.L + att_waves(f.d) * 32 - 1) / (att_waves(f.d) * 32), nt * f.H);
   DPB_ATT_DISPATCH(f.d, f.fl, hipLaunchKernelGGL((attn_jvp_kernel<D, FL>), grid, dim3(att_waves(D) * 64), 0, st, a));
   DPB_CHECK(hipGetLastError());
@@ -1205,6 +1324,12 @@
   dim3 grid((f.L + att_waves(f.d) * 32 - 1) / (att_waves(f.d) * 32), nt * f.H);
   if (!head_dim_ok(f.d)) { set_error("fused attention: head dim %d unsupported", f.d); return -1; }
   const int route = attn_adj_route(f.d, f.L, f.kps, nt, f.Drow != nullptr);
+  if (const int ks = attn_small_plan(f.d, f.L, nt * f.H); ks > 1) {
+    DPB_ATT_KS_LAUNCH(DPB_ADJQ80, DPB_ADJQ160, ks);
+    DPB_ATT_KS_LAUNCH(DPB_ADJKV80, DPB_ADJKV160, ks);
+    DPB_CHECK(hipGetLastError());
+    return 0;
+  }
   if (route & 1) {
     constexpr int TJ = 5;
     const int ngrp = (f.kps + TJ - 1) / TJ;
diff --git a/diffusion_pullback_amd/csrc/engine.cpp b/diffusion_pullback_amd/csrc/engine.cpp
--- a/diffusion_pullback_amd/csrc/engine.cpp
+++ b/diffusion_pullback_amd/csrc/engine.cpp
@@ -1408,6 +1408,7 @@
   else if (!strcmp(key, "gn_deterministic")) { gn_debug_deterministic(value); return 0; }
   else if (!strcmp(key, "graph_iterate")) { g_graph_iterate = value; return 0; }
   else if (!strcmp(key, "attn_shared")) { attn_debug_shared(value); return 0; }
+  else if (!strcmp(key, "attn_keysplit")) { attn_debug_keysplit(value); return 0; }
   else if (!strcmp(key, "lazy_reduce")) { g_lazy_reduce = value; return 0; }
   else if (!strcmp(key, "ln_fuse")) { g_ln_fuse = value; return 0; }
   else if (!strcmp(key, "cross_primal")) { g_cross_primal = value; return 0; }
@@ -1438,6 +1439,13 @@
   return 0;
 }
 
+int dpb_debug_attn_plan(int d, int L, int pairs, int* keysplit) {
+  if (!keysplit) return fail("null argument");
+  if (d <= 0 || L <= 0 || pairs <= 0) return fail("attention plan: d, L and pairs must be positive");
+  *keysplit = attn_small_plan(d, L, pairs);
+  return 0;
+}
+
 int dpb_engine_stats(const dpb_engine* e, int64_t* launches, double* gemm_flops, double* gemm_bytes) {
   if (!e) return fail("null engine");
   if (launches) *launches = e->n_launch;
diff --git a/diffusion_pullback_amd/csrc/kernels.h b/diffusion_pullback_amd/csrc/kernels.h
--- a/diffusion_pullback_amd/csrc/kernels.h
+++ b/diffusion_pullback_amd/csrc/kernels.h
@@ -131,6 +131,8 @@
 int launch_row_stats(int fl, const void* S, float* stats, long nrows, int Lk, int ld, hipStream_t st);
 int attn_adj_route_bits(int d, int L, int kps, int nt);
 int attn_adj_launches(int d, int L, int kps, int nt);
+int attn_small_plan(int d, int L, int pairs);
+void attn_debug_keysplit(int v);
 int attn_jvp_block_waves(int d, int L, int pairs);
 int launch_attn_fwd_fused(const FusedAttnArgs& f, int batch, void* O, float* stats, hipStream_t st);
 int launch_attn_jvp_fused(const FusedAttnArgs& f, int nt, hipStream_t st);
diff --git a/diffusion_pullback_amd/lib.py b/diffusion_pullback_amd/lib.py
--- a/diffusion_pullback_amd/lib.py
+++ b/diffusion_pullback_amd/lib.py
@@ -68,6 +68,7 @@
     "dpb_engine_profile": (_I, [_P, _I]),
     "dpb_debug_set": (_I, [C.c_char_p, _I]),
     "dpb_debug_gemm_plan": (_I, [_I, _I, _I, _I, _I, _I, _I, _L, C.POINTER(_I), C.POINTER(_I), C.POINTER(_I)]),
+    "dpb_debug_attn_plan": (_I, [_I, _I, _I, C.POINTER(_I)]),
     "dpb_engine_profile_dump": (_I, [_P, C.c_char_p]),
     "dpb_engine_profile_read": (_I, [_P, _I, C.POINTER(_L), C.POINTER(C.c_double), C.POINTER(C.c_double)]),
     "dpb_engine_profile_overhead": (_I, [_P, C.POINTER(C.c_double)]),
diff --git a/include/dpb.h b/include/dpb.h
--- a/include/dpb.h
+++ b/include/dpb.h
@@ -114,6 +114,8 @@
 int dpb_debug_gemm_plan(int dtype, int M, int N, int K, int conv_hw, int conv_cin, int epilogue, int64_t slab_bytes, int* kind, int* tile,
                         int* splitk);
 
+int dpb_debug_attn_plan(int d, int L, int pairs, int* keysplit);
+
 #ifdef __cplusplus
 }
 #endif
```

Result: no change. 120.2 iters/s, median of 6 (+0.6%).
